# deepsound-project/pggan-pytorch

Measured on AMD Instinct MI355X. Metric: images/sec, PGGAN full train step (D+GP step + G step + Adam) at 1024x1024, higher is better.
Workload: dtype f32; 1 GPU; BASELINE config 5: PGGAN 1024x1024 net (fmap_base 4096, C=3, latent 512), stage depth 8 = 1024x1024, alpha 1.00, minibatch 3/GPU (reference schedule), Trainer.train(): WGAN-GP + Adam(0,0.99) at lr 0, fp32; resolution=1024, depth=8, minibatch_per_gpu=3, global_batch=3, parallelism=dp1, fmap_base=4096, hip_graphs=False

## Files before the change

pggan-pytorch_amd/_lib.py:

```python
import ast
import ctypes
import os
import re

_HERE = os.path.dirname(os.path.abspath(__file__))
LIB_PATH = os.environ.get('PGGAN_HIP_LIB') or os.path.join(_HERE, 'libpggan_hip.so')
_INCLUDE = os.path.join(os.path.dirname(_HERE), 'include')


class PgganLibraryError(RuntimeError):
    pass


P = ctypes.c_void_p
I = ctypes.c_int
L = ctypes.c_int64
F = ctypes.c_float
D = ctypes.c_double

_ARGTYPES = {'pg_stream_t': P, 'int': I, 'int64_t': L, 'float': F, 'double': D, 'size_t': ctypes.c_size_t, 'uint64_t': ctypes.c_uint64}
_RESTYPES = {'int': I, 'const char*': ctypes.c_char_p}


def _define_value(name, text):
    def value(node):
        if isinstance(node, ast.Constant) and type(node.value) is int:
            return node.value
        if isinstance(node, ast.UnaryOp) and isinstance(node.op, ast.USub):
            return -value(node.operand)
        if isinstance(node, ast.BinOp) and isinstance(node.op, ast.LShift):
            return value(node.left) << value(node.right)
        raise PgganLibraryError('#define %s %s: not an integer expression' % (name, text))
    try:
        return value(ast.parse(text.strip(), mode='eval').body)
    except SyntaxError:
        raise PgganLibraryError('#define %s %s: not an integer expression' % (name, text))


def _argtype(name, param):
    if '*' in param:
        return P
    words = [w for w in param.split() if w != 'const']
    ctype = ' '.join(words[:-1])
    if ctype not in _ARGTYPES or not re.fullmatch(r'[A-Za-z_]\w*', words[-1]):
        raise PgganLibraryError('%s: parameter "%s" has no ctypes mapping' % (name, ' '.join(param.split())))
    return _ARGTYPES[ctype]


def parse_header(text):
    text = re.sub(r'/\*.*?\*/|//[^\n]*', ' ', text, flags=re.S)
    guards = set(re.findall(r'^[ \t]*#[ \t]*define[ \t]+(\w+)[ \t]*$', text, flags=re.M))
    constants, body, conditionals = {}, [], []
    for line in text.split('\n'):
        directive = re.match(r'\s*#\s*(\w+)\s*(.*?)\s*$', line)
        foreign = next((c for c in conditionals if c), None)
        if foreign and re.search(r'\bpg_\w+\s*\(|#\s*define\s+PG_', line):
            raise PgganLibraryError('declaration under the preprocessor conditional "%s": %s' % (foreign, line.strip()))
        if not directive:
            body.append(line)
            continue
        word, rest = directive.groups()
        if word in ('if', 'ifdef', 'ifndef'):
            known = (word, rest) == ('ifdef', '__cplusplus') or word == 'ifndef' and rest in guards
            conditionals.append(None if known else line.strip())
        elif word == 'endif':
            conditionals.pop()
        elif word == 'define' and rest.startswith('PG_'):
            name, value = re.match(r'(\w+)(.*)', rest).groups()
            constants[name] = _define_value(name, value)
    body = '\n'.join(body)
    argtypes, restypes = {}, {}
    for m in re.finditer(r'\b(pg_\w+)\s*\(', body):
        name = m.group(1)
        params = re.compile(r'([^()]*)\)\s*;').match(body, m.end())
        if not params:
            raise PgganLibraryError('%s: cannot read the parameter list' % name)
        ret = ' '.join(body[max(body.rfind(c, 0, m.start()) for c in ';{}') + 1:m.start()].split()).replace(' *', '*')
        if ret not in _RESTYPES:
            raise PgganLibraryError('%s: return type "%s" has no ctypes mapping' % (name, ret))
        params = [p.strip() for p in params.group(1).split(',')]
        argtypes[name] = [] if params in ([''], ['void']) else [_argtype(name, p) for p in params]
        restypes[name] = _RESTYPES[ret]
    return argtypes, restypes, constants


def _read_header(name):
    try:
        with open(os.path.join(_INCLUDE, name)) as f:
            return parse_header(f.read())
    except OSError as e:
        raise PgganLibraryError('cannot read the C-ABI header %s: %s' % (name, e))


SIGNATURES, _RESTYPE_OF, CONSTANTS = _read_header('pggan_hip.h')
DEBUG_SIGNATURES, _debug_restypes, _ = _read_header('pggan_hip_debug.h')
_RESTYPE_OF.update(_debug_restypes)
CLUSTER_SIGNATURES, _cluster_restypes, CLUSTER_CONSTANTS = _read_header('pggan_hip_cluster.h')
_RESTYPE_OF.update(_cluster_restypes)
GAN_SIGNATURES, _gan_restypes, GAN_CONSTANTS = _read_header('pggan_hip_gan.h')
_RESTYPE_OF.update(_gan_restypes)
PHASE_SIGNATURES, _phase_restypes, PHASE_CONSTANTS = _read_header('pggan_hip_phase.h')
_RESTYPE_OF.update(_phase_restypes)
SAMPLING_SIGNATURES, _sampling_restypes, SAMPLING_CONSTANTS = _read_header('pggan_hip_sampling.h')
_RESTYPE_OF.update(_sampling_restypes)
PROJECTION_SIGNATURES, _projection_restypes, PROJECTION_CONSTANTS = _read_header('pggan_hip_projection.h')
_RESTYPE_OF.update(_projection_restypes)
CROP_SIGNATURES, _crop_restypes, CROP_CONSTANTS = _read_header('pggan_hip_crop.h')
_RESTYPE_OF.update(_crop_restypes)
SWD_SIGNATURES, _swd_restypes, SWD_CONSTANTS = _read_header('pggan_hip_swd.h')
_RESTYPE_OF.update(_swd_restypes)
MEL_SIGNATURES, _mel_restypes, MEL_CONSTANTS = _read_header('pggan_hip_mel.h')
_RESTYPE_OF.update(_mel_restypes)
RESAMPLE_SIGNATURES, _resample_restypes, RESAMPLE_CONSTANTS = _read_header('pggan_hip_resample.h')
_RESTYPE_OF.update(_resample_restypes)
SHIFT_SIGNATURES, _shift_restypes, SHIFT_CONSTANTS = _read_header('pggan_hip_shift.h')
_RESTYPE_OF.update(_shift_restypes)
PRD_SIGNATURES, _prd_restypes, PRD_CONSTANTS = _read_header('pggan_hip_prd.h')
_RESTYPE_OF.update(_prd_restypes)
AUGMENT_SIGNATURES, _augment_restypes, AUGMENT_CONSTANTS = _read_header('pggan_hip_augment.h')
_RESTYPE_OF.update(_augment_restypes)
EMBED_SIGNATURES, _embed_restypes, EMBED_CONSTANTS = _read_header('pggan_hip_embed.h')
_RESTYPE_OF.update(_embed_restypes)
ABI_VERSION = CONSTANTS['PG_ABI_VERSION']

_lib = None


def load():
    global _lib
    if _lib is not None:
        return _lib
    if not os.path.exists(LIB_PATH):
        raise PgganLibraryError(
            'libpggan_hip.so not found at %s: the HIP extension is not built (run '
            '`python __graft_entry__.py`). There is no CPU fallback.' % LIB_PATH)
    try:
        lib = ctypes.CDLL(LIB_PATH)
    except OSError as e:
        raise PgganLibraryError('cannot load %s: %s' % (LIB_PATH, e))
    for name, argtypes in (list(SIGNATURES.items()) + list(DEBUG_SIGNATURES.items()) + list(CLUSTER_SIGNATURES.items())
                           + list(GAN_SIGNATURES.items()) + list(PHASE_SIGNATURES.items()) + list(SAMPLING_SIGNATURES.items())
                           + list(PROJECTION_SIGNATURES.items()) + list(CROP_SIGNATURES.items()) + list(SWD_SIGNATURES.items())
                           + list(MEL_SIGNATURES.items()) + list(RESAMPLE_SIGNATURES.items()) + list(SHIFT_SIGNATURES.items())
                           + list(PRD_SIGNATURES.items()) + list(AUGMENT_SIGNATURES.items()) + list(EMBED_SIGNATURES.items())):
        try:
            fn = getattr(lib, name)
        except AttributeError:
            raise PgganLibraryError('symbol %s missing from %s' % (name, LIB_PATH))
        fn.argtypes = argtypes
        fn.restype = _RESTYPE_OF[name]
    v = lib.pg_abi_version()
    if v != ABI_VERSION:
        raise PgganLibraryError('ABI version mismatch: library %d, binding %d' % (v, ABI_VERSION))
    _lib = lib
    return lib


_ERR = {CONSTANTS['PG_E_ARG']: 'PG_E_ARG (bad dimension / null pointer)', CONSTANTS['PG_E_ALIGN']: 'PG_E_ALIGN (channel count / alignment)',
        CONSTANTS['PG_E_UNSUP']: 'PG_E_UNSUP (unsupported configuration)', CONSTANTS['PG_E_NOLIB']: 'PG_E_NOLIB (no RCCL library could be loaded)'}
_E_UNSUP, _E_RCCL_BASE = CONSTANTS['PG_E_UNSUP'], CONSTANTS['PG_E_RCCL_BASE']


class Unsupported(RuntimeError):
    """PG_E_UNSUP: the entry point does not take this configuration (callers with a fallback catch exactly this)."""


def check(rc, name):
    if rc != 0:
        what = _ERR.get(rc) or ('RCCL ncclResult_t %d' % (_E_RCCL_BASE - rc) if rc <= _E_RCCL_BASE else 'hipError_t %d' % rc)
        raise (Unsupported if rc == _E_UNSUP else RuntimeError)('%s failed: %s' % (name, what))


CALL_HOOK = None


def call(name, *args):
    fn = getattr(load(), name)
    check(fn(*args) if CALL_HOOK is None else CALL_HOOK(fn, args, name), name)
```

pggan-pytorch_amd/csrc/conv_api.hip:

```cpp
#include "convp.h"

__thread char pgk::g_last_kernel[96] = "";
__thread int pgk::g_tune[4] = {-1, -1, -1, -1};

namespace {

using namespace pgk;

__device__ __forceinline__ void pack_dgrad_tile(const float* __restrict__ w, float* __restrict__ wt, int KS, int Cout, int Cin,
                                                int tap, int ci_b, int co_b)
{
    __shared__ float tile[32][33];
    const int kh = tap / KS, kw = tap % KS;
    const int otap = (KS - 1 - kh) * KS + (KS - 1 - kw);
    const int tx = threadIdx.x & 31, ty = threadIdx.x >> 5;
    for (int r = ty; r < 32; r += 8) {
        const int co = co_b + r, ci = ci_b + tx;
        tile[r][tx] = (co < Cout && ci < Cin) ? w[((size_t)tap * Cout + co) * Cin + ci] : 0.f;
    }
    __syncthreads();
    for (int r = ty; r < 32; r += 8) {
        const int ci = ci_b + r, co = co_b + tx;
        if (ci < Cin && co < Cout) wt[((size_t)otap * Cin + ci) * Cout + co] = tile[tx][r];
    }
}

__global__ void pack_dgrad_kernel(const float* __restrict__ w, float* __restrict__ wt, int KS, int Cout, int Cin)
{
    pack_dgrad_tile(w, wt, KS, Cout, Cin, blockIdx.z, blockIdx.x * 32, blockIdx.y * 32);
}

constexpr int PACK_MAX_LAYERS = 32;
struct PackDesc {
    int n;
    int first_block[PACK_MAX_LAYERS + 1];
    long long off[PACK_MAX_LAYERS];
    int ks[PACK_MAX_LAYERS], cout[PACK_MAX_LAYERS], cin[PACK_MAX_LAYERS];
};

__global__ void pack_dgrad_batched_kernel(const float* __restrict__ wbase, float* __restrict__ wtbase, PackDesc d)
{
    int l = 0;
    while (l + 1 < d.n && (int)blockIdx.x >= d.first_block[l + 1]) ++l;
    const int Cout = d.cout[l], Cin = d.cin[l];
    int b = blockIdx.x - d.first_block[l];
    const int nbx = (Cin + 31) / 32, nby = (Cout + 31) / 32;
    const int bx = b % nbx; b /= nbx;
    const int by = b % nby; const int tap = b / nby;
    pack_dgrad_tile(wbase + d.off[l], wtbase + d.off[l], d.ks[l], Cout, Cin, tap, bx * 32, by * 32);
}

}

static int second_pass(const ConvP& want, bool pooled, pg_stream_t stream)
{
    const int64_t P = (int64_t)want.N * want.Hout * want.Wout;
    if (want.ypool && !pooled)
        return pg_avgpool2_fwd(want.y, want.pool_other, want.ypool, want.N, want.Hout >> 1, want.Wout >> 1, want.Cout, want.pool_a, want.pool_b, stream);
    if (want.yup) return pg_avgpool2_bwd(want.y, want.upmask, want.yup, want.N, want.Hout, want.Wout, want.Cout, want.up_mul, want.mask_slope, stream);
    if (want.pn_r) return pg_pixelnorm_fwd(want.y, want.y, want.pn_r, P, want.Cout, want.pn_eps, stream);
    if (want.pnb_y) return pg_pixelnorm_lrelu_bwd(want.y, want.pnb_y, want.pnb_r, want.y, P, want.Cout, want.mask_slope, stream);
    return 0;
}

static bool thin_shape(const ConvP& p, bool channels)
{
    return channels && p.KS == 3 && p.pad == 1 && (p.Wout & 31) == 0 && (p.Hout & 7) == 0 && g_tune[PG_TUNE_PATH] != PG_PATH_NO_THIN;
}

static ConvP conv_request(const float* x, const float* w, const float* bias, const float* mask, float* y,
                          int N, int Hin, int Win, int Cin, int Cout, int KS, int pad, float scale, float slope, float mask_slope)
{
    ConvP p;
    p.x = x; p.w = w; p.bias = bias; p.mask = mask; p.y = y;
    p.N = N; p.Hin = Hin; p.Win = Win; p.Cin = Cin; p.Cout = Cout; p.KS = KS; p.pad = pad;
    p.scale = scale; p.slope = slope; p.mask_slope = mask_slope;
    return p;
}

static int conv2d_impl(ConvP& p, int flags, pg_stream_t stream)
{
    if (!p.x || !p.w || !p.y || p.N <= 0 || p.Hin <= 0 || p.Win <= 0 || p.Cin <= 0 || p.Cout <= 0) return PG_E_ARG;
    if ((p.Cin & 3) || (p.Cout & 3)) return PG_E_ALIGN;
    const int KS = p.KS, Cin = p.Cin, Cout = p.Cout;
    p.ups = flags & PG_FLAG_UPSAMPLE;
    p.mask_bytes = (flags & PG_FLAG_MASK_BYTES) ? 1 : 0; p.y_bytes = (flags & PG_FLAG_Y_BYTES) ? 1 : 0;
    if (flags & PG_FLAG_SIGNS_OUT) {
        if (!p.mask || p.mask_bytes) return PG_E_ARG;
        p.ysigns = reinterpret_cast<unsigned char*>(const_cast<float*>(p.mask));
        p.mask = nullptr;
    }
    p.Hout = p.Hin + 2 * p.pad - KS + 1; p.Wout = p.Win + 2 * p.pad - KS + 1;
    if (p.Hout <= 0 || p.Wout <= 0 || !is_pow2(p.Hout) || !is_pow2(p.Wout)) return PG_E_UNSUP;
    if (p.ups && ((p.Hin | p.Win) & 1)) return PG_E_ARG;
    if (p.ypool && ((p.Hout | p.Wout) & 1)) return PG_E_ARG;
    if ((long long)p.N * p.Hin * p.Win * Cin >= (1ll << 31) || (long long)p.N * p.Hout * p.Wout * Cout >= (1ll << 31) ||
        (long long)KS * KS * Cout * Cin >= (1ll << 31)) return PG_E_UNSUP;
    const ConvP want = p;
    if (KS != 3) p.ypool = nullptr;
    p.yup = nullptr; p.pn_r = nullptr; p.pnb_y = nullptr;
    hipStream_t s = (hipStream_t)stream;
    int rc;
    if (p.mask_bytes || p.y_bytes || p.ysigns) {
        if (KS != 3 || (p.y_bytes && !p.ypool) || want.pn_r || want.pnb_y) return PG_E_UNSUP;
        p.yup = want.yup;
        const bool thin_plain = !p.y_bytes && !p.yup && !p.ypool && ((Cout == 8 && (Cin == 8 || Cin == 16)) || (Cout == 16 && Cin == 8 && p.mask));
        const bool thin_pool = g_tune[PG_TUNE_PATH] != PG_PATH_NO_THIN_POOL16 && !p.yup && p.ypool && Cout == 16 && Cin == 8;
        return thin_shape(p, thin_plain || thin_pool) ? dispatch_thin(p, s) : dispatch_conv_tile(p, s);
    }
    const bool thin_pn = thin_shape(p, Cout == 8 && (Cin == 8 || Cin == 16));
    if (want.pnb_y && want.pnb_r && KS == 3 && Cout <= 32) {
        p.pnb_y = want.pnb_y;
        rc = thin_pn ? dispatch_thin(p, s) : dispatch_conv_tile(p, s);
        if (rc != PG_E_UNSUP) return rc;
        p.pnb_y = nullptr;
    }
    if (want.pn_r && KS == 3 && Cout <= 32 && !p.mask && g_tune[PG_TUNE_PATH] != PG_PATH_UNFUSED_PIXELNORM) {
        p.pn_r = want.pn_r;
        rc = thin_pn ? dispatch_thin(p, s) : dispatch_conv_tile(p, s);
        if (rc != PG_E_UNSUP) return rc;
        p.pn_r = nullptr;
    }
    if (want.yup && KS == 3) {
        p.yup = want.yup;
        rc = dispatch_conv_tile(p, s);
        if (rc != PG_E_UNSUP) return rc;
        p.yup = nullptr;
    }
    if (thin_shape(p, (Cout == 8 && (Cin == 8 || Cin == 16)) || (Cout == 16 && Cin == 8 && p.mask && !want.ypool)))
        rc = dispatch_thin(p, s);
    else if (k4_layer(p, KS))
        rc = launch_k4_conv(p, s);
    else
        rc = dispatch_conv_tile(p, s);
    if (rc) return rc;
    return second_pass(want, p.ypool && p.ksplit == 1, stream);
}

extern "C" int pg_conv2d_nhwc(const float* x, const float* w, const float* bias, const float* mask, float* y,
                              int N, int Hin, int Win, int Cin, int Cout, int KS, int pad, int ups,
                              float scale, float slope, float mask_slope, pg_stream_t stream)
{
    ConvP p = conv_request(x, w, bias, mask, y, N, Hin, Win, Cin, Cout, KS, pad, scale, slope, mask_slope);
    return conv2d_impl(p, ups, stream);
}

extern "C" int pg_conv2d_pixelnorm_nhwc(const float* x, const float* w, const float* bias, float* y, float* r,
                                        int N, int Hin, int Win, int Cin, int Cout, int KS, int pad, int ups,
                                        float scale, float slope, float eps, pg_stream_t stream)
{
    if (!r) return PG_E_ARG;
    ConvP p = conv_request(x, w, bias, nullptr, y, N, Hin, Win, Cin, Cout, KS, pad, scale, slope, 0.2f);
    p.pn_r = r; p.pn_eps = eps;
    return conv2d_impl(p, ups, stream);
}

extern "C" int pg_conv2d_pnbwd_nhwc(const float* x, const float* w, const float* ysaved, const float* r, float* y,
                                    int N, int Hin, int Win, int Cin, int Cout, int KS, int pad,
                                    float scale, float slope, pg_stream_t stream)
{
    if (!ysaved) return PG_E_ARG;
    ConvP p = conv_request(x, w, nullptr, nullptr, y, N, Hin, Win, Cin, Cout, KS, pad, scale, 1.0f, slope);
    p.pnb_y = ysaved; p.pnb_r = r;
    return conv2d_impl(p, 0, stream);
}

extern "C" int pg_conv2d_unpool_nhwc(const float* x, const float* w, const float* upmask, float* y, float* yup,
                                     int N, int Hin, int Win, int Cin, int Cout, int KS, int pad, int flags,
                                     float scale, float up_mul, float mask_slope, pg_stream_t stream)
{
    if (!yup) return PG_E_ARG;
    ConvP p = conv_request(x, w, nullptr, nullptr, y, N, Hin, Win, Cin, Cout, KS, pad, scale, 1.0f, mask_slope);
    p.yup = yup; p.upmask = upmask; p.up_mul = up_mul;
    return conv2d_impl(p, flags & PG_FLAG_MASK_BYTES, stream);
}

extern "C" int pg_conv2d_pool_nhwc(const float* x, const float* w, const float* bias, const float* mask, float* y,
                                   float* ypool, const float* pool_other, float pool_a, float pool_b, int pool_only,
                                   int N, int Hin, int Win, int Cin, int Cout, int KS, int pad, int ups,
                                   float scale, float slope, float mask_slope, pg_stream_t stream)
{
    if (!ypool) return PG_E_ARG;
    ConvP p = conv_request(x, w, bias, mask, y, N, Hin, Win, Cin, Cout, KS, pad, scale, slope, mask_slope);
    p.ypool = ypool; p.pool_other = pool_other; p.pool_a = pool_a; p.pool_b = pool_b; p.pool_only = pool_only;
    return conv2d_impl(p, ups, stream);
}

extern "C" int pg_conv2d_unpooled_nhwc(const float* g, const float* w, const unsigned char* gbytes, float gmul, float gslope,
                                       const float* mask, float* y, int N, int Hin, int Win, int Cin, int Cout, int flags,
                                       float scale, float mask_slope, pg_stream_t stream)
{
    if (!g || !w || !gbytes || !y || N <= 0 || Hin <= 0 || Win <= 0) return PG_E_ARG;
    if ((Hin | Win) & 1) return PG_E_ARG;
    if (!(Cout == 8 && (Cin == 8 || Cin == 16)) || (Win & 31) || (Hin & 7) || !is_pow2(Hin) || !is_pow2(Win)) return PG_E_UNSUP;
    if ((long long)N * Hin * Win * Cin >= (1ll << 31)) return PG_E_UNSUP;
    ConvP p = conv_request(g, w, nullptr, mask, y, N, Hin, Win, Cin, Cout, 3, 1, scale, 1.f, mask_slope);
    p.ups = 1; p.Hout = Hin; p.Wout = Win;
    p.mask_bytes = (flags & PG_FLAG_MASK_BYTES) ? 1 : 0;
    p.gbytes = gbytes; p.gmul = gmul; p.gslope = gslope;
    return dispatch_thin(p, (hipStream_t)stream);
}

extern "C" int pg_conv2d_fromrgb_nhwc(const float* img, const float* rgb_w, const float* rgb_b, float rgb_scale, float rgb_slope,
                                      unsigned char* x_signs, const float* w, const float* bias, float* y, unsigned char* y_signs,
                                      int N, int C, int H, int W, int Cmid, int Cout, float scale, float slope, pg_stream_t stream)
{
    if (!img || !rgb_w || !w || !y || N <= 0 || C <= 0 || H <= 0 || W <= 0 || Cmid <= 0 || Cout <= 0) return PG_E_ARG;
    return pgk::launch_conv_strip_fromrgb(img, rgb_w, rgb_b, rgb_scale, rgb_slope, x_signs, w, bias, y, y_signs, N, C, H, W, Cmid, Cout,
                                          scale, slope, (hipStream_t)stream);
}

extern "C" int pg_conv2d_pixelnorm_torgb_nhwc(const float* x, const float* w, const float* bias, float* y, float* r,
                                              const float* t_w, const float* t_b, float t_scale, float* img,
                                              int N, int C, int H, int W, int Cin, int Cout, float scale, float slope, float eps,
                                              pg_stream_t stream)
{
    if (!x || !w || !y || !r || !t_w || !img || N <= 0 || C <= 0 || H <= 0 || W <= 0 || Cin <= 0 || Cout <= 0) return PG_E_ARG;
    return pgk::launch_conv_strip_pn_torgb(x, w, bias, y, r, t_w, t_b, t_scale, img, N, C, H, W, Cin, Cout, scale, slope, eps,
                                           (hipStream_t)stream);
}

extern "C" int pg_conv2d_masked_fromrgb_bwd_nhwc(const float* gz, const float* wt, const unsigned char* mask_bytes, float mask_slope, float* y,
                                                 const float* rgb_w, float rgb_scale, float* gimg,
                                                 const float* img, float* rgb_dw, float* rgb_db,
                                                 int N, int C, int H, int W, int Cin, int Cout, float scale, pg_stream_t stream)
{
    if (!gz || !wt || !mask_bytes || N <= 0 || C <= 0 || H <= 0 || W <= 0 || Cin <= 0 || Cout <= 0) return PG_E_ARG;
    if ((!gimg && !rgb_dw) || (gimg && !rgb_w) || (rgb_dw && !img) || (rgb_db && !rgb_dw)) return PG_E_ARG;
    return pgk::launch_conv_strip_masked_rgb_bwd(gz, wt, mask_bytes, mask_slope, y, rgb_w, rgb_scale, gimg, img, rgb_dw, rgb_db,
                                                 N, C, H, W, Cin, Cout, scale, (hipStream_t)stream);
}

extern "C" const char* pg_debug_last_conv_kernel(void) { return g_last_kernel; }

extern "C" int pg_debug_set_tuning(int key, int value)
{
    if (key < 0 || key >= 4) return PG_E_ARG;
    g_tune[key] = value;
    return 0;
}

extern "C" int pg_pack_dgrad_weights_batched(const float* wbase, float* wtbase, int nlayers, const int64_t* off,
                                             const int* ks, const int* cout, const int* cin, pg_stream_t stream)
{
    if (!wbase || !wtbase || nlayers <= 0 || !off || !ks || !cout || !cin) return PG_E_ARG;
    for (int l0 = 0; l0 < nlayers; l0 += PACK_MAX_LAYERS) {
        PackDesc d;
        d.n = nlayers - l0 < PACK_MAX_LAYERS ? nlayers - l0 : PACK_MAX_LAYERS;
        int total = 0;
        for (int l = 0; l < d.n; ++l) {
            const int i = l0 + l;
            if (ks[i] <= 0 || cout[i] <= 0 || cin[i] <= 0 || off[i] < 0) return PG_E_ARG;
            d.first_block[l] = total;
            d.off[l] = off[i]; d.ks[l] = ks[i]; d.cout[l] = cout[i]; d.cin[l] = cin[i];
            total += ((cin[i] + 31) / 32) * ((cout[i] + 31) / 32) * ks[i] * ks[i];
        }
        d.first_block[d.n] = total;
        hipLaunchKernelGGL(pack_dgrad_batched_kernel, dim3(total), dim3(256), 0, (hipStream_t)stream, wbase, wtbase, d);
    }
    return (int)hipGetLastError();
}

extern "C" int pg_pack_dgrad_weights(const float* w, float* wt, int KS, int Cout, int Cin, pg_stream_t stream)
{
    if (!w || !wt || KS <= 0 || Cout <= 0 || Cin <= 0) return PG_E_ARG;
    dim3 grid((Cin + 31) / 32, (Cout + 31) / 32, KS * KS);
    hipLaunchKernelGGL(pack_dgrad_kernel, grid, dim3(256), 0, (hipStream_t)stream, w, wt, KS, Cout, Cin);
    return (int)hipGetLastError();
}
```

pggan-pytorch_amd/csrc/conv_strip.hip:

```cpp
#include "convp.h"

#ifndef PG_STRIP_ABL
#define PG_STRIP_ABL 0
#endif

namespace {

using pgk::ConvP;
using pgk::pg_sign_byte;
using pgk::pg_sign_factors;
using pgk::g_last_kernel; using pgk::set_smem; using pgk::SMEM_ANY;

constexpr int SW = 64;
constexpr int RP = SW + 2;
constexpr int RB = 4;
constexpr int NBLK = 3;

enum { EPI_GENERIC = 0, EPI_FWD = 1, EPI_MASK = 2, EPI_PN = 3, EPI_PNB = 4 };

struct SArgs {
    const float* x; const float* w; const float* bias; const void* mask; float* y;
    unsigned char* ysigns; float* pn_r; const float* pnb_y; const float* pnb_r; float* ypool; const float* pool_other;
    float scale, slope, mask_slope, pn_eps, pool_a, pool_b;
    int H, W, ups, mask_bytes, y_bytes, pool_only;
    int strips, segs, seg_rows;
    const unsigned char* gbytes; float gmul, gslope;
    const float* rgb_w; const float* rgb_b; float rgb_scale, rgb_slope; int rgbC; unsigned char* xsigns;
    float* t_out; const float* t_w; const float* t_b; float t_scale; int tC, t_sc, t_sco, t_only;
    const float* fw_img; float* fw_dw; float* fw_db; float fw_scale;
};

template <int CIN> struct Blk {
    static constexpr int C4 = CIN / 4;
    static constexpr int USED = C4 * RB * RP;
    static constexpr int NWI = (USED + 63) / 64;
    static constexpr int NI = (NWI + 3) / 4;
    static constexpr int SLOTS = NWI * 64;
};

typedef __attribute__((address_space(3))) const char* lds_cptr;
typedef __attribute__((address_space(3))) const f32x4* lds_v4ptr;

__device__ __forceinline__ pg_u32x4 rsrc_words(const void* base, unsigned bytes)
{
    const unsigned long long a = (unsigned long long)base;
    return pg_u32x4{(unsigned)__builtin_amdgcn_readfirstlane((int)(unsigned)a),
                    (unsigned)__builtin_amdgcn_readfirstlane((int)((unsigned)(a >> 32) & 0xffffu)), bytes, 0x00020000u};
}
__device__ __forceinline__ void buf_store4(__amdgpu_buffer_rsrc_t r, unsigned voff, float4 v)
{
    __builtin_amdgcn_raw_buffer_store_b128(pg_u32x4{__float_as_uint(v.x), __float_as_uint(v.y), __float_as_uint(v.z), __float_as_uint(v.w)},
                                           r, (int)voff, 0, 0);
}

constexpr int RGB_MAXC = 3;
template <int COUT, int CIN, int EPI, bool WREG, int GM, int XM = 0>
__device__ __forceinline__ void conv_strip_body(const SArgs& p)
{
    constexpr bool GATH = GM != 0;
    using B = Blk<CIN>;
    constexpr int C4 = B::C4;
    constexpr int QO = COUT / 4, QP = 16 / QO, PXG = 4 * QP;
    constexpr int GPR = 32 / PXG, G = 2 * GPR;
    constexpr int BLKB = B::SLOTS * 16;
    constexpr bool GEN = EPI == EPI_GENERIC;
    extern __shared__ __align__(16) float lds[];
    constexpr int WS = CIN == 16 ? CIN + 4 : CIN;
    float* wl = lds + NBLK * B::SLOTS * 4;
    const int tid = threadIdx.x, lane = tid & 63, wave = __builtin_amdgcn_readfirstlane(tid >> 6);
    const int blk = lane >> 2, j = lane & 3, qo = blk % QO, qp = blk / QO;

    int t = (int)pg_xcd_remap(blockIdx.x, gridDim.x);
    const int strip = __builtin_amdgcn_readfirstlane(t % p.strips); t /= p.strips;
    const int seg = __builtin_amdgcn_readfirstlane(t % p.segs), n = __builtin_amdgcn_readfirstlane(t / p.segs);
    const int r0 = seg * p.seg_rows, ow0 = strip * SW;
    const int niter = p.seg_rows / RB;
    const int xH = p.ups ? (p.H >> 1) : p.H, xW = p.ups ? (p.W >> 1) : p.W;
    const unsigned npix = (unsigned)(p.H * p.W);

    const unsigned rowbytes = 4u * (unsigned)(xW * CIN);
    unsigned voff[B::NI], vstep[B::NI];
    const unsigned blkstep = (p.ups ? 2u : 4u) * rowbytes;
#pragma unroll
    for (int i = 0; i < B::NI; ++i) {
        const int sl = (i * 4 + wave) * 64 + lane;
        const int q = sl / (RB * RP), rem = sl - q * (RB * RP);
        const int m = rem / RP, px = rem - m * RP;
        const int col = ow0 - 1 + px, row = r0 - 1 + m;
        const bool ok = sl < B::USED && (unsigned)col < (unsigned)p.W;
        voff[i] = ok ? (unsigned)(p.ups ? (row >> 1) : row) * rowbytes + 4u * (unsigned)((p.ups ? (col >> 1) : col) * CIN + 4 * q) : PG_OOB;
        vstep[i] = ok ? blkstep : 0u;
    }
    const size_t ximg = (size_t)xH * xW * CIN;
    const pg_u32x4 rxs = rsrc_words(p.x + (size_t)n * ximg, (unsigned)(ximg * 4));
    const unsigned lds0 = (unsigned)(size_t)(__attribute__((address_space(3))) char*)lds;
    const unsigned wdst = __builtin_amdgcn_readfirstlane(lds0 + (unsigned)wave * 1024u);
    auto dma16 = [&](unsigned vo, unsigned dst) {
        unsigned keep;
        asm volatile("s_mov_b32 %0, m0\n\ts_mov_b32 m0, %3\n\ts_nop 0\n\tbuffer_load_dwordx4 %1, %2, 0 offen lds\n\ts_mov_b32 m0, %0"
                     : "=&s"(keep) : "v"(vo), "s"(rxs), "s"(dst) : "memory");
    };
    auto issue_block = [&](int pos) {
#pragma unroll
        for (int i = 0; i < B::NI; ++i) {
            if (i * 4 + wave < B::NWI) dma16(voff[i], wdst + (unsigned)pos * BLKB + (unsigned)i * 4096u);
            voff[i] += vstep[i];
        }
    };

    constexpr int NG = GATH ? (B::USED + 255) / 256 : 1;
    unsigned cvo[NG], cvs[NG], bvo[NG], bvs[NG];
    float4 gxr[NG];
    unsigned gbr[NG];
    __amdgpu_buffer_rsrc_t rgx = pg_make_rsrc(p.x + (size_t)n * ximg, (unsigned)(ximg * 4)), rgb = rgx;
    constexpr int NR = GM == 2 ? NG : 1;
    int rrow[NR];
    float rw[NR][4][RGB_MAXC], rb[NR][4], rpx[NR][RGB_MAXC];
    if constexpr (GM == 2) {
        rgx = pg_make_rsrc(p.x + (size_t)n * npix * p.rgbC, npix * (unsigned)p.rgbC * 4u);
        rgb = pg_make_rsrc(p.xsigns + (size_t)n * npix * C4, npix * C4);
#pragma unroll
        for (int i = 0; i < NG; ++i) {
            const int sl = i * 256 + tid;
            const int q = sl / (RB * RP), rem = sl - q * (RB * RP);
            const int m = rem / RP, px = rem - m * RP;
            const int col = ow0 - 1 + px;
            const bool ok = sl < B::USED && (unsigned)col < (unsigned)p.W;
            rrow[i] = ok ? r0 - 1 + m : -(1 << 28);
            cvo[i] = ok ? 4u * (unsigned)((r0 - 1 + m) * p.W + col) : PG_OOB;
            cvs[i] = ok ? 4u * (unsigned)(RB * p.W) : 0u;
            bvo[i] = (ok && px >= 1 && px <= SW) ? (unsigned)((r0 - 1 + m) * p.W + col) * C4 + q : PG_OOB;
            bvs[i] = (ok && px >= 1 && px <= SW) ? (unsigned)(RB * p.W * C4) : 0u;
            const int qq = sl < B::USED ? q : 0;
#pragma unroll
            for (int k = 0; k < 4; ++k) {
#pragma unroll
                for (int c = 0; c < RGB_MAXC; ++c) rw[i][k][c] = c < p.rgbC ? p.rgb_w[(4 * qq + k) * p.rgbC + c] : 0.f;
                rb[i][k] = p.rgb_b ? p.rgb_b[4 * qq + k] : 0.f;
            }
        }
    }
    if constexpr (GM == 1) {
        rgb = pg_make_rsrc(p.gbytes + (size_t)n * npix * C4, npix * C4);
#pragma unroll
        for (int i = 0; i < NG; ++i) {
            const int sl = i * 256 + tid;
            const int q = sl / (RB * RP), rem = sl - q * (RB * RP);
            const int m = rem / RP, px = rem - m * RP;
            const int col = ow0 - 1 + px, row = r0 - 1 + m;
            const bool ok = sl < B::USED && (unsigned)col < (unsigned)p.W;
            cvo[i] = ok ? (unsigned)(row >> 1) * rowbytes + 4u * (unsigned)((col >> 1) * CIN + 4 * q) : PG_OOB;
            cvs[i] = ok ? 2u * rowbytes : 0u;
            bvo[i] = ok ? (unsigned)(row * p.W + col) * C4 + q : PG_OOB;
            bvs[i] = ok ? (unsigned)(RB * p.W * C4) : 0u;
        }
    }
    auto gather_load = [&]() {
        if constexpr (GM == 2) {
#pragma unroll
            for (int i = 0; i < NG; ++i) {
                const bool in = (unsigned)rrow[i] < (unsigned)p.H;
#pragma unroll
                for (int c = 0; c < RGB_MAXC; ++c)
                    rpx[i][c] = c < p.rgbC ? __uint_as_float(__builtin_amdgcn_raw_buffer_load_b32(rgx, in ? (int)(cvo[i] + (unsigned)c * npix * 4u) : (int)PG_OOB, 0, 0)) : 0.f;
                cvo[i] += cvs[i];
            }
            return;
        }
#pragma unroll
        for (int i = 0; i < NG; ++i) {
            gxr[i] = pg_buf_load4(rgx, cvo[i], 0);
            gbr[i] = __builtin_amdgcn_raw_buffer_load_b8(rgb, (int)bvo[i], 0, 0);
            cvo[i] += cvs[i]; bvo[i] += bvs[i];
        }
    };
    auto gather_store = [&](int pos) {
        if constexpr (GM == 2) {
#pragma unroll
            for (int i = 0; i < NG; ++i) {
                const int sl = i * 256 + tid;
                const bool in = (unsigned)rrow[i] < (unsigned)p.H;
                float o[4];
#pragma unroll
                for (int k = 0; k < 4; ++k) {
                    float a = 0.f;
#pragma unroll
                    for (int c = 0; c < RGB_MAXC; ++c) if (c < p.rgbC) a = fmaf(rpx[i][c], rw[i][k][c], a);
                    const float v = __fadd_rn(__fmul_rn(a, p.rgb_scale), rb[i][k]);
                    o[k] = in ? (v > 0.f ? v : v * p.rgb_slope) : 0.f;
                }
                const float4 v4 = make_float4(o[0], o[1], o[2], o[3]);
                if (sl < B::SLOTS) *reinterpret_cast<float4*>(lds + (pos * B::SLOTS + sl) * 4) = (cvs[i] ? v4 : make_float4(0.f, 0.f, 0.f, 0.f));
                if (p.xsigns && in && rrow[i] >= r0 && rrow[i] < r0 + p.seg_rows && bvs[i])
                    __builtin_amdgcn_raw_buffer_store_b8(pg_sign_byte(v4), rgb, (int)bvo[i], 0, 0);
                bvo[i] += bvs[i];
                rrow[i] += RB;
            }
            return;
        }
#pragma unroll
        for (int i = 0; i < NG; ++i) {
            const int sl = i * 256 + tid;
            if (sl < B::SLOTS) {
                const float4 f = pg_sign_factors((unsigned char)gbr[i], p.gslope);
                const float4 v = gxr[i];
                *reinterpret_cast<float4*>(lds + (pos * B::SLOTS + sl) * 4) =
                    make_float4(v.x * (f.x * p.gmul), v.y * (f.y * p.gmul), v.z * (f.z * p.gmul), v.w * (f.w * p.gmul));
            }
        }
    };

    float4 wreg[WREG ? 9 : 1][WREG ? C4 : 1];
    if constexpr (WREG) {
#pragma unroll
        for (int tp = 0; tp < 9; ++tp)
#pragma unroll
            for (int c4 = 0; c4 < C4; ++c4)
                wreg[tp][c4] = *reinterpret_cast<const float4*>(p.w + ((size_t)(tp * COUT + 4 * qo + j) * CIN + 4 * c4));
    } else {
        for (int e = tid; e < 9 * COUT * C4; e += 256)
            *reinterpret_cast<float4*>(wl + (e / C4) * WS + 4 * (e % C4)) = *reinterpret_cast<const float4*>(p.w + 4 * e);
    }
    const float* wrow = wl + (4 * qo + j) * WS;

    if constexpr (GATH) {
        gather_load(); gather_store(0);
        gather_load(); gather_store(1);
    } else {
        issue_block(0);
        issue_block(1);
    }

    const int rp = wave >> 1;
    const int col0 = (wave & 1) * 32;
    const lds_cptr lbase = (lds_cptr)lds + (col0 + 4 * qp + j) * 16;

    const bool has_mask = (GEN && p.mask) || EPI == EPI_MASK;
    const bool mask_bytes = has_mask && p.mask_bytes;
    const bool has_pnb = (GEN && p.pnb_y) || EPI == EPI_PNB;
    const bool has_pn = (GEN && p.pn_r) || EPI == EPI_PN;
    const bool has_signs = (GEN || EPI == EPI_FWD) && p.ysigns;
    const bool has_pool = GEN && p.ypool;
    const bool y_bytes = GEN && p.y_bytes;
    const bool has_trgb = (XM & 1) != 0 && (EPI == EPI_PN || EPI == EPI_MASK) && p.t_out != nullptr;
    const bool has_fw = (XM & 2) != 0 && EPI == EPI_MASK && COUT == 8 && p.fw_dw != nullptr;
    const bool y_store = !(has_pool && p.pool_only) && !y_bytes && !((has_trgb || has_fw) && p.t_only);
    const __amdgpu_buffer_rsrc_t ry = y_bytes ? pg_make_rsrc((const unsigned char*)p.y + (size_t)n * npix * (COUT / 4), npix * (COUT / 4))
                                              : pg_make_rsrc(p.y + (size_t)n * npix * COUT, npix * COUT * 4u);
    __amdgpu_buffer_rsrc_t rmask = ry, rsig = ry, rpnr = ry, rpnby = ry, rpnbr = ry;
    if (has_mask) rmask = mask_bytes ? pg_make_rsrc((const unsigned char*)p.mask + (size_t)n * npix * (COUT / 4), npix * (COUT / 4))
                                     : pg_make_rsrc((const float*)p.mask + (size_t)n * npix * COUT, npix * COUT * 4u);
    if (has_signs) rsig = pg_make_rsrc(p.ysigns + (size_t)n * npix * (COUT / 4), npix * (COUT / 4));
    if (has_pn) rpnr = pg_make_rsrc(p.pn_r + (size_t)n * npix, npix * 4u);
    if (has_pnb) {
        rpnby = pg_make_rsrc(p.pnb_y + (size_t)n * npix * COUT, npix * COUT * 4u);
        rpnbr = pg_make_rsrc(p.pnb_r + (size_t)n * npix, npix * 4u);
    }
    const unsigned pix0 = (unsigned)((r0 + 2 * rp) * p.W + ow0 + col0 + 4 * qp + j);
    float4 bv = make_float4(0.f, 0.f, 0.f, 0.f);
    if (!has_mask && p.bias) bv = *reinterpret_cast<const float4*>(p.bias + 4 * qo);
    float tw[RGB_MAXC][4], tb[RGB_MAXC];
    float aw[4][RGB_MAXC], ab[4], fi[G][RGB_MAXC];
#pragma unroll
    for (int k = 0; k < 4; ++k) {
        ab[k] = 0.f;
#pragma unroll
        for (int c = 0; c < RGB_MAXC; ++c) aw[k][c] = 0.f;
    }
    __amdgpu_buffer_rsrc_t rfimg = ry;
    if (has_fw) rfimg = pg_make_rsrc(p.fw_img + (size_t)n * npix * p.tC, npix * (unsigned)p.tC * 4u);
    __amdgpu_buffer_rsrc_t rtout = ry;
    if (has_trgb) {
        rtout = pg_make_rsrc(p.t_out + (size_t)n * npix * p.tC, npix * (unsigned)p.tC * 4u);
#pragma unroll
        for (int c = 0; c < RGB_MAXC; ++c) {
#pragma unroll
            for (int k = 0; k < 4; ++k) tw[c][k] = c < p.tC ? p.t_w[c * p.t_sc + (4 * qo + k) * p.t_sco] : 0.f;
            tb[c] = (c < p.tC && p.t_b) ? p.t_b[c] : 0.f;
        }
    }

    f32x4 acc[G], acc2[G];
    auto compute = [&](auto ph_, auto rp_) {
        constexpr int PH = decltype(ph_)::value, RPAIR = decltype(rp_)::value;
#pragma unroll
        for (int g = 0; g < G; ++g) { acc[g] = f32x4{0.f, 0.f, 0.f, 0.f}; acc2[g] = f32x4{0.f, 0.f, 0.f, 0.f}; }
#pragma unroll
        for (int tp = 0; tp < ((PG_STRIP_ABL & 4) ? 1 : 9); ++tp) {
            const int dy = tp / 3, dx = tp % 3;
#pragma unroll
            for (int c4 = 0; c4 < C4; ++c4) {
                float4 a;
                if constexpr (WREG) a = wreg[tp][c4];
                else a = *reinterpret_cast<const float4*>(wrow + tp * COUT * WS + 4 * c4);
                f32x4 bq[G];
#pragma unroll
                for (int g = 0; g < G; ++g) {
                    const int m = 2 * RPAIR + g / GPR + dy;
                    const int pos = m < RB ? PH : (PH + 1) % NBLK;
                    const int off = ((pos * B::SLOTS) + c4 * (RB * RP) + (m & (RB - 1)) * RP + (g % GPR) * PXG + dx) * 16;
                    bq[g] = *(lds_v4ptr)(lbase + off);
                }
#pragma unroll
                for (int g = 0; g < G; ++g) acc[g] = __builtin_amdgcn_mfma_f32_4x4x1f32(a.x, bq[g][0], acc[g], 0, 0, 0);
#pragma unroll
                for (int g = 0; g < G; ++g) acc2[g] = __builtin_amdgcn_mfma_f32_4x4x1f32(a.y, bq[g][1], acc2[g], 0, 0, 0);
#pragma unroll
                for (int g = 0; g < G; ++g) acc[g] = __builtin_amdgcn_mfma_f32_4x4x1f32(a.z, bq[g][2], acc[g], 0, 0, 0);
#pragma unroll
                for (int g = 0; g < G; ++g) acc2[g] = __builtin_amdgcn_mfma_f32_4x4x1f32(a.w, bq[g][3], acc2[g], 0, 0, 0);
            }
        }
#pragma unroll
        for (int g = 0; g < G; ++g) acc[g] += acc2[g];
    };

    float4 pm[G];
    unsigned pmb[G];
    float prr[G];
    auto prefetch_epilogue = [&](unsigned pix) {
#pragma unroll
        for (int g = 0; g < G; ++g) {
            const unsigned pg_ = pix + (unsigned)((g / GPR) * p.W + (g % GPR) * PXG);
            if (has_fw) {
#pragma unroll
                for (int c = 0; c < RGB_MAXC; ++c)
                    fi[g][c] = c < p.tC ? __uint_as_float(__builtin_amdgcn_raw_buffer_load_b32(rfimg, (int)(((unsigned)c * npix + pg_) * 4u), 0, 0)) : 0.f;
            }
            if (has_mask) {
                if (mask_bytes) pmb[g] = __builtin_amdgcn_raw_buffer_load_b8(rmask, (int)(pg_ * (COUT / 4) + qo), 0, 0);
                else pm[g] = pg_buf_load4(rmask, (pg_ * COUT + 4 * qo) * 4u, 0);
            } else if (has_pnb) {
                pm[g] = pg_buf_load4(rpnby, (pg_ * COUT + 4 * qo) * 4u, 0);
                prr[g] = __uint_as_float(__builtin_amdgcn_raw_buffer_load_b32(rpnbr, (int)(pg_ * 4u), 0, 0));
            }
        }
    };
    auto epilogue = [&](unsigned pix) {
        float4 ov[G];
#pragma unroll
        for (int g = 0; g < G; ++g) {
            const unsigned pg_ = pix + (unsigned)((g / GPR) * p.W + (g % GPR) * PXG);
            const unsigned off = pg_ * COUT + 4 * qo;
            float4 o = make_float4(acc[g][0] * p.scale, acc[g][1] * p.scale, acc[g][2] * p.scale, acc[g][3] * p.scale);
            if (has_mask) {
                float4 f;
                if (mask_bytes) f = pg_sign_factors((unsigned char)pmb[g], p.mask_slope);
                else {
// ... 28 lines not shown
                o.x *= rr; o.y *= rr; o.z *= rr; o.w *= rr;
                if (qo == 0 && !(PG_STRIP_ABL & 2)) __builtin_amdgcn_raw_buffer_store_b32(__float_as_uint(rr), rpnr, (int)(pg_ * 4u), 0, 0);
            }
            if (has_fw) {
                const float ov4[4] = {o.x, o.y, o.z, o.w};
#pragma unroll
                for (int k = 0; k < 4; ++k) {
                    ab[k] += ov4[k];
#pragma unroll
                    for (int c = 0; c < RGB_MAXC; ++c) aw[k][c] = fmaf(ov4[k], fi[g][c], aw[k][c]);
                }
            }
            if (has_trgb) {
#pragma unroll
                for (int c = 0; c < RGB_MAXC; ++c) {
                    if (c >= p.tC) break;
                    float a = fmaf(o.w, tw[c][3], fmaf(o.z, tw[c][2], fmaf(o.y, tw[c][1], o.x * tw[c][0])));
                    a += __shfl_xor(a, 4, 64);
                    if (QO >= 4) a += __shfl_xor(a, 8, 64);
                    if (qo == 0) __builtin_amdgcn_raw_buffer_store_b32(__float_as_uint(fmaf(a, p.t_scale, tb[c])), rtout, (int)(((unsigned)c * npix + pg_) * 4u), 0, 0);
                }
            }
            if (!(PG_STRIP_ABL & 2)) {
                if (y_bytes) __builtin_amdgcn_raw_buffer_store_b8(pg_sign_byte(o), ry, (int)(off >> 2), 0, 0);
                else if (y_store) buf_store4(ry, off * 4u, o);
            }
            ov[g] = o;
        }
        if (has_pool) {
#pragma unroll
            for (int g = 0; g < G; ++g) {
                ov[g].x += __shfl_xor(ov[g].x, 1, 64); ov[g].y += __shfl_xor(ov[g].y, 1, 64);
                ov[g].z += __shfl_xor(ov[g].z, 1, 64); ov[g].w += __shfl_xor(ov[g].w, 1, 64);
            }
#pragma unroll
            for (int g = 0; g < GPR; ++g) {
                float4 v = make_float4((ov[g].x + ov[g + GPR].x) * 0.25f, (ov[g].y + ov[g + GPR].y) * 0.25f,
                                       (ov[g].z + ov[g + GPR].z) * 0.25f, (ov[g].w + ov[g + GPR].w) * 0.25f);
                if (j & 1) continue;
                const unsigned pg_ = pix + (unsigned)(g * PXG);
                const unsigned oy = pg_ / (unsigned)p.W, ox = pg_ - oy * (unsigned)p.W;
                const size_t poff = (((size_t)n * (p.H >> 1) + (oy >> 1)) * (p.W >> 1) + (ox >> 1)) * COUT + 4 * qo;
                if (p.pool_other) {
                    const float4 q = *reinterpret_cast<const float4*>(p.pool_other + poff);
                    v.x = fmaf(v.x, p.pool_a, p.pool_b * q.x); v.y = fmaf(v.y, p.pool_a, p.pool_b * q.y);
                    v.z = fmaf(v.z, p.pool_a, p.pool_b * q.z); v.w = fmaf(v.w, p.pool_a, p.pool_b * q.w);
                } else if (p.pool_a != 1.f) { v.x *= p.pool_a; v.y *= p.pool_a; v.z *= p.pool_a; v.w *= p.pool_a; }
                *reinterpret_cast<float4*>(p.ypool + poff) = v;
            }
        }
    };

    int nstores = (y_bytes || y_store) ? G : 0;
    if (has_signs) nstores += G;
    if (has_pn) nstores += G;
    if (has_pool) nstores += GPR;
    if (has_trgb) nstores += G * p.tC;
    if (PG_STRIP_ABL & 2) nstores = 0;
    nstores = __builtin_amdgcn_readfirstlane(nstores);
    auto wait_dma = [&]() {
        if constexpr (EPI == EPI_MASK || EPI == EPI_PNB || EPI == EPI_PN) {
            static_assert(G == 2, "");
            if (!has_trgb && !has_fw) {
                if constexpr (EPI == EPI_PN) asm volatile("s_waitcnt vmcnt(4)" ::: "memory");
                else asm volatile("s_waitcnt vmcnt(2)" ::: "memory");
            } else switch (nstores) {
                case 2: asm volatile("s_waitcnt vmcnt(2)" ::: "memory"); break;
                case 4: asm volatile("s_waitcnt vmcnt(4)" ::: "memory"); break;
                case 6: asm volatile("s_waitcnt vmcnt(6)" ::: "memory"); break;
                case 8: asm volatile("s_waitcnt vmcnt(8)" ::: "memory"); break;
                case 10: asm volatile("s_waitcnt vmcnt(10)" ::: "memory"); break;
                default: asm volatile("s_waitcnt vmcnt(0)" ::: "memory"); break;
            }
        }
        else switch (nstores) {
            case 0: asm volatile("s_waitcnt vmcnt(0)" ::: "memory"); break;
            case 1: asm volatile("s_waitcnt vmcnt(1)" ::: "memory"); break;
            case 2: asm volatile("s_waitcnt vmcnt(2)" ::: "memory"); break;
            case 3: asm volatile("s_waitcnt vmcnt(3)" ::: "memory"); break;
            case 4: asm volatile("s_waitcnt vmcnt(4)" ::: "memory"); break;
            case 5: asm volatile("s_waitcnt vmcnt(5)" ::: "memory"); break;
            default: asm volatile("s_waitcnt vmcnt(6)" ::: "memory"); break;
        }
    };
    unsigned pix = pix0;
    const unsigned pixstep = (unsigned)(RB * p.W);
    auto step = [&](int it, auto ph_) {
        constexpr int PH = decltype(ph_)::value;
        if constexpr (!GATH) {
            if (it == 0 || (PG_STRIP_ABL & 2)) asm volatile("s_waitcnt vmcnt(0)" ::: "memory");
            else wait_dma();
        }
        __syncthreads();
        const bool more = it + 2 <= niter;
        if constexpr (GATH) { if (more) gather_load(); }
        else if (more && !((PG_STRIP_ABL & 1) && it > 0)) issue_block((PH + 2) % NBLK);
        prefetch_epilogue(pix);
        __builtin_amdgcn_sched_barrier(0);
        if (rp == 0) compute(ph_, std::integral_constant<int, 0>{});
        else compute(ph_, std::integral_constant<int, 1>{});
        if constexpr (GATH) { if (more) gather_store((PH + 2) % NBLK); }
        epilogue(pix);
        pix += pixstep;
    };
    for (int it = 0; it < niter; it += 3) {
        step(it, std::integral_constant<int, 0>{});
        if (it + 1 < niter) step(it + 1, std::integral_constant<int, 1>{});
        if (it + 2 < niter) step(it + 2, std::integral_constant<int, 2>{});
    }
    if (has_fw) {
        static_assert(COUT != 8 || QO == 2, "");
        float v[16];
#pragma unroll
        for (int k = 0; k < 4; ++k) {
#pragma unroll
            for (int c = 0; c < RGB_MAXC; ++c) v[4 * k + c] = aw[k][c];
            v[4 * k + 3] = ab[k];
        }
#pragma unroll
        for (int i = 0; i < 16; ++i) {
            float a = v[i];
            a += __shfl_xor(a, 1, 64); a += __shfl_xor(a, 2, 64); a += __shfl_xor(a, 8, 64); a += __shfl_xor(a, 16, 64); a += __shfl_xor(a, 32, 64);
            v[i] = a;
        }
        __syncthreads();
        if ((lane & ~4) == 0) {
#pragma unroll
            for (int i = 0; i < 16; ++i) lds[(wave * 2 + (lane >> 2)) * 16 + i] = v[i];
        }
        __syncthreads();
        const int q2 = (tid >> 4) & 1, i = tid & 15, k = i >> 2, c = i & 3, co = 4 * q2 + k;
        auto commit = [&](float a) {
            if (c < 3) { if (c < p.tC) atomicAdd(p.fw_dw + co * p.tC + c, a * p.fw_scale); }
            else if (p.fw_db) atomicAdd(p.fw_db + co, a);
        };
        float a = 0.f;
        if (tid < 32) a = (lds[(0 * 2 + q2) * 16 + i] + lds[(1 * 2 + q2) * 16 + i]) + (lds[(2 * 2 + q2) * 16 + i] + lds[(3 * 2 + q2) * 16 + i]);
        if (tid < 32) commit(a);
    }
}

template <int COUT, int CIN, int EPI, bool WREG, bool GATH>
__global__ __launch_bounds__(256, GATH ? 2 : (WREG ? 3 : 4)) void conv_strip_kernel(SArgs p)
{
    conv_strip_body<COUT, CIN, EPI, WREG, GATH ? 1 : 0>(p);
}

template <int EPI, bool WREG, int XM>
__global__ __launch_bounds__(256, 3) void conv_strip_x_kernel(SArgs p)
{
    conv_strip_body<8, 8, EPI, WREG, 0, XM>(p);
}

template <int EPI>
__global__ __launch_bounds__(256, 2) void conv_strip_rgb_kernel(SArgs p)
{
    conv_strip_body<8, 8, EPI, false, 2>(p);
}

template <int COUT, int CIN, int EPI, bool WREG, bool GATH = false>
int launch_strip(const SArgs& a, int N, hipStream_t s)
{
    using B = Blk<CIN>;
    const size_t smem = (size_t)NBLK * B::SLOTS * 16 + (WREG ? 0 : (size_t)9 * COUT * (CIN == 16 ? CIN + 4 : CIN) * 4);
    auto kern = conv_strip_kernel<COUT, CIN, EPI, WREG, GATH>;
    if (int rc = set_smem(kern, smem, SMEM_ANY)) return rc;
    snprintf(g_last_kernel, sizeof(g_last_kernel), "conv_strip_kernel<%d, %d, %d, %s, %s>", COUT, CIN, EPI, WREG ? "true" : "false", GATH ? "true" : "false");
    hipLaunchKernelGGL(kern, dim3((unsigned)(N * a.strips * a.segs)), dim3(256), smem, s, a);
    return (int)hipGetLastError();
}

template <int EPI, bool WREG, int XM>
int launch_strip_x(const SArgs& a, int N, hipStream_t s)
{
    const size_t smem = (size_t)NBLK * Blk<8>::SLOTS * 16 + (WREG ? 0 : (size_t)9 * 8 * 8 * 4);
    auto kern = conv_strip_x_kernel<EPI, WREG, XM>;
    if (int rc = set_smem(kern, smem, SMEM_ANY)) return rc;
    snprintf(g_last_kernel, sizeof(g_last_kernel), "conv_strip_x_kernel<%d, %s, %d>", EPI, WREG ? "true" : "false", XM);
    hipLaunchKernelGGL(kern, dim3((unsigned)(N * a.strips * a.segs)), dim3(256), smem, s, a);
    return (int)hipGetLastError();
}

template <int COUT, int CIN, bool WREG>
int launch_strip_epi(const SArgs& a, int epi, int N, hipStream_t s)
{
    switch (epi) {
        case EPI_FWD: return launch_strip<COUT, CIN, EPI_FWD, WREG>(a, N, s);
        case EPI_MASK: return launch_strip<COUT, CIN, EPI_MASK, WREG>(a, N, s);
        case EPI_PN: return launch_strip<COUT, CIN, EPI_PN, WREG>(a, N, s);
        case EPI_PNB: return launch_strip<COUT, CIN, EPI_PNB, WREG>(a, N, s);
        default: return launch_strip<COUT, CIN, EPI_GENERIC, WREG>(a, N, s);
    }
}

struct WArgs { const float* x; const float* gz; float* dw; float* db; float scale; int H, W, ups, strips, segs, seg_rows;
               const unsigned char* gbytes; float gmul, gslope; };

template <int CO, int CI, bool GATH>
__global__ __launch_bounds__(256, 2) void wgrad_strip_kernel(WArgs p)
{
    constexpr int TAPS = 9;
    constexpr int QO = CO / 4, QI = CI / 4, NB = QO * QI, PPM = 16 / NB, RNG = SW / PPM;
    static_assert(NB == 4 || NB == 8, "8x8, 16x8 or 8x16 channels");
    constexpr int XU = RNG + 2, XRS = PPM * XU;
    constexpr int XBS = 320, GBS = RB * SW;
    static_assert(RB * XRS <= XBS, "");
    constexpr int XRING = 3, GRING = 2;
    constexpr int XPS = XRING * XBS + 2, GPS = GRING * GBS + 2;
    constexpr int XNWI = QI * 5, GNWI = QO * RB, XNI = (XNWI + 3) / 4, GNI = (GNWI + 3) / 4;
    extern __shared__ __align__(16) float lds[];
    const unsigned lds0 = (unsigned)(size_t)(__attribute__((address_space(3))) char*)lds;
    constexpr unsigned GLDS = (unsigned)QI * XPS * 16;
    const int tid = threadIdx.x, lane = tid & 63, wave = __builtin_amdgcn_readfirstlane(tid >> 6);
    const int blk = lane >> 2, i4 = lane & 3;
    const int hi = blk % QI, ho = (blk / QI) % QO, slot = blk / NB;

    int t = (int)pg_xcd_remap(blockIdx.x, gridDim.x);
    const int strip = __builtin_amdgcn_readfirstlane(t % p.strips); t /= p.strips;
    const int seg = __builtin_amdgcn_readfirstlane(t % p.segs), n = __builtin_amdgcn_readfirstlane(t / p.segs);
    const int r0 = seg * p.seg_rows, ow0 = strip * SW;
    const int niter = p.seg_rows / RB;
    const int xH = p.ups ? (p.H >> 1) : p.H, xW = p.ups ? (p.W >> 1) : p.W;

    const unsigned xrowbytes = 4u * (unsigned)(xW * CI), grow = 4u * (unsigned)(p.W * CO);
    unsigned xvoff[XNI], xvstep[XNI], xdst[XNI], gvoff[GNI], gdst[GNI];
    const unsigned xblkstep = (p.ups ? 2u : 4u) * xrowbytes;
#pragma unroll
    for (int i = 0; i < XNI; ++i) {
        const int ii = i * 4 + wave, q = ii / 5, part = ii - q * 5;
        const int idx = part * 64 + lane;
        const int m = idx / XRS, e = idx - m * XRS, u = e / PPM, s = e - u * PPM;
        const int col = ow0 + RNG * s + u - 1, row = r0 - 1 + m;
        const bool ok = ii < XNWI && idx < RB * XRS && (unsigned)col < (unsigned)p.W;
        xvoff[i] = ok ? (unsigned)(p.ups ? (row >> 1) : row) * xrowbytes + 4u * (unsigned)((p.ups ? (col >> 1) : col) * CI + 4 * q) : PG_OOB;
        xvstep[i] = ok ? xblkstep : 0u;
        xdst[i] = lds0 + (unsigned)(q * XPS + part * 64) * 16u;
    }
#pragma unroll
    for (int i = 0; i < GNI; ++i) {
        const int jj = i * 4 + wave, q = jj / RB, m = jj - q * RB;
        const int u = lane / PPM, s = lane - u * PPM;
        const int col = ow0 + RNG * s + u, row = r0 + m;
        gvoff[i] = jj < GNWI ? (unsigned)row * grow + 4u * (unsigned)(col * CO + 4 * q) : PG_OOB;
        gdst[i] = lds0 + GLDS + (unsigned)(q * GPS + m * SW) * 16u;
    }
    const size_t ximg = (size_t)xH * xW * CI, gimg = GATH ? (size_t)(p.H >> 1) * (p.W >> 1) * CO : (size_t)p.H * p.W * CO;
    const pg_u32x4 rxs = rsrc_words(p.x + (size_t)n * ximg, (unsigned)(ximg * 4));
    const pg_u32x4 rgs = rsrc_words(p.gz + (size_t)n * gimg, (unsigned)(gimg * 4));
    constexpr int NGZ = GATH ? QO : 1;
    unsigned cvo[NGZ], bvo[NGZ];
    float4 gxr[NGZ];
    unsigned gbr[NGZ];
    __amdgpu_buffer_rsrc_t rgc = pg_make_rsrc(p.gz + (size_t)n * gimg, (unsigned)(gimg * 4)), rgb = rgc;
    if constexpr (GATH) {
        rgb = pg_make_rsrc(p.gbytes + (size_t)n * p.H * p.W * QO, (unsigned)(p.H * p.W * QO));
        const int m = tid >> 6, e = tid & 63, u = e / PPM, s = e - u * PPM;
        const int col = ow0 + RNG * s + u, row = r0 + m;
#pragma unroll
        for (int q = 0; q < NGZ; ++q) {
            cvo[q] = 4u * (unsigned)(((row >> 1) * (p.W >> 1) + (col >> 1)) * CO + 4 * q);
            bvo[q] = (unsigned)(row * p.W + col) * QO + q;
        }
    }
    auto gather_load = [&]() {
#pragma unroll
        for (int q = 0; q < NGZ; ++q) {
            gxr[q] = pg_buf_load4(rgc, cvo[q], 0);
            gbr[q] = __builtin_amdgcn_raw_buffer_load_b8(rgb, (int)bvo[q], 0, 0);
            cvo[q] += 2u * 4u * (unsigned)((p.W >> 1) * CO); bvo[q] += (unsigned)(RB * p.W * QO);
        }
    };
    auto gather_store = [&](int pos) {
#pragma unroll
        for (int q = 0; q < NGZ; ++q) {
            const float4 f = pg_sign_factors((unsigned char)gbr[q], p.gslope);
            const float4 v = gxr[q];
            *reinterpret_cast<float4*>(lds + GLDS / 4 + ((q * GPS + pos * GBS) + tid) * 4) =
                make_float4(v.x * (f.x * p.gmul), v.y * (f.y * p.gmul), v.z * (f.z * p.gmul), v.w * (f.w * p.gmul));
        }
    };
    auto dma16 = [&](const pg_u32x4& rs, unsigned vo, unsigned dst) {
        unsigned keep;
        asm volatile("s_mov_b32 %0, m0\n\ts_mov_b32 m0, %3\n\ts_nop 0\n\tbuffer_load_dwordx4 %1, %2, 0 offen lds\n\ts_mov_b32 m0, %0"
                     : "=&s"(keep) : "v"(vo), "s"(rs), "s"(dst) : "memory");
    };
    auto issue_x = [&](int pos) {
#pragma unroll
        for (int i = 0; i < XNI; ++i) {
            if (i * 4 + wave < XNWI) dma16(rxs, xvoff[i], __builtin_amdgcn_readfirstlane(xdst[i]) + (unsigned)pos * (XBS * 16u));
            xvoff[i] += xvstep[i];
        }
    };
    auto issue_g = [&](int pos) {
#pragma unroll
        for (int i = 0; i < GNI; ++i) {
            if (i * 4 + wave < GNWI) dma16(rgs, gvoff[i], __builtin_amdgcn_readfirstlane(gdst[i]) + (unsigned)pos * (GBS * 16u));
            gvoff[i] += 4u * grow;
        }
    };
    issue_x(0);
    if constexpr (GATH) { gather_load(); gather_store(0); } else issue_g(0);
    issue_x(1);

    f32x4 acc[TAPS];
#pragma unroll
    for (int tp = 0; tp < TAPS; ++tp) acc[tp] = f32x4{0.f, 0.f, 0.f, 0.f};
    float bsum = 0.f;
    typedef __attribute__((address_space(3))) const float* lds_fptr;
    const lds_cptr xl = (lds_cptr)lds + (hi * XPS + slot) * 16 + i4 * 4;
    const lds_cptr gl = (lds_cptr)lds + GLDS + (ho * GPS + slot) * 16 + i4 * 4;

    for (int it = 0; it < niter; ++it) {
        asm volatile("s_waitcnt vmcnt(0)" ::: "memory");
        __syncthreads();
        if (it + 2 <= niter) issue_x((it + 2) % XRING);
        if constexpr (GATH) { if (it + 1 < niter) gather_load(); }
        else if (it + 1 < niter) issue_g((it + 1) % GRING);
        __builtin_amdgcn_sched_barrier(0);
        const int rr0 = (RB * (it % XRING) + wave);
        lds_cptr xb[3];
#pragma unroll
        for (int dy = 0; dy < 3; ++dy) {
            int rr = rr0 + dy; if (rr >= RB * XRING) rr -= RB * XRING;
            xb[dy] = xl + ((rr / RB) * XBS + (rr % RB) * XRS) * 16;
        }
        const lds_cptr gb = gl + ((it % GRING) * GBS + wave * SW) * 16;
        float bcol[3][3];
#pragma unroll
        for (int dy = 0; dy < 3; ++dy) {
            bcol[dy][0] = *(lds_fptr)(xb[dy] + 0 * PPM * 16);
            bcol[dy][1] = *(lds_fptr)(xb[dy] + 1 * PPM * 16);
        }
#pragma unroll
        for (int ks = 0; ks < RNG; ++ks) {
            const float a = *(lds_fptr)(gb + ks * PPM * 16);
#pragma unroll
            for (int dy = 0; dy < 3; ++dy) bcol[dy][(ks + 2) % 3] = *(lds_fptr)(xb[dy] + (ks + 2) * PPM * 16);
            bsum += a;
#pragma unroll
            for (int dy = 0; dy < 3; ++dy)
#pragma unroll
                for (int dx = 0; dx < 3; ++dx)
                    acc[dy * 3 + dx] = __builtin_amdgcn_mfma_f32_4x4x1f32(a, bcol[dy][(ks + dx) % 3], acc[dy * 3 + dx], 0, 0, 0);
        }
        if constexpr (GATH) { if (it + 1 < niter) gather_store((it + 1) % GRING); }
    }

#pragma unroll
    for (int tp = 0; tp < TAPS; ++tp)
#pragma unroll
        for (int r = 0; r < 4; ++r) {
            float v = acc[tp][r];
            v += __shfl_xor(v, 32, 64);
            if (PPM >= 4) v += __shfl_xor(v, 16, 64);
            acc[tp][r] = v;
        }
    bsum += __shfl_xor(bsum, 32, 64);
    if (PPM >= 4) bsum += __shfl_xor(bsum, 16, 64);
    constexpr int NL = 4 * NB, NE = TAPS * 4 + 1;
    __syncthreads();
    float* red = lds;
    if (lane < NL) {
#pragma unroll
        for (int tp = 0; tp < TAPS; ++tp)
#pragma unroll
            for (int r = 0; r < 4; ++r) red[(wave * NE + tp * 4 + r) * NL + lane] = acc[tp][r];
        red[(wave * NE + TAPS * 4) * NL + lane] = bsum;
    }
    __syncthreads();
    for (int e = tid; e < NE * NL; e += 256) {
        const int l = e % NL, ve = e / NL;
        const float v = (red[e] + red[e + NE * NL]) + (red[e + 2 * NE * NL] + red[e + 3 * NE * NL]);
        const int b_ = l >> 2, jj = l & 3;
        const int hi_ = b_ % QI, ho_ = (b_ / QI) % QO;
        if (ve < TAPS * 4) {
            const int tp = ve >> 2, r = ve & 3;
            atomicAdd(p.dw + ((size_t)(tp * CO + 4 * ho_ + r) * CI + 4 * hi_ + jj), v * p.scale);
        } else if (p.db && hi_ == 0) {
            atomicAdd(p.db + 4 * ho_ + jj, v);
        }
    }
}

template <int CO, int CI, bool GATH = false>
int launch_wgrad_strip_t(const WArgs& a, int N, hipStream_t s)
{
    constexpr int QO = CO / 4, QI = CI / 4;
    const size_t smem = ((size_t)QI * (3 * 320 + 2) + (size_t)QO * (2 * RB * SW + 2)) * 16;
    auto kern = wgrad_strip_kernel<CO, CI, GATH>;
    if (int rc = set_smem(kern, smem, SMEM_ANY)) return rc;
    snprintf(g_last_kernel, sizeof(g_last_kernel), "wgrad_strip_kernel<%d, %d, %s>", CO, CI, GATH ? "true" : "false");
    hipLaunchKernelGGL(kern, dim3((unsigned)(N * a.strips * a.segs)), dim3(256), smem, s, a);
    return (int)hipGetLastError();
}

int strip_seg_rows(int N, int H, int W)
{
    int seg = 64;
    while (seg > 16 && ((long long)N * (W / SW) * (H / seg) < 768 || (H % seg))) seg >>= 1;
    return (seg < 16 || (seg % RB) || (H % seg)) ? 0 : seg;
}

constexpr bool STRIP_WREG = true;

}

int pgk::launch_conv_strip(ConvP& p, hipStream_t s)
{
    if (p.KS != 3 || p.pad != 1 || p.yup || p.ksplit != 1) return PG_E_UNSUP;
    if ((p.Wout % SW) || (p.Hout % 16) || p.Hout != p.Hin || p.Wout != p.Win) return PG_E_UNSUP;
    if (!(p.Cout == 8 && (p.Cin == 8 || p.Cin == 16))) return PG_E_UNSUP;
    if ((long long)p.Hin * p.Win * 16 * 4 >= (1ll << 31)) return PG_E_UNSUP;
    const int seg = strip_seg_rows(p.N, p.Hout, p.Wout);
    if (!seg) return PG_E_UNSUP;
    SArgs a{};
    a.x = p.x; a.w = p.w; a.bias = p.bias; a.mask = p.mask; a.y = p.y;
    a.ysigns = p.ysigns; a.pn_r = p.pn_r; a.pnb_y = p.pnb_y; a.pnb_r = p.pnb_r; a.ypool = p.ypool; a.pool_other = p.pool_other;
    a.scale = p.scale; a.slope = p.slope; a.mask_slope = p.mask_slope; a.pn_eps = p.pn_eps; a.pool_a = p.pool_a; a.pool_b = p.pool_b;
    a.H = p.Hout; a.W = p.Wout; a.ups = p.ups; a.mask_bytes = p.mask_bytes; a.y_bytes = p.y_bytes; a.pool_only = p.pool_only;
    a.strips = p.Wout / SW; a.segs = p.Hout / seg; a.seg_rows = seg;
    a.gbytes = p.gbytes; a.gmul = p.gmul; a.gslope = p.gslope;
    if (p.gbytes) {
        if (!p.ups || p.bias || p.ypool || p.y_bytes || p.pnb_y || p.pn_r || p.ysigns) return PG_E_UNSUP;
        if (p.Cin == 8) return p.mask ? launch_strip<8, 8, EPI_MASK, false, true>(a, p.N, s)
                                      : launch_strip<8, 8, EPI_FWD, false, true>(a, p.N, s);
        return p.mask ? launch_strip<8, 16, EPI_MASK, false, true>(a, p.N, s)
                      : launch_strip<8, 16, EPI_FWD, false, true>(a, p.N, s);
    }
    int epi = EPI_GENERIC;
    if (!p.ypool && !p.y_bytes) {
        if (p.pnb_y && !p.mask && !p.pn_r && !p.ysigns) epi = EPI_PNB;
        else if (p.pn_r && !p.mask && !p.pnb_y && !p.ysigns) epi = EPI_PN;
        else if (p.mask && !p.pnb_y && !p.pn_r) epi = EPI_MASK;
        else if (!p.mask && !p.pnb_y && !p.pn_r) epi = EPI_FWD;
    }
    if (p.Cin == 8) return launch_strip_epi<8, 8, STRIP_WREG>(a, epi, p.N, s);
    return launch_strip_epi<8, 16, false>(a, epi, p.N, s);
}

int pgk::launch_conv_strip_fromrgb(const float* img, const float* rgb_w, const float* rgb_b, float rgb_scale, float rgb_slope,
                                   unsigned char* x_signs, const float* w, const float* bias, float* y, unsigned char* y_signs,
                                   int N, int C, int H, int W, int Cmid, int Cout, float scale, float slope,
                                   hipStream_t s)
{
    if (C > RGB_MAXC || Cmid != 8 || Cout != 8 || (W % SW) || (H % 16)) return PG_E_UNSUP;
    if ((long long)H * W * 16 * 4 >= (1ll << 31)) return PG_E_UNSUP;
    const int seg = strip_seg_rows(N, H, W);
    if (!seg) return PG_E_UNSUP;
    SArgs a{};
    a.x = img; a.w = w; a.bias = bias; a.y = y; a.ysigns = y_signs;
    a.scale = scale; a.slope = slope; a.mask_slope = 1.f; a.pool_a = 1.f;
    a.H = H; a.W = W; a.strips = W / SW; a.segs = H / seg; a.seg_rows = seg;
    a.rgb_w = rgb_w; a.rgb_b = rgb_b; a.rgb_scale = rgb_scale; a.rgb_slope = rgb_slope; a.rgbC = C; a.xsigns = x_signs;
    const size_t smem = (size_t)NBLK * Blk<8>::SLOTS * 16 + (size_t)9 * 8 * 8 * 4;
    auto kern = conv_strip_rgb_kernel<EPI_FWD>;
    if (int rc = set_smem(kern, smem, SMEM_ANY)) return rc;
    snprintf(g_last_kernel, sizeof(g_last_kernel), "conv_strip_rgb_kernel<%d>", (int)EPI_FWD);
    hipLaunchKernelGGL(kern, dim3((unsigned)(N * a.strips * a.segs)), dim3(256), smem, s, a);
    return (int)hipGetLastError();
}

int pgk::launch_conv_strip_pn_torgb(const float* x, const float* w, const float* bias, float* y, float* r,
                                    const float* t_w, const float* t_b, float t_scale, float* img,
                                    int N, int C, int H, int W, int Cin, int Cout, float scale, float slope, float eps,
                                    hipStream_t s)
{
    if (C < 1 || C > RGB_MAXC || Cin != 8 || Cout != 8 || (W % SW) || (H % 16)) return PG_E_UNSUP;
    if ((long long)H * W * 16 * 4 >= (1ll << 31)) return PG_E_UNSUP;
    const int seg = strip_seg_rows(N, H, W);
    if (!seg) return PG_E_UNSUP;
    SArgs a{};
    a.x = x; a.w = w; a.bias = bias; a.y = y; a.pn_r = r; a.pn_eps = eps;
    a.scale = scale; a.slope = slope; a.mask_slope = 1.f; a.pool_a = 1.f;
    a.H = H; a.W = W; a.strips = W / SW; a.segs = H / seg; a.seg_rows = seg;
    a.t_out = img; a.t_w = t_w; a.t_b = t_b; a.t_scale = t_scale; a.tC = C; a.t_sc = Cout; a.t_sco = 1;
    return launch_strip_x<EPI_PN, STRIP_WREG, 1>(a, N, s);
}

int pgk::launch_conv_strip_masked_rgb_bwd(const float* gz, const float* wt, const unsigned char* mask_bytes, float mask_slope, float* y,
                                          const float* rgb_w, float rgb_scale, float* gimg,
                                          const float* img, float* rgb_dw, float* rgb_db,
                                          int N, int C, int H, int W, int Cin, int Cout, float scale,
                                          hipStream_t s)
{
    if (C < 1 || C > RGB_MAXC || Cin != 8 || Cout != 8 || (W % SW) || (H % 16)) return PG_E_UNSUP;
    if ((long long)H * W * 16 * 4 >= (1ll << 31)) return PG_E_UNSUP;
    const int seg = strip_seg_rows(N, H, W);
    if (!seg) return PG_E_UNSUP;
    SArgs a{};
    a.x = gz; a.w = wt; a.mask = mask_bytes; a.mask_bytes = 1; a.y = y;
    a.scale = scale; a.slope = 1.f; a.mask_slope = mask_slope; a.pool_a = 1.f;
    a.H = H; a.W = W; a.strips = W / SW; a.segs = H / seg; a.seg_rows = seg;
    a.t_out = gimg; a.t_w = rgb_w; a.t_b = nullptr; a.t_scale = rgb_scale; a.tC = C; a.t_sc = 1; a.t_sco = C; a.t_only = y ? 0 : 1;
    a.fw_img = img; a.fw_dw = rgb_dw; a.fw_db = rgb_db; a.fw_scale = rgb_scale;
    if (rgb_dw) return launch_strip_x<EPI_MASK, false, 3>(a, N, s);
    return launch_strip_x<EPI_MASK, false, 1>(a, N, s);
}

int pgk::launch_wgrad_strip(WgP& p, hipStream_t s)
{
    if (p.pad != 1 || p.Hout != p.Hin || p.Wout != p.Win || (p.gbytes && p.ups)) return PG_E_UNSUP;
    if ((p.Wout % SW) || (p.Hout % 16)) return PG_E_UNSUP;
    if (!((p.Cout == 8 && p.Cin == 8) || (p.Cout == 16 && p.Cin == 8) || (p.Cout == 8 && p.Cin == 16))) return PG_E_UNSUP;
    if ((long long)p.Hin * p.Win * 16 * 4 >= (1ll << 31)) return PG_E_UNSUP;
    int seg = 256;
    auto tasks = [&](int sg) { return (long long)p.N * (p.Wout / SW) * (p.Hout / sg); };
    while (seg > 64 && (seg > p.Hout || (p.Hout % seg) || tasks(seg) < 1024)) seg >>= 1;
    while (seg > 16 && (seg > p.Hout || (p.Hout % seg) || tasks(seg) < 512)) seg >>= 1;
    if (seg < 16 || (seg % RB) || (p.Hout % seg)) return PG_E_UNSUP;
    WArgs a;
    a.x = p.x; a.gz = p.gz; a.dw = p.dw; a.db = p.db; a.scale = p.scale;
    a.H = p.Hout; a.W = p.Wout; a.ups = p.ups; a.strips = p.Wout / SW; a.segs = p.Hout / seg; a.seg_rows = seg;
    a.gbytes = p.gbytes; a.gmul = p.gmul; a.gslope = p.gslope;
    if (p.gbytes) {
        if (p.Cout == 8 && p.Cin == 8) return launch_wgrad_strip_t<8, 8, true>(a, p.N, s);
        if (p.Cout == 16 && p.Cin == 8) return launch_wgrad_strip_t<16, 8, true>(a, p.N, s);
        return launch_wgrad_strip_t<8, 16, true>(a, p.N, s);
    }
    if (p.Cout == 8 && p.Cin == 8) return launch_wgrad_strip_t<8, 8>(a, p.N, s);
    if (p.Cout == 16 && p.Cin == 8) return launch_wgrad_strip_t<16, 8>(a, p.N, s);
    return launch_wgrad_strip_t<8, 16>(a, p.N, s);
}
```

pggan-pytorch_amd/csrc/conv_wgrad.hip:

```cpp
#include "convp.h"

namespace {

using namespace pgk;

#ifdef PG_WINO_TRACE
#define PG_WSTAMP(i) do { __builtin_amdgcn_sched_barrier(0); if (p.trace && lane == 0 && blockIdx.x < 1024 && (tile - t_begin) < 8) \
    p.trace[((size_t)(blockIdx.x * 4 + wave) * 8 + (tile - t_begin)) * 8 + (i)] = __builtin_amdgcn_s_memtime(); __builtin_amdgcn_sched_barrier(0); } while (0)
thread_local unsigned long long* g_wgrad_trace = nullptr;
#else
#define PG_WSTAMP(i) do { } while (0)
#endif

template <int KS, int WM, int WN, int WAVES_CO, int WAVES_CI, int BPX>
__global__ __launch_bounds__(256) void conv_wgrad_kernel(WgP p)
{
    constexpr int WAVES_K = 4 / (WAVES_CO * WAVES_CI);
    constexpr int BCO = 16 * WM * WAVES_CO, BCI = 16 * WN * WAVES_CI;
    constexpr int SZ = PixStride<BCO>::value, SX = PixStride<BCI>::value;
    constexpr int TAPS = KS * KS;
    constexpr int ZV = BCO / 4, XV = BCI / 4;
    constexpr int ZPT = (BPX * ZV + 255) / 256;
    constexpr int XMAX = KS == 1 ? BPX : (KS == 3 ? (BPX * 9) / 4 : 16 * BPX);
    constexpr int XPT = (XMAX * XV + 255) / 256;
    extern __shared__ __align__(16) float lds[];

    const int TW = 1 << p.lgTW, TH = 1 << p.lgTH;
    const int HT = TH + KS - 1, WT = TW + KS - 1;
    float* gzt = lds;
    float* xt = lds + BPX * SZ;

    const int tid = threadIdx.x, lane = tid & 63, wave = tid >> 6;
    const int wave_co = wave % WAVES_CO, wave_ci = (wave / WAVES_CO) % WAVES_CI, wave_k = wave / (WAVES_CO * WAVES_CI);
    const int li = lane & 15, kk = lane >> 4;
    const int co0 = blockIdx.y * BCO, ci0 = blockIdx.z * BCI;
    const bool do_bias = (p.db != nullptr) && blockIdx.z == 0 && wave_ci == 0;

    f32x4 acc[TAPS][WM][WN];
    f32x4 accb[WM];
#pragma unroll
    for (int tp = 0; tp < TAPS; ++tp)
#pragma unroll
        for (int m = 0; m < WM; ++m)
#pragma unroll
            for (int n = 0; n < WN; ++n) acc[tp][m][n] = f32x4{0.f, 0.f, 0.f, 0.f};
#pragma unroll
    for (int m = 0; m < WM; ++m) accb[m] = f32x4{0.f, 0.f, 0.f, 0.f};

    const int xH = p.ups ? (p.Hin >> 1) : p.Hin, xW = p.ups ? (p.Win >> 1) : p.Win;
    const int npix = p.TN * HT * WT;

    int zq[ZPT], zc[ZPT];
    int xq[XPT], xc[XPT], xdst[XPT];
#pragma unroll
    for (int i = 0; i < ZPT; ++i) {
        const int idx = tid + 256 * i;
        const int q = idx / ZV, v = idx - q * ZV;
        zq[i] = idx < BPX * ZV ? q : -1;
        zc[i] = co0 + 4 * v;
    }
#pragma unroll
    for (int i = 0; i < XPT; ++i) {
        const int idx = tid + 256 * i;
        const int q = idx / XV, v = idx - q * XV;
        const int r2 = (int)__umulhi((unsigned)q, p.mWT), tw = q - r2 * WT;
        const int tn = (int)__umulhi((unsigned)r2, p.mHT), th = r2 - tn * HT;
        xq[i] = q < npix ? ((tn << 20) | (th << 10) | tw) : -1;
        xc[i] = ci0 + 4 * v;
        xdst[i] = q * SX + 4 * v;
    }
    int tapoff[TAPS];
#pragma unroll
    for (int tp = 0; tp < TAPS; ++tp) tapoff[tp] = ((tp / KS) * WT + (tp % KS)) * SX;

    float4 zreg[ZPT], xreg[XPT];
    auto fetch = [&](int tile) {
        int t = tile;
        const int tw_i = t % p.tilesW; t /= p.tilesW;
        const int th_i = t % p.tilesH; t /= p.tilesH;
        const int n0 = t * p.TN;
        const int oh0 = th_i << p.lgTH, ow0 = tw_i << p.lgTW;
#pragma unroll
        for (int i = 0; i < ZPT; ++i) {
            float4 val = make_float4(0.f, 0.f, 0.f, 0.f);
            if (zq[i] >= 0) {
                const int q = zq[i];
                const int tw = q & (TW - 1), th = (q >> p.lgTW) & (TH - 1), tn = q >> (p.lgTW + p.lgTH);
                const int n = n0 + tn;
                if (n < p.N && zc[i] < p.Cout)
                    val = *reinterpret_cast<const float4*>(p.gz + (((size_t)n * p.Hout + oh0 + th) * p.Wout + ow0 + tw) * p.Cout + zc[i]);
            }
            zreg[i] = val;
        }
#pragma unroll
        for (int i = 0; i < XPT; ++i) {
            float4 val = make_float4(0.f, 0.f, 0.f, 0.f);
            if (xq[i] >= 0) {
                const int tw = xq[i] & 1023, th = (xq[i] >> 10) & 1023, tn = xq[i] >> 20;
                const int n = n0 + tn;
                int ih = oh0 + th - p.pad, iw = ow0 + tw - p.pad;
                if (n < p.N && xc[i] < p.Cin && (unsigned)ih < (unsigned)p.Hin && (unsigned)iw < (unsigned)p.Win) {
                    if (p.ups) { ih >>= 1; iw >>= 1; }
                    val = *reinterpret_cast<const float4*>(p.x + (((size_t)n * xH + ih) * xW + iw) * p.Cin + xc[i]);
                }
            }
            xreg[i] = val;
        }
    };

    const int t_begin = (int)pg_xcd_remap(blockIdx.x, gridDim.x) * p.tiles_per_block;
    const int t_end = min(t_begin + p.tiles_per_block, p.ntiles);
    constexpr int NSTEPS = BPX / 4;

    if (t_begin < t_end) fetch(t_begin);
    for (int tile = t_begin; tile < t_end; ++tile) {
#pragma unroll
        for (int i = 0; i < ZPT; ++i)
            if (zq[i] >= 0) *reinterpret_cast<float4*>(gzt + zq[i] * SZ + (zc[i] - co0)) = zreg[i];
#pragma unroll
        for (int i = 0; i < XPT; ++i)
            if (xq[i] >= 0) *reinterpret_cast<float4*>(xt + xdst[i]) = xreg[i];
        __syncthreads();
        if (tile + 1 < t_end) fetch(tile + 1);

        auto frag_addr = [&](int step, int& aoff, int& boff) {
            const int q = 4 * step + kk;
            const int tw = q & (TW - 1), th = (q >> p.lgTW) & (TH - 1), tn = q >> (p.lgTW + p.lgTH);
            aoff = q * SZ + wave_co * WM * 16 + li;
            boff = ((tn * HT + th) * WT + tw) * SX + wave_ci * WN * 16 + li;
        };
        float a[2][WM], b[2][TAPS][WN];
        auto load_frags = [&](int step, float (&af)[WM], float (&bf)[TAPS][WN]) {
            int ao, bo; frag_addr(step, ao, bo);
#pragma unroll
            for (int m = 0; m < WM; ++m) af[m] = gzt[ao + m * 16];
#pragma unroll
            for (int tp = 0; tp < TAPS; ++tp)
#pragma unroll
                for (int n = 0; n < WN; ++n) bf[tp][n] = xt[bo + tapoff[tp] + n * 16];
        };
        auto mfmas = [&](const float (&af)[WM], const float (&bf)[TAPS][WN]) {
            if (do_bias) {
#pragma unroll
                for (int m = 0; m < WM; ++m) accb[m] = MFMA16(af[m], 1.0f, accb[m]);
            }
#pragma unroll
            for (int tp = 0; tp < TAPS; ++tp)
#pragma unroll
                for (int m = 0; m < WM; ++m)
#pragma unroll
                    for (int n = 0; n < WN; ++n) acc[tp][m][n] = MFMA16(af[m], bf[tp][n], acc[tp][m][n]);
        };
        constexpr int T = NSTEPS / WAVES_K;
// ... 304 lines not shown
#pragma unroll
        for (int g = 0; g < GQ; ++g) {
#pragma unroll
            for (int tp = 0; tp < TAPS; ++tp)
#pragma unroll
                for (int r = 0; r < 4; ++r) red[(wave * NE + g * (TAPS * 4 + 1) + tp * 4 + r) * NL + lane] = acc[g][tp][r];
            red[(wave * NE + g * (TAPS * 4 + 1) + TAPS * 4) * NL + lane] = bsum[g];
        }
    }
    __syncthreads();
    for (int e = tid; e < NE * NL; e += 256) {
        const int l = e % NL, ve = e / NL;
        const int g = ve / (TAPS * 4 + 1), slot_e = ve % (TAPS * 4 + 1);
        const float v = (red[e] + red[e + NE * NL]) + (red[e + 2 * NE * NL] + red[e + 3 * NE * NL]);
        const int b_ = l >> 2, j = l & 3;
        const int hi_ = b_ % QI, ho_ = ((16 * g + b_) / QI) % QO;
        if (slot_e < TAPS * 4) {
            const int tp = slot_e >> 2, r = slot_e & 3;
            float* dst = p.dw + ((size_t)(tp * CO + 4 * ho_ + r) * CI + 4 * hi_ + j);
            if (p.atomic) atomicAdd(dst, v * p.scale); else *dst += v * p.scale;
        } else if (do_bias && hi_ == 0) {
            float* dst = p.db + 4 * ho_ + j;
            if (p.atomic) atomicAdd(dst, v); else *dst += v;
        }
    }
}

template <int CO, int CI, int BPX, bool FIX>
int launch_wgrad_thin_kernel(const WgP& p, int chunks, size_t smem, hipStream_t s)
{
    auto kern = conv_wgrad_thin_kernel<CO, CI, BPX, FIX>;
    if (int rc = set_smem(kern, smem)) return rc;
    hipLaunchKernelGGL(kern, dim3(chunks), dim3(256), smem, s, p);
    return (int)hipGetLastError();
}

template <int BPX, bool FIX>
int launch_wgrad_thin_shape(const WgP& p, int chunks, size_t smem, hipStream_t s)
{
    if (p.Cout == 8 && p.Cin == 8) return launch_wgrad_thin_kernel<8, 8, BPX, FIX>(p, chunks, smem, s);
    if (p.Cout == 16 && p.Cin == 8) return launch_wgrad_thin_kernel<16, 8, BPX, FIX>(p, chunks, smem, s);
    if (p.Cout == 8 && p.Cin == 16) return launch_wgrad_thin_kernel<8, 16, BPX, FIX>(p, chunks, smem, s);
    if (p.Cout == 32 && p.Cin == 16) return launch_wgrad_thin_kernel<32, 16, BPX, FIX>(p, chunks, smem, s);
    if (p.Cout == 16 && p.Cin == 32) return launch_wgrad_thin_kernel<16, 32, BPX, FIX>(p, chunks, smem, s);
    return PG_E_UNSUP;
}

template <int BPX>
int launch_wgrad_thin(WgP& p, hipStream_t s)
{
    if (g_tune[PG_TUNE_WGRAD] != PG_WGRAD_TILE_NOT_STRIP) {
        const int rc = launch_wgrad_strip(p, s);
        if (rc != PG_E_UNSUP) return rc;
    }
    TileGeom g;
    if (!set_geom(p, g, BPX, 3, halo_max(3, BPX))) return PG_E_UNSUP;
    if ((long long)g.TN * p.Hout * p.Wout * (p.Cout > p.Cin ? p.Cout : p.Cin) * 4 >= (1ll << 31)) return PG_E_UNSUP;
    const int sz = p.Cout == 16 ? 16 : p.Cout + 16, sx = p.Cin == 16 ? 16 : p.Cin + 16;
    size_t smem = ((size_t)BPX * sz + (size_t)g.halo * sx) * sizeof(float);
    const int nb = (p.Cout / 4) * (p.Cin / 4);
    const size_t red = (size_t)4 * (nb <= 16 ? 1 : nb / 16) * 37 * (nb <= 16 ? 4 * nb : 64) * sizeof(float);
    if (red > smem) smem = red;
    int chunks = 1024; if (chunks > g.ntiles) chunks = g.ntiles;
    p.tiles_per_block = (g.ntiles + chunks - 1) / chunks;
    chunks = (g.ntiles + p.tiles_per_block - 1) / p.tiles_per_block;
    p.atomic = chunks > 1 ? 1 : 0;
    snprintf(g_last_kernel, sizeof(g_last_kernel), "conv_wgrad_thin_kernel<%d, %d, %d>", p.Cout, p.Cin, BPX);
#ifdef PG_WINO_TRACE
    p.trace = g_wgrad_trace;
#endif
    const bool fix = BPX == 64 && g.lgTW == 4 && g.lgTH == 2 && g.TN == 1;
    return fix ? launch_wgrad_thin_shape<BPX, BPX == 64>(p, chunks, smem, s) : launch_wgrad_thin_shape<BPX, false>(p, chunks, smem, s);
}

template <int KS>
int dispatch_wgrad(WgP& p, hipStream_t s)
{
    if constexpr (KS == 4) {
        return launch_wgrad<KS, 1, 1, 2, 2, 16>(p, s);
    } else {
        const long long M = (long long)p.N * p.Hout * p.Wout;
        if (M <= 32) return launch_wgrad<KS, 1, 1, 2, 2, 16>(p, s);
        if constexpr (KS == 3) {
            if ((p.Cout == 16 && p.Cin == 32) || (p.Cout == 32 && p.Cin == 16 && M < 1500000))
                return launch_wgrad_thin<64>(p, s);
        }
        if (p.Cout <= 16 && p.Cin <= 16) {
            if constexpr (KS == 3) {
                if ((p.Cout == 8 || p.Cin == 8) && (p.Cout == 8 || p.Cout == 16) && (p.Cin == 8 || p.Cin == 16))
                    return launch_wgrad_thin<64>(p, s);
            }
            return launch_wgrad<KS, 1, 1, 1, 1, 128>(p, s);
        }
        if constexpr (KS == 3) {
            switch (g_tune[PG_TUNE_WGRAD]) {
                case PG_WGRAD_32x16_128PX: return launch_wgrad<KS, 2, 1, 1, 1, 128>(p, s);
                case PG_WGRAD_64x16_64PX: return launch_wgrad<KS, 2, 1, 2, 1, 64>(p, s);
                default: break;
            }
        }
        if constexpr (KS == 3) {
            const double macs = (double)M * p.Cout * p.Cin;
            if (g_tune[PG_TUNE_WGRAD] < 0 && macs >= 4e8) {
                if (p.Cin >= 64) return launch_wgrad<KS, 2, 1, 2, 1, 64>(p, s);
                return launch_wgrad<KS, 2, 1, 1, 1, 128>(p, s);
            }
        }
        return launch_wgrad<KS, 2, 1, 1, 1, 64>(p, s);
    }
}

}

extern "C" int pg_conv2d_wgrad_nhwc(const float* x, const float* gz, float* dw, float* db,
                                    int N, int Hin, int Win, int Cin, int Cout, int KS, int pad, int ups,
                                    float scale, pg_stream_t stream)
{
    if (!x || !gz || !dw || N <= 0 || Hin <= 0 || Win <= 0 || Cin <= 0 || Cout <= 0) return PG_E_ARG;
    if ((Cin & 3) || (Cout & 3)) return PG_E_ALIGN;
    WgP p;
    p.x = x; p.gz = gz; p.dw = dw; p.db = db;
    p.N = N; p.Hin = Hin; p.Win = Win; p.Cin = Cin; p.Cout = Cout; p.pad = pad; p.ups = ups;
    p.Hout = Hin + 2 * pad - KS + 1; p.Wout = Win + 2 * pad - KS + 1;
    if (p.Hout <= 0 || p.Wout <= 0 || !is_pow2(p.Hout) || !is_pow2(p.Wout)) return PG_E_UNSUP;
    if (ups && ((Hin | Win) & 1)) return PG_E_ARG;
    p.scale = scale;
    hipStream_t s = (hipStream_t)stream;
    if (k4_layer(p, KS)) return launch_k4_wgrad(p, s);
    switch (KS) {
        case 1: return dispatch_wgrad<1>(p, s);
        case 3: return dispatch_wgrad<3>(p, s);
        case 4: return dispatch_wgrad<4>(p, s);
        default: return PG_E_UNSUP;
    }
}

extern "C" int pg_conv2d_wgrad_unpooled_nhwc(const float* x, const float* g, const unsigned char* gbytes, float gmul, float gslope,
                                             float* dw, float* db, int N, int Hin, int Win, int Cin, int Cout,
                                             float scale, pg_stream_t stream)
{
    if (!x || !g || !gbytes || !dw || N <= 0 || Hin <= 0 || Win <= 0) return PG_E_ARG;
    if ((Hin | Win) & 1) return PG_E_ARG;
    if (!((Cout == 16 && Cin == 8) || (Cout == 8 && Cin == 8) || (Cout == 8 && Cin == 16)) || !is_pow2(Hin) || !is_pow2(Win) || Hin < 8 || Win < 8)
        return PG_E_UNSUP;
    WgP p;
    p.x = x; p.gz = g; p.dw = dw; p.db = db;
    p.N = N; p.Hin = Hin; p.Win = Win; p.Cin = Cin; p.Cout = Cout; p.pad = 1; p.ups = 0;
    p.Hout = Hin; p.Wout = Win;
    p.scale = scale;
    p.gbytes = gbytes; p.gmul = gmul; p.gslope = gslope;
    return launch_wgrad_thin<64>(p, (hipStream_t)stream);
}

#ifdef PG_WINO_TRACE
extern "C" int pg_debug_wgrad_trace(void* buf) { g_wgrad_trace = (unsigned long long*)buf; return 0; }
#endif
```

pggan-pytorch_amd/csrc/convp.h:

```cpp
#pragma once
#include <hip/hip_runtime.h>
#include <stdint.h>
#include <cstdio>
#include <type_traits>
#include "pggan_hip.h"
#include "pggan_hip_debug.h"
#include "bufload.h"

typedef float f32x4 __attribute__((ext_vector_type(4)));
#define MFMA16(a, b, c) __builtin_amdgcn_mfma_f32_16x16x4f32((a), (b), (c), 0, 0, 0)

namespace pgk {

inline int ilog2(int v) { int l = 0; while ((1 << l) < v) ++l; return l; }
inline bool is_pow2(int v) { return v > 0 && (v & (v - 1)) == 0; }

struct ConvP {
    const float* x = nullptr; const float* w = nullptr; const float* bias = nullptr; const float* mask = nullptr; float* y = nullptr;
    int N = 0, Hin = 0, Win = 0, Cin = 0, Cout = 0, Hout = 0, Wout = 0, KS = 0, pad = 0, ups = 0;
    float scale = 1.f, slope = 1.f, mask_slope = 1.f;
    int lgTW = 0, lgTH = 0, TN = 0, tilesW = 0, tilesH = 0;
    unsigned mWT = 0, mHT = 0;
    int ksplit = 1;
    float* ypool = nullptr; const float* pool_other = nullptr; float pool_a = 1.f, pool_b = 0.f; int pool_only = 0;
    float* yup = nullptr; const float* upmask = nullptr; float up_mul = 1.f;
    float* pn_r = nullptr; float pn_eps = 0.f;
    const float* pnb_y = nullptr; const float* pnb_r = nullptr;
    int mask_bytes = 0, y_bytes = 0;
    unsigned char* ysigns = nullptr;
    const unsigned char* gbytes = nullptr; float gmul = 1.f, gslope = 1.f;
};
static_assert(sizeof(ConvP) == 248 && std::is_trivially_copyable_v<ConvP>, "ConvP is a kernel argument: its layout is part of the compiled kernels");

__device__ __forceinline__ float4 pg_sign_factors(unsigned char b, float slope)
{
    return make_float4((b & 1) ? 1.f : slope, (b & 2) ? 1.f : slope, (b & 4) ? 1.f : slope, (b & 8) ? 1.f : slope);
}
__device__ __forceinline__ unsigned char pg_sign_byte(float4 o)
{
    return (unsigned char)((o.x > 0.f ? 1 : 0) | (o.y > 0.f ? 2 : 0) | (o.z > 0.f ? 4 : 0) | (o.w > 0.f ? 8 : 0));
}

struct WgP {
    const float* x = nullptr; const float* gz = nullptr; float* dw = nullptr; float* db = nullptr;
    int N = 0, Hin = 0, Win = 0, Cin = 0, Cout = 0, Hout = 0, Wout = 0, pad = 0, ups = 0;
    float scale = 1.f;
    int lgTW = 0, lgTH = 0, TN = 0, tilesW = 0, tilesH = 0, ntiles = 0, tiles_per_block = 0;
    unsigned mWT = 0, mHT = 0;
    int atomic = 0;
    const unsigned char* gbytes = nullptr; float gmul = 1.f, gslope = 1.f;
#ifdef PG_WINO_TRACE
    unsigned long long* trace = nullptr;
#endif
};
#ifndef PG_WINO_TRACE
static_assert(sizeof(WgP) == 128, "WgP is a kernel argument: its layout is part of the compiled kernels");
#endif
static_assert(std::is_trivially_copyable_v<WgP>, "WgP is a kernel argument");

struct Workspace { int device; hipStream_t stream; char* ptr; size_t bytes; };
constexpr size_t WS_TICKETS = 4096, WS_HEAD = WS_TICKETS * sizeof(unsigned);
bool find_workspace(hipStream_t s, Workspace& out);

template <int VEC> __device__ __forceinline__ void lds_load(const float* p, float (&o)[VEC]);
template <> __device__ __forceinline__ void lds_load<4>(const float* p, float (&o)[4]) {
    float4 v = *reinterpret_cast<const float4*>(p); o[0] = v.x; o[1] = v.y; o[2] = v.z; o[3] = v.w;
}
template <> __device__ __forceinline__ void lds_load<2>(const float* p, float (&o)[2]) {
    float2 v = *reinterpret_cast<const float2*>(p); o[0] = v.x; o[1] = v.y;
}
template <> __device__ __forceinline__ void lds_load<1>(const float* p, float (&o)[1]) { o[0] = *p; }

template <int VEC> struct RowStride { static constexpr int value = VEC == 4 ? 24 : (VEC == 2 ? 12 : 8); };

template <int B> struct PixStride { static constexpr int value = (B % 32 == 16) ? B : B + 16; };

constexpr int halo_max(int KS, int BPX)
{
    return KS == 1 ? BPX : (KS == 4 ? 16 * BPX : (BPX >= 512 ? (BPX / 32 + 2) * 34 : (BPX * 9) / 4));
}

template <typename P>
inline bool k4_layer(const P& p, int KS)
{
    return KS == 4 && !p.ups && (p.Cin & 15) == 0 && (p.Cout & 15) == 0 &&
           ((p.pad == 3 && p.Hin == 1 && p.Win == 1) || (p.pad == 0 && p.Hin == 4 && p.Win == 4));
}

struct TileGeom { int lgTW, lgTH, TN, tilesW, tilesH, ntiles, HT, WT, halo; };

inline TileGeom make_geom(int N, int Hout, int Wout, int BPX, int KS, int max_tw = 32)
{
    TileGeom g;
    int TW = Wout < max_tw ? Wout : max_tw; if (TW > BPX) TW = BPX;
    while (TW > 4 && BPX / TW < 4 && Hout >= 4) TW >>= 1;
    int TH = BPX / TW; if (TH > Hout) TH = Hout;
    g.lgTW = ilog2(TW); g.lgTH = ilog2(TH);
    g.TN = BPX / (TW * TH);
    g.tilesW = Wout / TW; g.tilesH = Hout / TH;
    g.ntiles = ((N + g.TN - 1) / g.TN) * g.tilesH * g.tilesW;
    g.HT = TH + KS - 1; g.WT = TW + KS - 1;
    g.halo = g.TN * g.HT * g.WT;
    return g;
}

template <typename P>
inline bool set_geom(P& p, TileGeom& g, int BPX, int KS, int halo_budget, int max_tw = 32)
{
    g = make_geom(p.N, p.Hout, p.Wout, BPX, KS, max_tw);
    p.lgTW = g.lgTW; p.lgTH = g.lgTH; p.TN = g.TN; p.tilesW = g.tilesW; p.tilesH = g.tilesH;
    if constexpr (std::is_same_v<P, WgP>) p.ntiles = g.ntiles;
    auto magic = [](int d) { return (unsigned)((1ull << 32) / (unsigned)d) + 1u; };
    p.mWT = magic(g.WT); p.mHT = magic(g.HT);
    return g.halo <= halo_budget;
}

inline int whole_slices(int nchunks, int ks)
{
    if (ks > nchunks) ks = nchunks;
    const int cper = (nchunks + ks - 1) / ks;
    return (nchunks + cper - 1) / cper;
}

inline int splitk_rule(long long blocks, int nchunks)
{
    if (blocks >= 192 || nchunks < 4) return 1;
    return whole_slices(nchunks, (int)((512 + blocks - 1) / blocks));
}

constexpr size_t SMEM_ANY = ~(size_t)0;
template <typename K>
inline int set_smem(K kern, size_t smem, size_t refuse_above = 160 * 1024)
{
    if (smem > refuse_above) return PG_E_UNSUP;
    if (smem > 48 * 1024) {
        hipError_t e = hipFuncSetAttribute(reinterpret_cast<const void*>(kern), hipFuncAttributeMaxDynamicSharedMemorySize, (int)smem);
        if (e != hipSuccess) return (int)e;
    }
    return 0;
}

extern __thread char g_last_kernel[96];
extern __thread int g_tune[4];

int dispatch_conv_tile(ConvP& p, hipStream_t s);
int dispatch_thin(ConvP& p, hipStream_t s);
int launch_k4_conv(ConvP& p, hipStream_t s);
int launch_k4_wgrad(WgP& p, hipStream_t s);
int launch_conv_strip(ConvP& p, hipStream_t s);
int launch_wgrad_strip(WgP& p, hipStream_t s);
int launch_conv_strip_pn_torgb(const float* x, const float* w, const float* bias, float* y, float* r,
                               const float* t_w, const float* t_b, float t_scale, float* img,
                               int N, int C, int H, int W, int Cin, int Cout, float scale, float slope, float eps, hipStream_t s);
int launch_conv_strip_masked_rgb_bwd(const float* gz, const float* wt, const unsigned char* mask_bytes, float mask_slope, float* y,
                                     const float* rgb_w, float rgb_scale, float* gimg, const float* img, float* rgb_dw, float* rgb_db,
                                     int N, int C, int H, int W, int Cin, int Cout, float scale, hipStream_t s);
int launch_conv_strip_fromrgb(const float* img, const float* rgb_w, const float* rgb_b, float rgb_scale, float rgb_slope,
                              unsigned char* x_signs, const float* w, const float* bias, float* y, unsigned char* y_signs,
                              int N, int C, int H, int W, int Cmid, int Cout, float scale, float slope, hipStream_t s);

}
```

pggan-pytorch_amd/engine.py:

```python
import collections as _collections
import contextlib as _contextlib
import os
import weakref as _weakref

import torch

from . import ops
from . import saved


def _check_dev(t, what):
    if not torch.is_tensor(t) or not t.is_cuda:
        raise RuntimeError('%s must be a tensor on the MI355X device (no CPU path exists); got %s'
                           % (what, getattr(t, 'device', type(t))))
    if t.dtype != torch.float32:
        raise RuntimeError('%s must be float32' % what)
    return t.contiguous()


USE_WINOGRAD = True
WINO_MIN_WORKGROUPS = 32
_WINO_MIN_CHANNELS = 8
_WINO_MIN_COUT = 16
_WINO_WGRAD_MIN_CHANNELS = 16
# ... 216 lines not shown
    if mask is None or mask.bytes is None:
        return run(mask and mask.f32, False)
    return _bytes_first(run, mask, lambda: 'dgrad masked %dx%d %s' % (Hout, Hout, tuple(layer.conv.weight.shape)))


def _dgrad_pool(net, gz, layer, N, H, other=None, a=1.0, b=0.0, pnb=None):
    u = _wino(layer, N, H, layer.conv.weight.shape[3], transposed=True)
    if pnb is not None:
        if u is not None and u.shape[1] <= 32 and pnb[1] is not None:
            return ops.conv2d_wino_pnbwd(gz, u, pnb[0], pnb[1], N, H, H, layer.c, pnb[2], pool=True, other=other, a=a, b=b), True
        return _dgrad_pool(net, gz, layer, N, H, other=other, a=a, b=b), False
    if u is not None:
        return ops.conv2d_wino(gz, u, None, N, H, H, layer.c, 1.0, pool=True, other=other, a=a, b=b, pool_only=True)[1]
    return ops.conv2d_pool(gz, _wt(net, layer), None, N, H, H, layer.ksize, layer.ksize - 1 - layer.pad, layer.c, 1.0,
                           other=other, a=a, b=b, pool_only=True)[1]


def _dgrad_unpool(net, gz, layer, N, H, up, mul):
    u = _wino(layer, N, H, layer.conv.weight.shape[3], transposed=True)
    if u is not None:
        return ops.conv2d_wino(gz, u, None, N, H, H, layer.c, 1.0, mask_slope=up.slope, unpool=True,
                               upmask=up.bytes if up.bytes is not None else up.f32, up_mul=mul)

    def launch(mask):
        return ops.conv2d_unpool(gz, _wt(net, layer), N, H, H, layer.ksize, layer.ksize - 1 - layer.pad, layer.c,
                                 upmask=mask(), mul=mul, mask_slope=up.slope)
    return _bytes_first(lambda m, _: launch(lambda: m), up, lambda: 'dgrad unpool %dx%d %s' % (H, H, tuple(layer.conv.weight.shape)),
                        redo=lambda: launch(lambda: _f32(up)))


def _dgrad_pnbwd(net, gz, layer, N, H, ysaved, r, slope):
    u = _wino(layer, N, H, layer.conv.weight.shape[3], transposed=True)
    if u is not None and u.shape[1] <= 32 and r is not None:
        return ops.conv2d_wino_pnbwd(gz, u, ysaved, r, N, H, H, layer.c, slope)
    if u is not None:
        g = ops.conv2d_wino(gz, u, None, N, H, H, layer.c, 1.0)
        return ops.pixelnorm_lrelu_bwd(g, ysaved, r, slope, inplace=True)
    return ops.conv2d_pnbwd(gz, _wt(net, layer), ysaved, r, N, H, H, layer.ksize, layer.ksize - 1 - layer.pad, layer.c, slope)


ASYNC_WGRAD = os.environ.get('PGGAN_ASYNC_WGRAD', '1') != '0'
DERIVED_EVENT = True
_SIDE = {}


def _wait_stream(waiter, other):
    waiter.wait_stream(other)


def _record_event(ev, stream):
    ev.record(stream)


def _wait_event(stream, ev):
    stream.wait_event(ev)


PROBES = None


def probe(tag):
    if PROBES is not None:
        ev = torch.cuda.Event(enable_timing=True)
        _record_event(ev, torch.cuda.current_stream(torch._C._cuda_getDevice()))
        PROBES.setdefault(tag, []).append(ev)


def _side_stream():
    dev = torch.cuda.current_device()
    if dev not in _SIDE:
        _SIDE[dev] = torch.cuda.Stream(device=dev)
        ops._no_workspace_streams.add(_SIDE[dev].cuda_stream)
    return _SIDE[dev]


class _on_side(object):

    def __init__(self, *tensors):
        self.tensors = [t for t in tensors if t is not None]
        self.active = ASYNC_WGRAD and len(self.tensors) > 0 and self.tensors[0].is_cuda

    def __enter__(self):
        if not self.active:
            return self
        main = torch.cuda.current_stream(torch._C._cuda_getDevice())
        self.side = _side_stream()
        _wait_stream(self.side, main)
        self.ctx = torch.cuda.stream(self.side)
        self.ctx.__enter__()
        return self

    def __exit__(self, *exc):
        if not self.active:
            return False
        self.ctx.__exit__(*exc)
        for t in self.tensors:
            t.record_stream(self.side)
        return False


def _join_side():
    if ASYNC_WGRAD and torch.cuda.is_available() and torch.cuda.current_device() in _SIDE:
        _wait_stream(torch.cuda.current_stream(torch._C._cuda_getDevice()), _SIDE[torch.cuda.current_device()])


def defer_to_side(net, fn):
    if not (ASYNC_WGRAD and net._flat_param.is_cuda):
        fn()
        return
    main = torch.cuda.current_stream(torch._C._cuda_getDevice())
    side = _side_stream()
    side.wait_stream(main)
    rt = net._rt
    rt.defer_active = True
    try:
        with torch.cuda.stream(side):
            fn()
            ev = rt.take('pending_ev')
            if ev is None:
                ev = torch.cuda.Event()
                ev.record(side)
    finally:
        rt.defer_active = False
    rt.pending = ev


def wait_pending(net):
    ev = net._rt.pending
    if ev is not None:
        torch.cuda.current_stream(torch._C._cuda_getDevice()).wait_event(ev)
        net._rt.pending = None


def _grads_ready(net, layers):
    hook = net._rt.grad_hook
    if hook is not None:
        for m in layers:
            if m._pending_wgrad is not None:
                _flush_wgrad(m)
        side = None
        if ASYNC_WGRAD and net._flat_param.is_cuda:
            side = _SIDE.get(torch.cuda.current_device())
        hook(layers, side)


DEFER_TANGENT_WGRAD = True


def _wino_wgrad_ok(layer, Hin):
    return (USE_WINOGRAD and layer.ksize == 3 and layer.pad == 1 and Hin >= 16 and not (Hin & (Hin - 1))
            and min(layer._gw.shape[2], layer._gw.shape[3]) >= _WINO_WGRAD_MIN_CHANNELS)


def _tail_wgrad_on_main(H):
    return 2 if H >= 1024 else 1 if H >= 512 else 0


def _on_main(*tensors):
    return _contextlib.nullcontext()


def _wgrad(x, gz, layer, N, Hin, bias=True, ups=False, defer=False, on_main=False):
    wino = _wino_wgrad_ok(layer, Hin)
    if defer and wino and DEFER_TANGENT_WGRAD and not bias and not ups:
        layer._pending_wgrad = (x, gz, N, Hin)
        return
    pend = layer._pending_wgrad
    if pend is not None and not (wino and pend[3] == Hin and not ups):
        _flush_wgrad(layer)
        pend = None
    layer._pending_wgrad = None
    with (_on_main if on_main else _on_side)(x, gz, *(pend[:2] if pend is not None else ())):
        if wino:
            ops.conv2d_wgrad_wino(x, gz, layer._gw, layer._gb if bias else None, N, Hin, Hin, layer.c, ups=ups,
                                  second=(pend[0], pend[1], pend[2], False) if pend is not None else None)
            return
        ops.conv2d_wgrad(x, gz, layer._gw, layer._gb if bias else None, N, Hin, Hin, layer.ksize, layer.pad,
                         layer.c, ups=ups)


def _flush_wgrad(layer):
    pend = layer._pending_wgrad
    if pend is None:
        return
    layer._pending_wgrad = None
    x, gz, N, Hin = pend
    with _on_side(x, gz):
        ops.conv2d_wgrad_wino(x, gz, layer._gw, None, N, Hin, Hin, layer.c)


_ONES = {}


def _ones(n, device):
    key = (n, str(device))
    if key not in _ONES:
        _ONES[key] = torch.ones(n, device=device, dtype=torch.float32)
    return _ONES[key]


def generator_forward(G, z, save=False, out=None, pair_out=None):
    wait_pending(G)
    ops.require_gpu()
    G._sync_version()
    z = _check_dev(z, 'latents')
    N, L = z.shape
    if L != G.latent_size or L % 4:
        raise ValueError('latent size %d (expected %d, multiple of 4)' % (L, G.latent_size))
    depth, alpha = int(G.depth), float(G.alpha)
    C = G.num_channels
    b0 = G.block0
    G._ensure_buffers()
    ctx = saved.GContext(N=N, depth=depth, alpha=alpha, recs=[])
    if G.normalize_latents:
        zn, _ = ops.pixelnorm_fwd(z, G.eps)
    else:
        zn = z
    ctx.zn = zn

    def layer(x, lay, H, ups=False):
        if lay.pixelnorm:
            u = _wino(lay, N, H, lay.conv.weight.shape[2]) if lay.ksize == 3 else None
            if u is not None and u.shape[1] <= 32:
                return ops.conv2d_wino_pixelnorm(x, u, lay.conv.bias.data, N, H, H, lay.c, lay.slope, lay.eps, ups=ups)
            if u is not None:
                y = ops.conv2d_wino(x, u, lay.conv.bias.data, N, H, H, lay.c, lay.slope, ups=ups)
                return ops.pixelnorm_fwd(y, lay.eps, inplace=True)
            return ops.conv2d_pixelnorm(x, lay.conv.weight.data, lay.conv.bias.data, N, H, H, lay.ksize, lay.pad, lay.c,
                                        lay.slope, lay.eps, ups=ups)
        return _conv(x, lay, N, H, ups=ups), None

    y1, r1 = layer(zn.view(N, 1, 1, L), b0.c1, 1)
    y2, r2 = layer(y1, b0.c2, 4)
    ctx.y1, ctx.r1, ctx.y2, ctx.r2 = y1, r1, y2, r2
    def to_rgb(h, t, H, out_mul=1.0, prev=None, prev_mul=0.0):
        if pair_out is None:
            return ops.torgb_fwd(h, t.conv.weight.data, t.conv.bias.data, N, C, H, H, t.c, out_mul=out_mul, prev=prev, prev_mul=prev_mul, out=out)
        n2 = N // 2
        return tuple(ops.torgb_fwd(h[a:b], t.conv.weight.data, t.conv.bias.data, n2, C, H, H, t.c, out_mul=out_mul,
                                   prev=prev[a:b] if prev is not None else None, prev_mul=prev_mul, out=o)
                     for (a, b), o in zip(((0, n2), (n2, N)), pair_out))
    if depth == 0:
        img = to_rgb(y2, b0.toRGB, 4)
        return (img, ctx) if save else img
    h, H = y2, 4
    for i in range(depth):
        blk = G.blocks[i]
        H *= 2
        a1, ra1 = layer(h, blk.c1, H, ups=True)
        img = None
        if (i == depth - 1 and alpha >= 1.0 and pair_out is None and blk.c2.pixelnorm and blk.c2.ksize == 3 and a1.is_cuda
                and _wino(blk.c2, N, H, blk.c2.conv.weight.shape[2]) is None):
            t = blk.toRGB
            try:
                a2, ra2, img = ops.conv2d_pixelnorm_torgb(a1, blk.c2.conv.weight.data, blk.c2.conv.bias.data, t.conv.weight.data, t.conv.bias.data,
                                                          N, C, H, H, blk.c2.c, blk.c2.slope, t.c, blk.c2.eps, out=out)
            except ops.Unsupported:
                FALLBACKS['toRGB in the epilogue %dx%d' % (H, H)] += 1
                img = None
        if img is None:
            a2, ra2 = layer(a1, blk.c2, H)
        ctx.recs.append(saved.GBlock(blk=blk, inp=h, a1=a1, r1=ra1, a2=a2, r2=ra2, H=H))
        hprev, h = h, a2
    if img is not None:
        return (img, ctx) if save else img
    t, pt = G.rgb_heads(depth, alpha)
    prev = None
    if pt is not None:
        prev = ops.torgb_fwd(hprev, pt.conv.weight.data, pt.conv.bias.data, N, C, H // 2, H // 2, pt.c)
    img = to_rgb(h, t, H, out_mul=alpha, prev=prev, prev_mul=1.0 - alpha)
    return (img, ctx) if save else img


def generator_backward(G, ctx, g_out):
    wait_pending(G)
    G._ensure_buffers()
    N, depth, alpha = ctx.N, ctx.depth, ctx.alpha
    C = G.num_channels
    b0 = G.block0
    active = [b0.c1, b0.c2]
    g_extra = None
    top_done = False
    t, pt = G.rgb_heads(depth, alpha)
    if depth == 0:
        with _on_side(g_out, ctx.y2):
            ops.torgb_wgrad(g_out, ctx.y2, t._gw, t._gb, N, C, 4, 4, t.c, 1.0)
        g = ops.torgb_bwd_data(g_out, t.conv.weight.data, N, C, 4, 4, t.c)
        active.append(t)
    else:
        rec = ctx.recs[-1]
        H = rec.H
        with _on_side(g_out, rec.a2):
            ops.torgb_wgrad(g_out, rec.a2, t._gw, t._gb, N, C, H, H, alpha * t.c, alpha)
        if rec.r2 is not None:
            g = ops.torgb_bwd_data_pnbwd(g_out, t.conv.weight.data, rec.a2, rec.r2, N, C, H, H, alpha * t.c, rec.blk.c2.slope)
            top_done = True
        else:
            g = ops.torgb_bwd_data(g_out, t.conv.weight.data, N, C, H, H, alpha * t.c)
        active.append(t)
        if pt is not None:
            with _on_side(g_out, rec.inp):
                ops.torgb_wgrad(g_out, rec.inp, pt._gw, pt._gb, N, C, H // 2, H // 2, (1 - alpha) * pt.c,
                                1 - alpha, down=True)
            g_extra = ops.torgb_bwd_data(g_out, pt.conv.weight.data, N, C, H // 2, H // 2, (1 - alpha) * pt.c, down=True)
            active.append(pt)
    _grads_ready(G, active[2:])
    recs = ctx.recs
    for k in range(len(recs) - 1, -1, -1):
        rec = recs[k]
        blk, H = rec.blk, rec.H
        c1, c2 = blk.c1, blk.c2
        if top_done:
            gz2, top_done = g, False
        else:
            gz2 = ops.pixelnorm_lrelu_bwd(g, rec.a2, rec.r2, c2.slope, inplace=True)
        _wgrad(rec.a1, gz2, c2, N, H)
        gz1 = _dgrad_pnbwd(G, gz2, c2, N, H, rec.a1, rec.r1, c1.slope)
        _wgrad(rec.inp, gz1, c1, N, H, ups=True)
        prev = (recs[k - 1].a2, recs[k - 1].r2, recs[k - 1].blk.c2.slope) if k > 0 else (ctx.y2, ctx.r2, b0.c2.slope)
        g, top_done = _dgrad_pool(G, gz1, c1, N, H, other=g_extra, a=4.0, b=1.0, pnb=prev)
        g_extra = None
        active += [c1, c2]
        _grads_ready(G, [c1, c2])
    gz2 = g if top_done else ops.pixelnorm_lrelu_bwd(g, ctx.y2, ctx.r2, b0.c2.slope, inplace=True)
    _wgrad(ctx.y1, gz2, b0.c2, N, 4)
    g1 = _dgrad(G, gz2, b0.c2, N, 4)
    gz1 = ops.pixelnorm_lrelu_bwd(g1, ctx.y1, ctx.r1, b0.c1.slope, inplace=True)
    _wgrad(ctx.zn.view(N, 1, 1, -1), gz1, b0.c1, N, 1)
    _grads_ready(G, [b0.c1, b0.c2])
    return active


def _mbstd_fwd(D, x, groups, cp):
    dp = D._rt.global_stddev
    if dp is None:
        return ops.mbstd_fwd(x, groups, cp)
    if D._rt.gs_checked != (int(x.shape[0]), groups):
        dp.assert_same_on_all_ranks(int(x.shape[0]) // groups, 'exact-global minibatch stddev: the per-rank minibatch size')
        D._rt.gs_checked = (int(x.shape[0]), groups)
    st = ops.mbstd_stats(x, groups)
    return ops.mbstd_write(x, st, dp.all_gather_rows(st), cp)


def _mbstd_tangent(D, x, tx, stats, cp):
    dp = D._rt.global_stddev
    if dp is None:
        return ops.mbstd_tangent(x, tx, stats, cp)
    ts = ops.mbstd_tangent_stats(x, tx, stats)
    return ops.mbstd_tangent_write(tx, ts, dp.all_gather_rows(ts), stats, cp)


def _mbstd_bwd(D, gy, x, stats, cp, apply_mask, mask_slope, tx=None, tstats=None, gy_first=None, out=None):
    dp = D._rt.global_stddev
    if dp is None:
        return ops.mbstd_bwd(gy, x, stats, cp, apply_mask, mask_slope, tx=tx, tstats=tstats, gy_first=gy_first, out=out)
    gs = ops.mbstd_gsum(gy, gy_first if tx is not None else None, stats.shape[0], tuple(x.shape), cp)
    dp.all_reduce_flat(gs.view(-1))
    return ops.mbstd_bwd_global(gy, x, stats, cp, apply_mask, gs, dp.world_size, mask_slope, tx=tx, tstats=tstats, gy_first=gy_first, out=out)


def _mbstd_bwd_hvp(D, g_head, g_mixed, rec, hvp, fr_slope):
    nh, inp, stats, cp = hvp.n_head, rec.inp, rec.stats, rec.blk.c1.cin_store
    gin = torch.empty_like(inp)
    ng = stats.shape[0] - 1
    _mbstd_bwd(D, g_head, inp[:nh], stats[:ng], cp, rec.first, fr_slope, out=gin[:nh])
    _mbstd_bwd(D, g_mixed, inp[nh:], stats[ng:], cp, rec.first, fr_slope, tx=hvp.tx, tstats=hvp.tstats, gy_first=hvp.gy_first, out=gin[nh:])
    return gin


def d_forward(D, x, groups=1, keep_input=True):
    wait_pending(D)
    D._sync_version()
    NB, C, r, _ = x.shape
    depth, alpha = int(D.depth), float(D.alpha)
    if r != 4 * 2 ** depth or C != D.num_channels:
        raise ValueError('input %s does not match depth %d / %d channels' % (tuple(x.shape), depth, D.num_channels))
    nb = len(D.blocks)
    e = nb - 1 - depth
    D._ensure_buffers()
    ctx = saved.DContext(NB=NB, groups=groups, depth=depth, alpha=alpha, x=x, recs=[])
    pn = bool(getattr(D, 'pixelnorm', False))
    fr = D.blocks[e].fromRGB
    sb = USE_SIGN_BYTES and not pn
    curb = None
    fused = None
    if not keep_input and sb and r >= SIGN_BYTES_MIN_H and e < nb - 1 and x.is_cuda:
        c1 = D.blocks[e].c1
        if c1.ksize == 3 and c1.pad == 1 and _wino(c1, NB, r, c1.conv.weight.shape[2]) is None:
            try:
                a1, a1b, curb = ops.conv2d_fromrgb(x, fr.conv.weight.data, fr.conv.bias.data, fr.c, fr.slope, c1.conv.weight.data,
                                                   c1.conv.bias.data, NB, C, r, r, c1.c, c1.slope)
                fused, cur = (a1, a1b), None
            except ops.Unsupported:
                FALLBACKS['fromRGB in the gather %dx%d' % (r, r)] += 1
    if fused is None:
        cur = ops.fromrgb_fwd(x, fr.conv.weight.data, fr.conv.bias.data, NB, C, r, r, fr.c, fr.slope, signs_out=sb and r >= SIGN_BYTES_MIN_H)
        if sb and r >= SIGN_BYTES_MIN_H:
            cur, curb = cur
    H = r
    a2 = None
    for k, j in enumerate(range(e, nb)):
        blk = D.blocks[j]
        last = (j == nb - 1)
        rec = saved.DBlock(blk=blk, inp=cur, H=H, first=(k == 0), last=last, inpb=curb if k == 0 else None)
        if last:
            mb, stats = _mbstd_fwd(D, cur, groups, blk.c1.cin_store)
            a1 = _conv(mb, blk.c1, NB, H)
            if pn:
                a1, rec.r1 = ops.pixelnorm_fwd(a1, inplace=True)
            a2 = _conv(a1, blk.c2, NB, H)
            if pn:
                a2, rec.r2 = ops.pixelnorm_fwd(a2, inplace=True)
            rec.mb, rec.stats, rec.a1, rec.a2 = mb, stats, a1, a2
        else:
            if k == 0 and fused is not None:
                a1, rec.a1b = fused
            elif sb and H >= SIGN_BYTES_MIN_H:
                a1, rec.a1b = _conv(cur, blk.c1, NB, H, signs_out=True)
            else:
                a1 = _conv(cur, blk.c1, NB, H)
            if pn:
                a1, rec.r1 = ops.pixelnorm_fwd(a1, inplace=True)
            pf = None
            if k == 0 and alpha < 1.0:
                nfr = D.blocks[j + 1].fromRGB
                pf = rec.pf = ops.fromrgb_fwd(x, nfr.conv.weight.data, nfr.conv.bias.data, NB, C, H // 2, H // 2,
                                              nfr.c, nfr.slope, pool=True)
            pa, pb = (alpha, 1.0 - alpha) if pf is not None else (1.0, 0.0)
            if pn:
                a2 = _conv(a1, blk.c2, NB, H)
                a2, rec.r2 = ops.pixelnorm_fwd(a2, inplace=True)
                cur = ops.avgpool2_fwd(a2, pf, pa, pb)
            else:
                a2, cur = _conv_pool(a1, blk.c2, NB, H, other=pf, a=pa, b=pb, y_bytes=USE_SIGN_BYTES and H >= SIGN_BYTES_MIN_H)
            rec.a1, rec.a2 = a1, a2
            H //= 2
        ctx.recs.append(rec)
    s = ops.linear1_fwd(a2, D.linear.weight.data, D.linear.bias.data)
    return s, ctx


class _DForwardBuffers(object):

    def __init__(self):
        self.arena = ops.Arena()
        self.x3 = None
        self.g_out = None
        self.key = None
        self.owner = None


class _ArenaUse(object):
    __slots__ = ('consumed', '__weakref__')

    def __init__(self):
        self.consumed = False


def _arena_free(st):
    tok = st.owner() if st.owner is not None else None
    return tok is None or tok.consumed


def _lazy_unpool_ok(rec, save_adjoints):
    if not (USE_LAZY_UNPOOL and not save_adjoints and rec.H % 32 == 0 and rec.a2.dtype == torch.uint8):
        return False
    c2 = rec.blk.c2
    w = c2.conv.weight.shape
    return w[3] == 8 and w[2] in (8, 16) and c2.ksize == 3


def _consume(D, hand, rec, n, full):
    c2, H = rec.blk.c2, rec.H
    a1 = saved.Sign.a1(rec, n if rec.last else None)

    def lazy(up, _):
        if up is not hand.up.bytes:
            return ops.avgpool2_bwd(hand.coarse, up, 4.0 * hand.mul, hand.up.slope), None
        gz1 = ops.conv2d_unpooled(hand.coarse, _wt(D, c2), up, hand.mul, hand.up.slope, n, H, H, c2.c,
                                  mask=a1.bytes if a1.bytes is not None else a1.f32, mask_slope=a1.slope)
        if full:
            _flush_wgrad(c2)
            with _on_side(a1.f32, hand.coarse, up):
                ops.conv2d_wgrad_unpooled(a1.f32, hand.coarse, up, hand.mul, hand.up.slope, c2._gw, c2._gb, n, H, H, c2.c)
        return None, gz1
    gz2, gz1 = (hand.g, None) if hand.g is not None else _bytes_first(lazy, hand.up, lambda: 'lazy unpool %dx%d' % (H, H))
    if gz1 is None:
        if full:
            _wgrad(a1.f32, gz2, c2, n, H)
        gz1 = _dgrad(D, gz2, c2, n, 1 if rec.last else H, a1)
    return gz2, gz1


_NO_INJECTION = saved.PNInjection()


def _pn_bwd(gy, y, r, slope, nh, inj):
    if inj is None:
        return ops.pixelnorm_lrelu_bwd(gy, y, r, slope, inplace=True)
    per = r.numel() // y.shape[0]
    if nh > 0:
        ops.pixelnorm_lrelu_bwd(gy[:nh], y[:nh], r[:nh * per], slope, inplace=True)
    ops.pixelnorm_lrelu_bwd(gy[nh:], y[nh:], r[nh * per:], slope, inj=inj, out=gy[nh:])
    return gy


def _pn_head_seed(D, gscore, a2, nh):
    g = ops.linear1_bwd_data(gscore, D.linear.weight.data, None, (nh,) + tuple(a2.shape[1:]))
    if nh < a2.shape[0]:
        gtop, g = g, torch.empty_like(a2)
        ops.zero_(g[nh:])
        ops.axpby_mask(gtop, a=1.0, out=g[:nh])
    return g


def _pn_adjoints(D, hand, rec, n, nh, full, adj, inj):
    c1, c2, H = rec.blk.c1, rec.blk.c2, rec.H
    if adj is not None:
        adj.gy2 = ops.axpby_mask(hand.g, a=1.0)
    gz2 = _pn_bwd(hand.g, rec.a2, rec.r2, c2.slope, nh, inj.inj2)
    if full:
        _wgrad(rec.a1, gz2, c2, n, H)
    gy1 = _dgrad(D, gz2, c2, n, 1 if rec.last else H)
    if adj is not None:
        adj.gy1 = ops.axpby_mask(gy1, a=1.0)
    return gz2, _pn_bwd(gy1, rec.a1, rec.r1, c1.slope, nh, inj.inj1)


def _fade_in(D, ctx, rec, prev, gin, full, adj):
    pfr = rec.blk.fromRGB
    x, H = ctx.x, rec.H
    gpf = ops.axpby_mask(gin, mask=prev.pf, a=1.0 - ctx.alpha, mask_slope=pfr.slope)
    if adj is not None:
        adj.gpf = gpf
    if full:
        with _on_side(gpf, x):
            ops.fromrgb_wgrad(gpf, x, pfr._gw, pfr._gb, ctx.NB, D.num_channels, H, H, pfr.c, pool=True)
    return gpf, pfr


def _hand_over(D, ctx, rec, prev, gz1, gin, full, adj, pn):
    c1, H, NB = rec.blk.c1, rec.H, ctx.NB
    fade = prev.first and ctx.alpha < 1.0
    mul = ctx.alpha if fade else 1.0
    up = None if pn else saved.Sign.a2(prev)
    lazy = not pn and (gin is None or fade) and _lazy_unpool_ok(prev, adj is not None)
    if gin is None and not (fade or lazy or pn):
        return saved.PoolAdjoint(g=_dgrad_unpool(D, gz1, c1, NB, H, up, 1.0)), None
    if gin is None:
        gin = _dgrad(D, gz1, c1, NB, H)
    if lazy:
        hand = saved.PoolAdjoint(coarse=gin, up=up, mul=0.25 * mul)
    elif pn:
        hand = saved.PoolAdjoint(g=ops.avgpool2_bwd(gin, None, mul))
    else:
        hand = saved.PoolAdjoint(g=ops.avgpool2_bwd(gin, _f32(up), mul, up.slope))
    return hand, (_fade_in(D, ctx, rec, prev, gin, full, adj) if fade else None)


def _entry(D, ctx, rec, gz1, gin, full, want_gimg, adj, faded, tail, pn):
    blk, H, NB, x, C = rec.blk, rec.H, ctx.NB, ctx.x, D.num_channels
    c1, fr = blk.c1, blk.fromRGB
    gimg = None
    fused = fw_fused = False
    fw = full and D._rt.grad_hook is None
    if (not pn and gin is None and (want_gimg or fw) and rec.inpb is not None and x.is_cuda and c1.ksize == 3 and c1.pad == 1
            and _wino(c1, NB, H, c1.conv.weight.shape[3], transposed=True) is None):
        try:
            gin, gimg = ops.conv2d_masked_fromrgb_bwd(gz1, _wt(D, c1), rec.inpb, fr.slope, fr.conv.weight.data, fr.c, NB, C, H, H, c1.c,
                                                      keep_gf=adj is not None or (full and not fw), want_gimg=want_gimg,
                                                      img=x if fw else None, rgb_dw=fr._gw if fw else None, rgb_db=fr._gb if fw else None)
            fused, fw_fused = True, fw
        except ops.Unsupported:
            FALLBACKS['fromRGB adjoint in the epilogue %dx%d' % (H, H)] += 1
    if gin is None and not fused:
        gin = _dgrad(D, gz1, c1, NB, H, saved.Sign.inp(rec))
    if adj is not None:
        adj.gf = gin
    if full and not fw_fused:
        with (_on_main if tail >= 1 else _on_side)(gin, x):
            ops.fromrgb_wgrad(gin, x, fr._gw, fr._gb, NB, C, H, H, fr.c)
    if not want_gimg:
        return None
    if not fused:
        gimg = torch.empty_like(x)
        ops.fromrgb_bwd_data(gin, fr.conv.weight.data, gimg, NB, C, H, H, fr.c)
    if faded is not None:
        gpf, pfr = faded
        ops.fromrgb_bwd_data(gpf, pfr.conv.weight.data, gimg, NB, C, H // 2, H // 2, pfr.c, pool=True, accumulate=True)
    return gimg


def d_backward(D, ctx, gscore, full, want_gimg, save_adjoints=False, hvp=None):
    wait_pending(D)
    D._ensure_buffers()
    pn = bool(getattr(D, 'pixelnorm', False))
    NB, alpha, recs = ctx.NB, ctx.alpha, ctx.recs
    adj = [saved.DAdjoint() for _ in recs] if save_adjoints else [None] * len(recs)
    nh = NB if hvp is None else hvp.n_head
    injs = hvp.injs if pn and hvp is not None else None
    n4 = NB if pn else nh
    a2 = recs[-1].a2
    tail = _tail_wgrad_on_main(recs[0].H) if (full and not pn and ASYNC_WGRAD and D._rt.grad_hook is None and len(recs) > 1) else 0
    if full and not pn:
        ops.linear1_wgrad(gscore, a2[:nh], D._lin_gw, D._lin_gb)
    hand = saved.PoolAdjoint(g=_pn_head_seed(D, gscore, a2, nh) if pn else ops.linear1_bwd_data(
        gscore, D.linear.weight.data, a2[:nh], (nh,) + tuple(a2.shape[1:]), recs[-1].blk.c2.slope))
    if full and pn:
        ops.linear1_wgrad(gscore, a2[:nh], D._lin_gw, D._lin_gb)
    gimg = faded = None
    for idx in range(len(recs) - 1, -1, -1):
        rec = recs[idx]
        c1, H = rec.blk.c1, rec.H
        n = n4 if rec.last else NB
        if pn:
            gz2, gz1 = _pn_adjoints(D, hand, rec, n, nh, full, adj[idx], injs[idx] if injs is not None else _NO_INJECTION)
        else:
            gz2, gz1 = _consume(D, hand, rec, n, full)
        if full:
            _wgrad(rec.mb[:n] if rec.last else rec.inp, gz1, c1, n, H, on_main=rec.first and not rec.last and tail >= 2)
        gin = None
        if rec.last:
            gmb = _dgrad(D, gz1, c1, n, H)
            if hvp is None:
                gin = _mbstd_bwd(D, gmb, rec.inp, rec.stats, c1.cin_store, rec.first, rec.blk.fromRGB.slope)
            else:
                gin = _mbstd_bwd_hvp(D, gmb[:nh], gmb[nh:] if pn else None, rec, hvp, rec.blk.fromRGB.slope)
        if save_adjoints:
            adj[idx].gz2, adj[idx].gz1 = gz2, gz1
            if rec.last:
                adj[idx].gmb = gmb
        if rec.first:
            gimg = _entry(D, ctx, rec, gz1, gin, full, want_gimg, adj[idx], faded, tail, pn)
        else:
            hand, faded = _hand_over(D, ctx, rec, recs[idx - 1], gz1, gin, full, adj[idx - 1], pn)
        if full:
            _grads_ready(D, _d_block_done(D, recs, idx, alpha))
    return gimg, (adj if save_adjoints else None)


def _d_block_done(D, recs, idx, alpha):
    rec = recs[idx]
    blk = rec.blk
    done = [blk.c1, blk.c2]
    if rec.last:
        done.append(D._lin_layer)
    if rec.first or (recs[idx - 1].first and alpha < 1.0):
        done.append(blk.fromRGB)
    return done


def d_tangent_wgrad(D, sub, adj, u):
    wait_pending(D)
    D._ensure_buffers()
    N, alpha = sub.NB, sub.alpha
    C = D.num_channels
    recs = sub.recs
    rec0 = recs[0]
    fr = rec0.blk.fromRGB
    H = rec0.H
    with _on_side(adj[0].gf, u):
        ops.fromrgb_wgrad(adj[0].gf, u, fr._gw, None, N, C, H, H, fr.c)
    cur = _bytes_first(lambda m, _: ops.fromrgb_fwd(u, fr.conv.weight.data, None, N, C, H, H, fr.c, 1.0, mask=m, mask_slope=fr.slope),
                       saved.Sign.inp(rec0), None, count=False)
    hvp = None
    t2 = None
    pn = bool(getattr(D, 'pixelnorm', False))
    injs = [saved.PNInjection() for _ in recs] if pn else None
    for idx, rec in enumerate(recs):
        blk, H = rec.blk, rec.H
        c1, c2 = blk.c1, blk.c2
        if rec.last:
            tmb, tstats = _mbstd_tangent(D, rec.inp, cur, rec.stats, c1.cin_store)
            hvp = saved.Hvp(tx=cur, tstats=tstats, gy_first=adj[idx].gmb, injs=injs)
            _wgrad(tmb, adj[idx].gz1, c1, N, H, bias=False, defer=True)
            t1 = _conv(tmb, c1, N, H, mask=saved.Sign.a1(rec), bias=False)
            if pn:
                t1, injs[idx].inj1 = ops.pixelnorm_tangent(t1, rec.a1, rec.r1, adj[idx].gy1)
            _wgrad(t1, adj[idx].gz2, c2, N, H, bias=False, defer=True)
            t2 = _conv(t1, c2, N, H, mask=saved.Sign.a2(rec), bias=False)
            if pn:
                t2, injs[idx].inj2 = ops.pixelnorm_tangent(t2, rec.a2, rec.r2, adj[idx].gy2)
        else:
            _wgrad(cur, adj[idx].gz1, c1, N, H, bias=False, defer=True)
            t1 = _conv(cur, c1, N, H, mask=saved.Sign.a1(rec), bias=False)
            if pn:
                t1, injs[idx].inj1 = ops.pixelnorm_tangent(t1, rec.a1, rec.r1, adj[idx].gy1)
            _wgrad(t1, adj[idx].gz2, c2, N, H, bias=False, defer=True)
            tpf = None
            if rec.first and alpha < 1.0:
                nfr = recs[idx + 1].blk.fromRGB
                with _on_side(adj[idx].gpf, u):
                    ops.fromrgb_wgrad(adj[idx].gpf, u, nfr._gw, None, N, C, H // 2, H // 2, nfr.c, pool=True)
                tpf = ops.fromrgb_fwd(u, nfr.conv.weight.data, None, N, C, H // 2, H // 2, nfr.c, 1.0,
                                      pool=True, mask=rec.pf, mask_slope=nfr.slope)
            pa, pb = (alpha, 1.0 - alpha) if tpf is not None else (1.0, 0.0)
            if pn:
                t2 = _conv(t1, c2, N, H, mask=saved.Sign.a2(rec), bias=False)
                t2, injs[idx].inj2 = ops.pixelnorm_tangent(t2, rec.a2, rec.r2, adj[idx].gy2)
                cur = ops.avgpool2_fwd(t2, tpf, pa, pb)
            else:
                t2, cur = _conv_pool(t1, c2, N, H, bias=False, mask=saved.Sign.a2(rec), other=tpf, a=pa, b=pb, pool_only=True)
    ops.linear1_wgrad(_ones(N, u.device), t2, D._lin_gw, None)
    return hvp


def d_active_params(D, depth, alpha):
    nb = len(D.blocks)
    e = nb - 1 - depth
    layers = [D.blocks[e].fromRGB]
    if depth > 0 and alpha < 1.0:
        layers.append(D.blocks[e + 1].fromRGB)
    for j in range(e, nb):
        layers += [D.blocks[j].c1, D.blocks[j].c2]
    return layers


def d_exchange_layers(D, depth, alpha):
    D._ensure_buffers()
    return d_active_params(D, depth, alpha) + [D._lin_layer]


def g_exchange_layers(G, depth, alpha):
    G._ensure_buffers()
    return [lay for _, lay in G.stage_convs(depth)] + [t for t in G.rgb_heads(depth, alpha) if t is not None]


def discriminator_forward(D, x):
    ops.require_gpu()
    x = _check_dev(x, 'D input')
    s, _ = d_forward(D, x, 1)
    return s.view(-1, 1)


def _assign_grads(net, layers, linear=False):
    for m in layers:
        m.conv.weight.grad = m._gw
        m.conv.bias.grad = m._gb
    if linear:
        net.linear.weight.grad = net._lin_gw
        net.linear.bias.grad = net._lin_gb


REAL_THIRD_IN_STEP = True


class Objective(_collections.namedtuple('Objective', 'kind drift penalty weight target family augment', defaults=('pinned', None))):
    __slots__ = ()


WGAN_GP = Objective('wgan', 0.001, 'gp', 10.0, 1.0, 'original')


def _d_loss_block(obj, s, pen, N):
    if obj.family == 'original':
        return ops.d_loss(s, pen, N, obj.drift)
    return ops.gan_d_loss(s, pen, N, obj.kind, obj.drift)


def _g_loss_block(obj, s):
    return ops.g_loss(s) if obj.family == 'original' else ops.gan_g_loss(s, obj.kind)


def _penalty_seed(obj, gimg, ss, N):
    if obj.penalty == 'r1':
        return ops.r1_seed(gimg, ss, obj.weight, 1.0 / N)
    return ops.gp_seed(gimg, ss, obj.weight, obj.target, 1.0 / N)


def _augmented(aug, x, table, out=None):
    return ops.augment_apply(x, table, aug.channel_mask, out=out)


def _step_table(objective, table, rows):
    if objective.augment is None:
        if table is not None:
            raise ValueError('an augmentation table for an objective without an Augmenter')
        return None
    if table is None or tuple(table.shape) != (rows, ops.AUGMENT_COLS):
        raise ValueError('an objective with an Augmenter needs a table of %d rows (got %s)' % (rows, None if table is None else tuple(table.shape)))
    return table


def _count_real_signs(aug, s, N):
    if aug is not None and aug.controller is not None:
        ops.score_signs(s[:N], aug.acc)


def d_loss_forward(D, G, real, latents, mix, objective, table=None):
    if objective.penalty is None:
        return _d_plain_loss_forward(D, G, real, latents, objective, table)
    ops.require_gpu()
    real = _check_dev(real, 'real images')
    latents = _check_dev(latents, 'latents')
    mix = _check_dev(mix, 'mixing factors').view(-1)
    N = real.shape[0]
    aug, table = objective.augment, _step_table(objective, table, 2 * real.shape[0])
    D._sync_version()
    fake_done = None
    arena_st = None
    if (REAL_THIRD_IN_STEP and float(D.alpha) >= 1.0 and not getattr(D, 'pixelnorm', False) and ASYNC_WGRAD and real.is_cuda
            and hasattr(ops, 'Arena') and D._rt.global_stddev is None
            and _three_pass_buffers(D, real) is not None):
        st = arena_st = D._rt.d_fwd_buffers
        x3 = st.x3
        main = torch.cuda.current_stream(torch._C._cuda_getDevice())
        side = _side_stream()
        wait_pending(D)
        step_start = torch.cuda.Event()
        _record_event(step_start, main)
        probe('D.start')
        if aug is None:
            d_step_generator(D, G, latents, x3[N:2 * N])
        else:
            if st.g_out is None:
                st.g_out = torch.empty_like(x3[:N])
            d_step_generator(D, G, latents, st.g_out)
            _augmented(aug, st.g_out, table[N:], out=x3[N:2 * N])
        probe('D.g_fwd_end')
        with torch.cuda.stream(side):
            _wait_event(side, step_start)
            probe('D.side_start')
            if aug is None:
                ops.axpby_mask(real, a=1.0, out=x3[:N])
            else:
                _augmented(aug, real, table[:N], out=x3[:N])
            real_copied = torch.cuda.Event()
            _record_event(real_copied, side)
            with st.arena.pass_(0):
                s_r, ctx_r = d_forward(D, x3[:N], groups=1)
            probe('D.real_end')
        real.record_stream(side)
        if aug is not None:
            table.record_stream(side)
        _wait_stream(side, main)
        with torch.cuda.stream(side):
            probe('D.fake_start')
            with st.arena.pass_(2):
# ... 227 lines not shown
```

pggan-pytorch_amd/ops.py:

```python
import os as _os

import ctypes

import torch

from . import _lib

_C = _lib.CONSTANTS


def _stream():
    return torch._C._cuda_getCurrentRawStream(torch._C._cuda_getDevice())


WORKSPACE_BYTES = int(_os.environ.get('PGGAN_WORKSPACE_MB', '32')) << 20
_workspaces = {}
_capture_workspace = {}
_no_workspace_streams = set()


def workspace_bytes(kind, N, H, W, cin, cout):
    n = ctypes.c_size_t(0)
    _lib.call('pg_workspace_bytes', kind, N, H, W, cin, cout, ctypes.addressof(n))
    return int(n.value)
# ... 143 lines not shown
    if u is None:
        u = torch.empty((16, cout, cin), device=w.device, dtype=torch.float32)
    _lib.call('pg_wino_transform_weights', _p(w), _p(u), cout, cin, _stream())
    return u


def wino_transform_weights_batched(flat_w, flat_u, layers, transposed=False):
    n = len(layers)
    if n == 0:
        return
    woff = (ctypes.c_int64 * n)(*[l[0] for l in layers])
    uoff = (ctypes.c_int64 * n)(*[l[1] for l in layers])
    co = (ctypes.c_int * n)(*[l[2] for l in layers])
    ci = (ctypes.c_int * n)(*[l[3] for l in layers])
    if isinstance(transposed, (list, tuple)):
        tr = (ctypes.c_int * n)(*[1 if t else 0 for t in transposed]) if any(transposed) else None
    else:
        tr = (ctypes.c_int * n)(*([1] * n)) if transposed else None
    _lib.call('pg_wino_transform_weights_batched', _p(flat_w), _p(flat_u), n, ctypes.cast(woff, ctypes.c_void_p),
              ctypes.cast(uoff, ctypes.c_void_p), ctypes.cast(co, ctypes.c_void_p), ctypes.cast(ci, ctypes.c_void_p),
              ctypes.cast(tr, ctypes.c_void_p) if tr is not None else None, _stream())


def signbytes_to_mask(b):
    m = torch.empty(tuple(b.shape[:-1]) + (4 * b.shape[-1],), device=b.device, dtype=torch.float32)
    _lib.call('pg_signbytes_to_mask', _p(b), _p(m), b.numel(), _stream())
    return m


def conv2d_wino(x, u, bias, N, H, W, scale, slope=1.0, mask=None, mask_slope=0.2, ups=False, out=None,
                pool=False, other=None, a=1.0, b=0.0, pool_only=False, unpool=False, upmask=None, up_mul=1.0, y_bytes=False,
                signs_out=False):
    cout, cin = u.shape[1], u.shape[2]
    flags = (FLAG_UPSAMPLE if ups else 0) | (FLAG_MASK_BYTES if _is_bytes(mask) or _is_bytes(upmask) else 0) | (FLAG_Y_BYTES if y_bytes else 0)
    if y_bytes:
        y = _empty((N, H, W, cout // 4), device=x.device, dtype=torch.uint8)
    else:
        y = out if out is not None else _empty((N, H, W, cout), device=x.device, dtype=torch.float32)
    yp = _empty((N, H // 2, W // 2, cout), device=x.device, dtype=torch.float32) if pool else None
    yu = _empty((N, 2 * H, 2 * W, cout), device=x.device, dtype=torch.float32) if unpool else None
    sb = None
    if signs_out:
        sb = _empty((N, H, W, cout // 4), device=x.device, dtype=torch.uint8)
        mask, flags = sb, flags | FLAG_SIGNS_OUT
    _lib.call('pg_conv2d_wino_nhwc', _p(x), _p(u), _p(bias), _p(mask), _p(y), _p(yp), _p(other), a, b, 1 if pool_only else 0,
              _p(yu), _p(upmask), up_mul, N, H, W, cin, cout, flags, scale, slope, mask_slope, _stream_with_workspace())
    if signs_out:
        return y, sb
    if pool:
        return y, yp
    if unpool:
        return yu
    return y


def conv2d_wino_pixelnorm(x, u, bias, N, H, W, scale, slope, eps=1e-8, ups=False):
    cout, cin = u.shape[1], u.shape[2]
    y = torch.empty((N, H, W, cout), device=x.device, dtype=torch.float32)
    r = torch.empty((N * H * W,), device=x.device, dtype=torch.float32)
    _lib.call('pg_conv2d_wino_pixelnorm_nhwc', _p(x), _p(u), _p(bias), _p(y), _p(r), N, H, W, cin, cout, 1 if ups else 0,
              scale, slope, eps, _stream())
    return y, r


def conv2d_wino_pnbwd(x, u, ysaved, r, N, H, W, scale, slope, pool=False, other=None, a=1.0, b=0.0):
    cout, cin = u.shape[1], u.shape[2]
    y = torch.empty((N, H // 2, W // 2, cout) if pool else (N, H, W, cout), device=x.device, dtype=torch.float32)
    _lib.call('pg_conv2d_wino_pnbwd_nhwc', _p(x), _p(u), _p(ysaved), _p(r), _p(y), 1 if pool else 0, _p(other), a, b,
              N, H, W, cin, cout, scale, slope, _stream())
    return y


def conv2d_pool(x, w, bias, N, Hin, Win, ks, pad, scale, slope=1.0, mask=None, mask_slope=0.2, other=None, a=1.0, b=0.0,
                pool_only=False, y_bytes=False):
    cout, cin = w.shape[2], w.shape[3]
    ho, wo = Hin + 2 * pad - ks + 1, Win + 2 * pad - ks + 1
    flags = (FLAG_MASK_BYTES if _is_bytes(mask) else 0) | (FLAG_Y_BYTES if y_bytes else 0)
    if y_bytes:
        y = _empty((N, ho, wo, cout // 4), device=x.device, dtype=torch.uint8)
    else:
        y = _empty((N, ho, wo, cout), device=x.device, dtype=torch.float32)
    yp = _empty((N, ho // 2, wo // 2, cout), device=x.device, dtype=torch.float32)
    _lib.call('pg_conv2d_pool_nhwc', _p(x), _p(w), _p(bias), _p(mask), _p(y), _p(yp), _p(other), a, b, 1 if pool_only else 0,
              N, Hin, Win, cin, cout, ks, pad, flags, scale, slope, mask_slope, _stream())
    return y, yp


def conv2d_pixelnorm(x, w, bias, N, Hin, Win, ks, pad, scale, slope, eps=1e-8, ups=False):
    cout, cin = w.shape[2], w.shape[3]
    ho, wo = Hin + 2 * pad - ks + 1, Win + 2 * pad - ks + 1
    y = torch.empty((N, ho, wo, cout), device=x.device, dtype=torch.float32)
    r = torch.empty((N * ho * wo,), device=x.device, dtype=torch.float32)
    _lib.call('pg_conv2d_pixelnorm_nhwc', _p(x), _p(w), _p(bias), _p(y), _p(r), N, Hin, Win, cin, cout, ks, pad,
              1 if ups else 0, scale, slope, eps, _stream())
    return y, r


def conv2d_pixelnorm_torgb(x, w, bias, t_w, t_b, N, C, H, W, scale, slope, t_scale, eps=1e-8, out=None):
    cout, cin = w.shape[2], w.shape[3]
    y = torch.empty((N, H, W, cout), device=x.device, dtype=torch.float32)
    r = torch.empty((N * H * W,), device=x.device, dtype=torch.float32)
    if out is None:
        out = torch.empty((N, C, H, W), device=x.device, dtype=torch.float32)
    _lib.call('pg_conv2d_pixelnorm_torgb_nhwc', _p(x), _p(w), _p(bias), _p(y), _p(r), _p(t_w), _p(t_b), t_scale, _p(out),
              N, C, H, W, cin, cout, scale, slope, eps, _stream())
    return y, r, out


def conv2d_pnbwd(x, w, ysaved, r, N, Hin, Win, ks, pad, scale, slope):
    cout, cin = w.shape[2], w.shape[3]
    ho, wo = Hin + 2 * pad - ks + 1, Win + 2 * pad - ks + 1
    y = torch.empty((N, ho, wo, cout), device=x.device, dtype=torch.float32)
    _lib.call('pg_conv2d_pnbwd_nhwc', _p(x), _p(w), _p(ysaved), _p(r), _p(y), N, Hin, Win, cin, cout, ks, pad, scale, slope, _stream())
    return y


def conv2d_unpool(x, w, N, Hin, Win, ks, pad, scale, upmask=None, mul=1.0, mask_slope=0.2):
    cout, cin = w.shape[2], w.shape[3]
    ho, wo = Hin + 2 * pad - ks + 1, Win + 2 * pad - ks + 1
    y = torch.empty((N, ho, wo, cout), device=x.device, dtype=torch.float32)
    yup = torch.empty((N, 2 * ho, 2 * wo, cout), device=x.device, dtype=torch.float32)
    _lib.call('pg_conv2d_unpool_nhwc', _p(x), _p(w), _p(upmask), _p(y), _p(yup), N, Hin, Win, cin, cout, ks, pad,
              FLAG_MASK_BYTES if _is_bytes(upmask) else 0, scale, mul, mask_slope, _stream())
    return yup


def conv2d_unpooled(g, w, gbytes, gmul, gslope, N, Hin, Win, scale, mask=None, mask_slope=0.2):
    cout, cin = w.shape[2], w.shape[3]
    y = torch.empty((N, Hin, Win, cout), device=g.device, dtype=torch.float32)
    _lib.call('pg_conv2d_unpooled_nhwc', _p(g), _p(w), _p(gbytes), gmul, gslope, _p(mask), _p(y), N, Hin, Win, cin, cout,
              FLAG_MASK_BYTES if _is_bytes(mask) else 0, scale, mask_slope, _stream())
    return y


def conv2d_fromrgb(img, rgb_w, rgb_b, rgb_scale, rgb_slope, w, bias, N, C, H, W, scale, slope, signs_out=True):
    cout, cmid = w.shape[2], w.shape[3]
    y = _empty((N, H, W, cout), device=img.device, dtype=torch.float32)
    yb = _empty((N, H, W, cout // 4), device=img.device, dtype=torch.uint8) if signs_out else None
    xb = _empty((N, H, W, cmid // 4), device=img.device, dtype=torch.uint8)
    _lib.call('pg_conv2d_fromrgb_nhwc', _p(img), _p(rgb_w), _p(rgb_b), rgb_scale, rgb_slope, _p(xb), _p(w), _p(bias), _p(y), _p(yb),
              N, C, H, W, cmid, cout, scale, slope, _stream())
    return y, yb, xb


def conv2d_masked_fromrgb_bwd(gz, wt, mask_bytes, mask_slope, rgb_w, rgb_scale, N, C, H, W, scale, keep_gf=True, gimg=None, want_gimg=True,
                              img=None, rgb_dw=None, rgb_db=None):
    cout, cin = wt.shape[2], wt.shape[3]
    gf = _empty((N, H, W, cout), device=gz.device, dtype=torch.float32) if keep_gf else None
    if gimg is None and want_gimg:
        gimg = torch.empty((N, C, H, W), device=gz.device, dtype=torch.float32)
    _lib.call('pg_conv2d_masked_fromrgb_bwd_nhwc', _p(gz), _p(wt), _p(mask_bytes), mask_slope, _p(gf), _p(rgb_w), rgb_scale, _p(gimg),
              _p(img), _p(rgb_dw), _p(rgb_db), N, C, H, W, cin, cout, scale, _stream())
    return gf, gimg



def conv2d_wgrad_unpooled(x, g, gbytes, gmul, gslope, dw, db, N, Hin, Win, scale):
    cout, cin = dw.shape[2], dw.shape[3]
    _lib.call('pg_conv2d_wgrad_unpooled_nhwc', _p(x), _p(g), _p(gbytes), gmul, gslope, _p(dw), _p(db), N, Hin, Win, cin, cout,
              scale, _stream())


def conv2d_wgrad(x, gz, dw, db, N, Hin, Win, ks, pad, scale, ups=False):
    cout, cin = dw.shape[2], dw.shape[3]
    _lib.call('pg_conv2d_wgrad_nhwc', _p(x), _p(gz), _p(dw), _p(db), N, Hin, Win, cin, cout, ks, pad,
              1 if ups else 0, scale, _stream())


def conv2d_wgrad_wino(x, gz, dw, db, N, H, W, scale, ups=False, second=None):
    cout, cin = dw.shape[2], dw.shape[3]
    if second is None:
        _lib.call('pg_conv2d_wgrad_wino_nhwc', _p(x), _p(gz), _p(dw), _p(db), N, H, W, cin, cout, 1 if ups else 0, scale, _stream())
        return
    x2, gz2, n2, bias2 = second
    _lib.call('pg_conv2d_wgrad_wino2_nhwc', _p(x), _p(gz), N, _p(x2), _p(gz2), n2, _p(dw), _p(db),
              (1 if db is not None else 0) | (2 if (bias2 and db is not None) else 0), H, W, cin, cout, 1 if ups else 0, scale, _stream())


def pack_dgrad_weights(w, wt):
    ks, _, cout, cin = w.shape
    _lib.call('pg_pack_dgrad_weights', _p(w), _p(wt), ks, cout, cin, _stream())
    return wt


def pack_dgrad_weights_batched(flat_w, flat_wt, layers):
    n = len(layers)
    off = (ctypes.c_int64 * n)(*[l[0] for l in layers])
    ks = (ctypes.c_int * n)(*[l[1] for l in layers])
    co = (ctypes.c_int * n)(*[l[2] for l in layers])
    ci = (ctypes.c_int * n)(*[l[3] for l in layers])
    _lib.call('pg_pack_dgrad_weights_batched', _p(flat_w), _p(flat_wt), n, ctypes.cast(off, ctypes.c_void_p),
              ctypes.cast(ks, ctypes.c_void_p), ctypes.cast(co, ctypes.c_void_p), ctypes.cast(ci, ctypes.c_void_p), _stream())


def fromrgb_fwd(img, w, bias, N, C, H, W, scale, slope, pool=False, mask=None, mask_slope=0.2, signs_out=False):
    cout = w.shape[0]
    y = _empty((N, H, W, cout), device=img.device, dtype=torch.float32)
    flags = (1 if pool else 0) | (FLAG_MASK_BYTES if _is_bytes(mask) else 0)
    sb = None
    if signs_out:
        sb = _empty((N, H, W, cout // 4), device=img.device, dtype=torch.uint8)
        mask, flags = sb, flags | FLAG_SIGNS_OUT
    _lib.call('pg_fromrgb_fwd', _p(img), _p(w), _p(bias), _p(mask), _p(y), N, C, H, W, cout, flags,
              scale, slope, mask_slope, _stream())
    return (y, sb) if signs_out else y


def fromrgb_bwd_data(gz, w, gimg, N, C, H, W, scale, pool=False, accumulate=False):
    cout = w.shape[0]
    _lib.call('pg_fromrgb_bwd_data', _p(gz), _p(w), _p(gimg), N, C, H, W, cout, 1 if pool else 0,
              1 if accumulate else 0, scale, _stream())


def fromrgb_wgrad(gz, img, dw, db, N, C, H, W, scale, pool=False):
    cout = dw.shape[0]
    _lib.call('pg_fromrgb_wgrad', _p(gz), _p(img), _p(dw), _p(db), N, C, H, W, cout, 1 if pool else 0, scale, _stream())


def torgb_fwd(x, w, bias, N, C, H, W, scale, out_mul=1.0, prev=None, prev_mul=0.0, out=None):
    cin = w.shape[1]
    if out is None:
        out = torch.empty((N, C, H, W), device=x.device, dtype=torch.float32)
    _lib.call('pg_torgb_fwd', _p(x), _p(w), _p(bias), _p(prev), _p(out), N, C, H, W, cin, scale, out_mul, prev_mul, _stream())
    return out


def torgb_bwd_data(g, w, N, C, H, W, mul_scale, down=False):
    cin = w.shape[1]
    gx = torch.empty((N, H, W, cin), device=g.device, dtype=torch.float32)
    _lib.call('pg_torgb_bwd_data', _p(g), _p(w), _p(gx), N, C, H, W, cin, 1 if down else 0, mul_scale, _stream())
    return gx


def torgb_bwd_data_pnbwd(g, w, ysaved, r, N, C, H, W, mul_scale, slope):
    cin = w.shape[1]
    gx = torch.empty((N, H, W, cin), device=g.device, dtype=torch.float32)
    try:
        _lib.call('pg_torgb_bwd_data_pnbwd', _p(g), _p(w), _p(ysaved), _p(r), _p(gx), N, C, H, W, cin, mul_scale, slope, _stream())
        return gx
    except Unsupported:
        return pixelnorm_lrelu_bwd(torgb_bwd_data(g, w, N, C, H, W, mul_scale), ysaved, r, slope, inplace=True)


def torgb_wgrad(g, x, dw, db, N, C, H, W, mul_scale, mul, down=False):
    cin = dw.shape[1]
    _lib.call('pg_torgb_wgrad', _p(g), _p(x), _p(dw), _p(db), N, C, H, W, cin, 1 if down else 0, mul_scale, mul, _stream())


def avgpool2_fwd(x, other=None, a=1.0, b=0.0):
    N, H2, W2, C = x.shape
    y = torch.empty((N, H2 // 2, W2 // 2, C), device=x.device, dtype=torch.float32)
    _lib.call('pg_avgpool2_fwd', _p(x), _p(other), _p(y), N, H2 // 2, W2 // 2, C, a, b, _stream())
    return y


def avgpool2_bwd(gy, mask=None, mul=1.0, mask_slope=0.2):
    N, H, W, C = gy.shape
    gx = torch.empty((N, 2 * H, 2 * W, C), device=gy.device, dtype=torch.float32)
    _lib.call('pg_avgpool2_bwd', _p(gy), _p(mask), _p(gx), N, H, W, C, mul, mask_slope, _stream())
    return gx


def upsample2_bwd(g):
    N, H2, W2, C = g.shape
    gx = torch.empty((N, H2 // 2, W2 // 2, C), device=g.device, dtype=torch.float32)
    _lib.call('pg_upsample2_bwd', _p(g), _p(gx), N, H2 // 2, W2 // 2, C, _stream())
    return gx


def axpby_mask(x, other=None, mask=None, a=1.0, b=0.0, mask_slope=0.2, out=None):
    y = out if out is not None else torch.empty_like(x)
    _lib.call('pg_axpby_mask', _p(x), _p(other), _p(mask), _p(y), x.numel(), a, b, mask_slope, _stream())
    return y


def pixelnorm_fwd(x, eps=1e-8, inplace=False):
    C = x.shape[-1]
    P = x.numel() // C
    y = x if inplace else torch.empty_like(x)
    r = torch.empty((P,), device=x.device, dtype=torch.float32)
    _lib.call('pg_pixelnorm_fwd', _p(x), _p(y), _p(r), P, C, eps, _stream())
    return y, r


def pixelnorm_lrelu_bwd(gy, y, r, slope, inplace=False, inj=None, out=None):
    C = y.shape[-1]
    P = y.numel() // C
    gz = out if out is not None else (gy if inplace else torch.empty_like(gy))
    if inj is None:
        _lib.call('pg_pixelnorm_lrelu_bwd', _p(gy), _p(y), _p(r), _p(gz), P, C, slope, _stream())
    else:
        _lib.call('pg_pixelnorm_lrelu_bwd_inj', _p(gy), _p(y), _p(r), _p(inj), _p(gz), P, C, slope, _stream())
    return gz


def pixelnorm_tangent(t, y, r, a):
    C = y.shape[-1]
    P = y.numel() // C
    ty, inj = torch.empty_like(t), torch.empty_like(t)
    _lib.call('pg_pixelnorm_tangent', _p(t), _p(y), _p(r), _p(a), _p(ty), _p(inj), P, C, _stream())
    return ty, inj


MBSTD_STATS_STRIDE = _C['PG_MBSTD_STATS_STRIDE']


# ... 1111 lines not shown
```

Measured before the change: 300.1 images/sec.

## Fuse fromRGB into entry-layer wgrad and tangent conv for 1024 D step

Adds kernels that recompute the 1x1 fromRGB activation on the fly inside the entry-layer 3x3 weight-gradient and tangent (GP double-backward) convolutions. The full-resolution 8-channel fromRGB activation therefore no longer has to be stored and reloaded in the D step. The D forward now keeps the input lazily by default when alpha is 1, and the fused wgrad can be placed on the main stream. This trades extra per-tile arithmetic and register pressure for less HBM traffic at 1024x1024, and it adds new code paths gated by environment flags.

```diff
diff --git a/include/pggan_hip_fromrgb.h b/include/pggan_hip_fromrgb.h
--- /dev/null
+++ b/include/pggan_hip_fromrgb.h
@@ -0,0 +1,24 @@
+#ifndef PGGAN_HIP_FROMRGB_H
+#define PGGAN_HIP_FROMRGB_H
+
+#include "pggan_hip.h"
+
+#ifdef __cplusplus
+extern "C" {
+#endif
+
+int pg_conv2d_wgrad_fromrgb_nhwc(const float* img, const float* rgb_w, const float* rgb_b, float rgb_scale, float rgb_slope,
+                                 const float* gz, float* dw, float* db,
+                                 int N, int C, int H, int W, int Cmid, int Cout, float scale, pg_stream_t stream);
+int pg_conv2d_fromrgb_tangent_nhwc(const float* v, const float* rgb_w, float rgb_scale, const unsigned char* x_signs, float rgb_slope,
+                                   const float* w, const unsigned char* mask_bytes, float mask_slope, float* y,
+                                   int N, int C, int H, int W, int Cmid, int Cout, float scale, pg_stream_t stream);
+int pg_conv2d_wgrad_fromrgb_tangent_nhwc(const float* v, const float* rgb_w, float rgb_scale, const unsigned char* x_signs,
+                                         float rgb_slope, const float* gz, float* dw,
+                                         int N, int C, int H, int W, int Cmid, int Cout, float scale, pg_stream_t stream);
+
+#ifdef __cplusplus
+}
+#endif
+
+#endif
diff --git a/pggan-pytorch_amd/_lib.py b/pggan-pytorch_amd/_lib.py
--- a/pggan-pytorch_amd/_lib.py
+++ b/pggan-pytorch_amd/_lib.py
@@ -121,6 +121,8 @@
 _RESTYPE_OF.update(_augment_restypes)
 EMBED_SIGNATURES, _embed_restypes, EMBED_CONSTANTS = _read_header('pggan_hip_embed.h')
 _RESTYPE_OF.update(_embed_restypes)
+FROMRGB_SIGNATURES, _fromrgb_restypes, _ = _read_header('pggan_hip_fromrgb.h')
+_RESTYPE_OF.update(_fromrgb_restypes)
 ABI_VERSION = CONSTANTS['PG_ABI_VERSION']
 
 _lib = None
@@ -142,7 +144,8 @@
                            + list(GAN_SIGNATURES.items()) + list(PHASE_SIGNATURES.items()) + list(SAMPLING_SIGNATURES.items())
                            + list(PROJECTION_SIGNATURES.items()) + list(CROP_SIGNATURES.items()) + list(SWD_SIGNATURES.items())
                            + list(MEL_SIGNATURES.items()) + list(RESAMPLE_SIGNATURES.items()) + list(SHIFT_SIGNATURES.items())
-                           + list(PRD_SIGNATURES.items()) + list(AUGMENT_SIGNATURES.items()) + list(EMBED_SIGNATURES.items())):
+                           + list(PRD_SIGNATURES.items()) + list(AUGMENT_SIGNATURES.items()) + list(EMBED_SIGNATURES.items())
+                           + list(FROMRGB_SIGNATURES.items())):
         try:
             fn = getattr(lib, name)
         except AttributeError:
diff --git a/pggan-pytorch_amd/csrc/conv_api.hip b/pggan-pytorch_amd/csrc/conv_api.hip
--- a/pggan-pytorch_amd/csrc/conv_api.hip
+++ b/pggan-pytorch_amd/csrc/conv_api.hip
@@ -1,4 +1,5 @@
 #include "convp.h"
+#include "pggan_hip_fromrgb.h"
 
 __thread char pgk::g_last_kernel[96] = "";
 __thread int pgk::g_tune[4] = {-1, -1, -1, -1};
@@ -210,6 +211,15 @@
                                           scale, slope, (hipStream_t)stream);
 }
 
+extern "C" int pg_conv2d_fromrgb_tangent_nhwc(const float* v, const float* rgb_w, float rgb_scale, const unsigned char* x_signs, float rgb_slope,
+                                              const float* w, const unsigned char* mask_bytes, float mask_slope, float* y,
+                                              int N, int C, int H, int W, int Cmid, int Cout, float scale, pg_stream_t stream)
+{
+    if (!v || !rgb_w || !x_signs || !w || !mask_bytes || !y || N <= 0 || C <= 0 || H <= 0 || W <= 0 || Cmid <= 0 || Cout <= 0) return PG_E_ARG;
+    return pgk::launch_conv_strip_fromrgb_tangent(v, rgb_w, rgb_scale, x_signs, rgb_slope, w, mask_bytes, mask_slope, y, N, C, H, W, Cmid, Cout,
+                                                  scale, (hipStream_t)stream);
+}
+
 extern "C" int pg_conv2d_pixelnorm_torgb_nhwc(const float* x, const float* w, const float* bias, float* y, float* r,
                                               const float* t_w, const float* t_b, float t_scale, float* img,
                                               int N, int C, int H, int W, int Cin, int Cout, float scale, float slope, float eps,
diff --git a/pggan-pytorch_amd/csrc/conv_strip.hip b/pggan-pytorch_amd/csrc/conv_strip.hip
--- a/pggan-pytorch_amd/csrc/conv_strip.hip
+++ b/pggan-pytorch_amd/csrc/conv_strip.hip
@@ -113,10 +113,10 @@
     float4 gxr[NG];
     unsigned gbr[NG];
     __amdgpu_buffer_rsrc_t rgx = pg_make_rsrc(p.x + (size_t)n * ximg, (unsigned)(ximg * 4)), rgb = rgx;
-    constexpr int NR = GM == 2 ? NG : 1;
+    constexpr int NR = GM >= 2 ? NG : 1;
     int rrow[NR];
     float rw[NR][4][RGB_MAXC], rb[NR][4], rpx[NR][RGB_MAXC];
-    if constexpr (GM == 2) {
+    if constexpr (GM >= 2) {
         rgx = pg_make_rsrc(p.x + (size_t)n * npix * p.rgbC, npix * (unsigned)p.rgbC * 4u);
         rgb = pg_make_rsrc(p.xsigns + (size_t)n * npix * C4, npix * C4);
 #pragma unroll
@@ -129,14 +129,15 @@
             rrow[i] = ok ? r0 - 1 + m : -(1 << 28);
             cvo[i] = ok ? 4u * (unsigned)((r0 - 1 + m) * p.W + col) : PG_OOB;
             cvs[i] = ok ? 4u * (unsigned)(RB * p.W) : 0u;
-            bvo[i] = (ok && px >= 1 && px <= SW) ? (unsigned)((r0 - 1 + m) * p.W + col) * C4 + q : PG_OOB;
-            bvs[i] = (ok && px >= 1 && px <= SW) ? (unsigned)(RB * p.W * C4) : 0u;
+            const bool bok = ok && (GM == 3 || (px >= 1 && px <= SW));
+            bvo[i] = bok ? (unsigned)((r0 - 1 + m) * p.W + col) * C4 + q : PG_OOB;
+            bvs[i] = bok ? (unsigned)(RB * p.W * C4) : 0u;
             const int qq = sl < B::USED ? q : 0;
 #pragma unroll
             for (int k = 0; k < 4; ++k) {
 #pragma unroll
                 for (int c = 0; c < RGB_MAXC; ++c) rw[i][k][c] = c < p.rgbC ? p.rgb_w[(4 * qq + k) * p.rgbC + c] : 0.f;
-                rb[i][k] = p.rgb_b ? p.rgb_b[4 * qq + k] : 0.f;
+                rb[i][k] = (GM == 2 && p.rgb_b) ? p.rgb_b[4 * qq + k] : 0.f;
             }
         }
     }
@@ -156,7 +157,7 @@
         }
     }
     auto gather_load = [&]() {
-        if constexpr (GM == 2) {
+        if constexpr (GM >= 2) {
 #pragma unroll
             for (int i = 0; i < NG; ++i) {
                 const bool in = (unsigned)rrow[i] < (unsigned)p.H;
@@ -164,6 +165,10 @@
                 for (int c = 0; c < RGB_MAXC; ++c)
                     rpx[i][c] = c < p.rgbC ? __uint_as_float(__builtin_amdgcn_raw_buffer_load_b32(rgx, in ? (int)(cvo[i] + (unsigned)c * npix * 4u) : (int)PG_OOB, 0, 0)) : 0.f;
                 cvo[i] += cvs[i];
+                if constexpr (GM == 3) {
+                    gbr[i] = __builtin_amdgcn_raw_buffer_load_b8(rgb, in ? (int)bvo[i] : (int)PG_OOB, 0, 0);
+                    bvo[i] += bvs[i];
+                }
             }
             return;
         }
@@ -175,25 +180,35 @@
         }
     };
     auto gather_store = [&](int pos) {
-        if constexpr (GM == 2) {
+        if constexpr (GM >= 2) {
 #pragma unroll
             for (int i = 0; i < NG; ++i) {
                 const int sl = i * 256 + tid;
                 const bool in = (unsigned)rrow[i] < (unsigned)p.H;
                 float o[4];
+                float4 f = make_float4(1.f, 1.f, 1.f, 1.f);
+                if constexpr (GM == 3) f = pg_sign_factors((unsigned char)gbr[i], p.rgb_slope);
+                const float f4[4] = {f.x, f.y, f.z, f.w};
 #pragma unroll
                 for (int k = 0; k < 4; ++k) {
+#pragma clang fp contract(off)
                     float a = 0.f;
 #pragma unroll
                     for (int c = 0; c < RGB_MAXC; ++c) if (c < p.rgbC) a = fmaf(rpx[i][c], rw[i][k][c], a);
-                    const float v = __fadd_rn(__fmul_rn(a, p.rgb_scale), rb[i][k]);
-                    o[k] = in ? (v > 0.f ? v : v * p.rgb_slope) : 0.f;
+                    const float sa = a * p.rgb_scale;
+                    if constexpr (GM == 3) o[k] = in ? sa * f4[k] : 0.f;
+                    else {
+                        const float v = sa + rb[i][k];
+                        o[k] = in ? (v > 0.f ? v : v * p.rgb_slope) : 0.f;
+                    }
                 }
                 const float4 v4 = make_float4(o[0], o[1], o[2], o[3]);
                 if (sl < B::SLOTS) *reinterpret_cast<float4*>(lds + (pos * B::SLOTS + sl) * 4) = (cvs[i] ? v4 : make_float4(0.f, 0.f, 0.f, 0.f));
-                if (p.xsigns && in && rrow[i] >= r0 && rrow[i] < r0 + p.seg_rows && bvs[i])
-                    __builtin_amdgcn_raw_buffer_store_b8(pg_sign_byte(v4), rgb, (int)bvo[i], 0, 0);
-                bvo[i] += bvs[i];
+                if constexpr (GM == 2) {
+                    if (p.xsigns && in && rrow[i] >= r0 && rrow[i] < r0 + p.seg_rows && bvs[i])
+                        __builtin_amdgcn_raw_buffer_store_b8(pg_sign_byte(v4), rgb, (int)bvo[i], 0, 0);
+                    bvo[i] += bvs[i];
+                }
                 rrow[i] += RB;
             }
             return;
@@ -528,10 +543,10 @@
     conv_strip_body<8, 8, EPI, WREG, 0, XM>(p);
 }
 
-template <int EPI>
+template <int EPI, int GM = 2>
 __global__ __launch_bounds__(256, 2) void conv_strip_rgb_kernel(SArgs p)
 {
-    conv_strip_body<8, 8, EPI, false, 2>(p);
+    conv_strip_body<8, 8, EPI, false, GM>(p);
 }
 
 template <int COUT, int CIN, int EPI, bool WREG, bool GATH = false>
@@ -570,10 +585,11 @@
 }
 
 struct WArgs { const float* x; const float* gz; float* dw; float* db; float scale; int H, W, ups, strips, segs, seg_rows;
-               const unsigned char* gbytes; float gmul, gslope; };
-
-template <int CO, int CI, bool GATH>
-__global__ __launch_bounds__(256, 2) void wgrad_strip_kernel(WArgs p)
+               const unsigned char* gbytes; float gmul, gslope;
+               const float* rgb_w; const float* rgb_b; float rgb_scale, rgb_slope; int rgbC; const unsigned char* xsigns; };
+
+template <int CO, int CI, bool GATH, int XM>
+__device__ __forceinline__ void wgrad_strip_body(const WArgs& p)
 {
     constexpr int TAPS = 9;
     constexpr int QO = CO / 4, QI = CI / 4, NB = QO * QI, PPM = 16 / NB, RNG = SW / PPM;
@@ -660,6 +676,77 @@
         asm volatile("s_mov_b32 %0, m0\n\ts_mov_b32 m0, %3\n\ts_nop 0\n\tbuffer_load_dwordx4 %1, %2, 0 offen lds\n\ts_mov_b32 m0, %0"
                      : "=&s"(keep) : "v"(vo), "s"(rs), "s"(dst) : "memory");
     };
+    constexpr int NXP = XM ? (RB * XRS + 255) / 256 : 1;
+    unsigned ivo[NXP], ivs[NXP], ibo[NXP];
+    int irow[NXP];
+    float ipx[NXP][RGB_MAXC];
+    unsigned ibr[NXP];
+    float rw[XM ? CI : 1][RGB_MAXC], rb[XM ? CI : 1];
+    const unsigned npix = (unsigned)(p.H * p.W);
+    __amdgpu_buffer_rsrc_t rimg = rgc, rxb = rgc;
+    if constexpr (XM != 0) {
+        static_assert(XM == 0 || (CI == 8 && !GATH), "fromRGB feeds the 8-channel entry layer");
+        rimg = pg_make_rsrc(p.x + (size_t)n * npix * p.rgbC, npix * (unsigned)p.rgbC * 4u);
+        if constexpr (XM == 2) rxb = pg_make_rsrc(p.xsigns + (size_t)n * npix * QI, npix * QI);
+#pragma unroll
+        for (int i = 0; i < NXP; ++i) {
+            const int idx = i * 256 + tid;
+            const int m = idx / XRS, e = idx - m * XRS, u = e / PPM, s = e - u * PPM;
+            const int col = ow0 + RNG * s + u - 1;
+            const bool ok = idx < RB * XRS && (unsigned)col < (unsigned)p.W;
+            irow[i] = ok ? r0 - 1 + m : -(1 << 28);
+            ivo[i] = ok ? 4u * (unsigned)((r0 - 1 + m) * p.W + col) : PG_OOB;
+            ivs[i] = ok ? 4u * (unsigned)(RB * p.W) : 0u;
+            ibo[i] = ok ? (unsigned)((r0 - 1 + m) * p.W + col) * QI : PG_OOB;
+        }
+#pragma unroll
+        for (int k = 0; k < CI; ++k) {
+#pragma unroll
+            for (int c = 0; c < RGB_MAXC; ++c) rw[k][c] = c < p.rgbC ? p.rgb_w[k * p.rgbC + c] : 0.f;
+            rb[k] = (XM == 1 && p.rgb_b) ? p.rgb_b[k] : 0.f;
+        }
+    }
+    auto xload = [&]() {
+#pragma unroll
+        for (int i = 0; i < NXP; ++i) {
+            const bool in = (unsigned)irow[i] < (unsigned)p.H;
+#pragma unroll
+            for (int c = 0; c < RGB_MAXC; ++c)
+                ipx[i][c] = c < p.rgbC ? __uint_as_float(__builtin_amdgcn_raw_buffer_load_b32(rimg, in ? (int)(ivo[i] + (unsigned)c * npix * 4u) : (int)PG_OOB, 0, 0)) : 0.f;
+            if constexpr (XM == 2) ibr[i] = __builtin_amdgcn_raw_buffer_load_b16(rxb, in ? (int)ibo[i] : (int)PG_OOB, 0, 0);
+            ivo[i] += ivs[i]; ibo[i] += ivs[i] ? (unsigned)(RB * p.W * QI) : 0u;
+        }
+    };
+    auto xstore = [&](int pos) {
+#pragma unroll
+        for (int i = 0; i < NXP; ++i) {
+            const int idx = i * 256 + tid;
+            const bool in = (unsigned)irow[i] < (unsigned)p.H;
+            irow[i] += RB;
+            if (idx >= RB * XRS) continue;
+#pragma unroll
+            for (int q = 0; q < QI; ++q) {
+                float o[4];
+                float4 f = make_float4(1.f, 1.f, 1.f, 1.f);
+                if constexpr (XM == 2) f = pg_sign_factors((unsigned char)(ibr[i] >> (8 * q)), p.rgb_slope);
+                const float f4[4] = {f.x, f.y, f.z, f.w};
+#pragma unroll
+                for (int k = 0; k < 4; ++k) {
+#pragma clang fp contract(off)
+                    float a = 0.f;
+#pragma unroll
+                    for (int c = 0; c < RGB_MAXC; ++c) if (c < p.rgbC) a = fmaf(ipx[i][c], rw[4 * q + k][c], a);
+                    const float sa = a * p.rgb_scale;
+                    if constexpr (XM == 2) o[k] = in ? sa * f4[k] : 0.f;
+                    else {
+                        const float v = sa + rb[4 * q + k];
+                        o[k] = in ? (v > 0.f ? v : v * p.rgb_slope) : 0.f;
+                    }
+                }
+                *reinterpret_cast<float4*>(lds + ((q * XPS + pos * XBS) + idx) * 4) = make_float4(o[0], o[1], o[2], o[3]);
+            }
+        }
+    };
     auto issue_x = [&](int pos) {
 #pragma unroll
         for (int i = 0; i < XNI; ++i) {
@@ -674,9 +761,16 @@
             gvoff[i] += 4u * grow;
         }
     };
-    issue_x(0);
-    if constexpr (GATH) { gather_load(); gather_store(0); } else issue_g(0);
-    issue_x(1);
+    if constexpr (XM != 0) {
+        xload();
+        issue_g(0);
+        xstore(0);
+        xload(); xstore(1);
+    } else {
+        issue_x(0);
+        if constexpr (GATH) { gather_load(); gather_store(0); } else issue_g(0);
+        issue_x(1);
+    }
 
     f32x4 acc[TAPS];
 #pragma unroll
@@ -689,7 +783,8 @@
     for (int it = 0; it < niter; ++it) {
         asm volatile("s_waitcnt vmcnt(0)" ::: "memory");
         __syncthreads();
-        if (it + 2 <= niter) issue_x((it + 2) % XRING);
+        if constexpr (XM != 0) { if (it + 2 <= niter) xload(); }
+        else if (it + 2 <= niter) issue_x((it + 2) % XRING);
         if constexpr (GATH) { if (it + 1 < niter) gather_load(); }
         else if (it + 1 < niter) issue_g((it + 1) % GRING);
         __builtin_amdgcn_sched_barrier(0);
@@ -720,6 +815,7 @@
                     acc[dy * 3 + dx] = __builtin_amdgcn_mfma_f32_4x4x1f32(a, bcol[dy][(ks + dx) % 3], acc[dy * 3 + dx], 0, 0, 0);
         }
         if constexpr (GATH) { if (it + 1 < niter) gather_store((it + 1) % GRING); }
+        if constexpr (XM != 0) { if (it + 2 <= niter) xstore((it + 2) % XRING); }
     }
 
 #pragma unroll
@@ -758,6 +854,18 @@
     }
 }
 
+template <int CO, int CI, bool GATH>
+__global__ __launch_bounds__(256, 2) void wgrad_strip_kernel(WArgs p)
+{
+    wgrad_strip_body<CO, CI, GATH, 0>(p);
+}
+
+template <int XM>
+__global__ __launch_bounds__(256, 2) void wgrad_strip_rgb_kernel(WArgs p)
+{
+    wgrad_strip_body<8, 8, false, XM>(p);
+}
+
 template <int CO, int CI, bool GATH = false>
 int launch_wgrad_strip_t(const WArgs& a, int N, hipStream_t s)
 {
@@ -770,10 +878,30 @@
     return (int)hipGetLastError();
 }
 
+template <int XM>
+int launch_wgrad_strip_rgb_t(const WArgs& a, int N, hipStream_t s)
+{
+    const size_t smem = ((size_t)2 * (3 * 320 + 2) + (size_t)2 * (2 * RB * SW + 2)) * 16;
+    auto kern = wgrad_strip_rgb_kernel<XM>;
+    if (int rc = set_smem(kern, smem, SMEM_ANY)) return rc;
+    snprintf(g_last_kernel, sizeof(g_last_kernel), "wgrad_strip_rgb_kernel<%d>", XM);
+    hipLaunchKernelGGL(kern, dim3((unsigned)(N * a.strips * a.segs)), dim3(256), smem, s, a);
+    return (int)hipGetLastError();
+}
+
 int strip_seg_rows(int N, int H, int W)
 {
     int seg = 64;
     while (seg > 16 && ((long long)N * (W / SW) * (H / seg) < 768 || (H % seg))) seg >>= 1;
+    return (seg < 16 || (seg % RB) || (H % seg)) ? 0 : seg;
+}
+
+int wgrad_seg_rows(int N, int H, int W)
+{
+    int seg = 256;
+    auto tasks = [&](int sg) { return (long long)N * (W / SW) * (H / sg); };
+    while (seg > 64 && (seg > H || (H % seg) || tasks(seg) < 1024)) seg >>= 1;
+    while (seg > 16 && (seg > H || (H % seg) || tasks(seg) < 512)) seg >>= 1;
     return (seg < 16 || (seg % RB) || (H % seg)) ? 0 : seg;
 }
 
@@ -879,12 +1007,9 @@
     if ((p.Wout % SW) || (p.Hout % 16)) return PG_E_UNSUP;
     if (!((p.Cout == 8 && p.Cin == 8) || (p.Cout == 16 && p.Cin == 8) || (p.Cout == 8 && p.Cin == 16))) return PG_E_UNSUP;
     if ((long long)p.Hin * p.Win * 16 * 4 >= (1ll << 31)) return PG_E_UNSUP;
-    int seg = 256;
-    auto tasks = [&](int sg) { return (long long)p.N * (p.Wout / SW) * (p.Hout / sg); };
-    while (seg > 64 && (seg > p.Hout || (p.Hout % seg) || tasks(seg) < 1024)) seg >>= 1;
-    while (seg > 16 && (seg > p.Hout || (p.Hout % seg) || tasks(seg) < 512)) seg >>= 1;
-    if (seg < 16 || (seg % RB) || (p.Hout % seg)) return PG_E_UNSUP;
-    WArgs a;
+    const int seg = wgrad_seg_rows(p.N, p.Hout, p.Wout);
+    if (!seg) return PG_E_UNSUP;
+    WArgs a{};
     a.x = p.x; a.gz = p.gz; a.dw = p.dw; a.db = p.db; a.scale = p.scale;
     a.H = p.Hout; a.W = p.Wout; a.ups = p.ups; a.strips = p.Wout / SW; a.segs = p.Hout / seg; a.seg_rows = seg;
     a.gbytes = p.gbytes; a.gmul = p.gmul; a.gslope = p.gslope;
@@ -897,3 +1022,40 @@
     if (p.Cout == 16 && p.Cin == 8) return launch_wgrad_strip_t<16, 8>(a, p.N, s);
     return launch_wgrad_strip_t<8, 16>(a, p.N, s);
 }
+
+int pgk::launch_wgrad_strip_fromrgb(const float* img, const float* rgb_w, const float* rgb_b, float rgb_scale, float rgb_slope,
+                                    const unsigned char* x_signs, const float* gz, float* dw, float* db,
+                                    int N, int C, int H, int W, int Cmid, int Cout, float scale, hipStream_t s)
+{
+    if (C < 1 || C > RGB_MAXC || Cmid != 8 || Cout != 8 || (W % SW) || (H % 16)) return PG_E_UNSUP;
+    if ((long long)H * W * 16 * 4 >= (1ll << 31)) return PG_E_UNSUP;
+    const int seg = wgrad_seg_rows(N, H, W);
+    if (!seg) return PG_E_UNSUP;
+    WArgs a{};
+    a.x = img; a.gz = gz; a.dw = dw; a.db = db; a.scale = scale;
+    a.H = H; a.W = W; a.strips = W / SW; a.segs = H / seg; a.seg_rows = seg;
+    a.rgb_w = rgb_w; a.rgb_b = rgb_b; a.rgb_scale = rgb_scale; a.rgb_slope = rgb_slope; a.rgbC = C; a.xsigns = x_signs;
+    if (x_signs) return launch_wgrad_strip_rgb_t<2>(a, N, s);
+    return launch_wgrad_strip_rgb_t<1>(a, N, s);
+}
+
+int pgk::launch_conv_strip_fromrgb_tangent(const float* v, const float* rgb_w, float rgb_scale, const unsigned char* x_signs, float rgb_slope,
+                                           const float* w, const unsigned char* mask_bytes, float mask_slope, float* y,
+                                           int N, int C, int H, int W, int Cmid, int Cout, float scale, hipStream_t s)
+{
+    if (C < 1 || C > RGB_MAXC || Cmid != 8 || Cout != 8 || (W % SW) || (H % 16)) return PG_E_UNSUP;
+    if ((long long)H * W * 16 * 4 >= (1ll << 31)) return PG_E_UNSUP;
+    const int seg = strip_seg_rows(N, H, W);
+    if (!seg) return PG_E_UNSUP;
+    SArgs a{};
+    a.x = v; a.w = w; a.mask = mask_bytes; a.mask_bytes = 1; a.y = y;
+    a.scale = scale; a.slope = 1.f; a.mask_slope = mask_slope; a.pool_a = 1.f;
+    a.H = H; a.W = W; a.strips = W / SW; a.segs = H / seg; a.seg_rows = seg;
+    a.rgb_w = rgb_w; a.rgb_scale = rgb_scale; a.rgb_slope = rgb_slope; a.rgbC = C; a.xsigns = const_cast<unsigned char*>(x_signs);
+    const size_t smem = (size_t)NBLK * Blk<8>::SLOTS * 16 + (size_t)9 * 8 * 8 * 4;
+    auto kern = conv_strip_rgb_kernel<EPI_MASK, 3>;
+    if (int rc = set_smem(kern, smem, SMEM_ANY)) return rc;
+    snprintf(g_last_kernel, sizeof(g_last_kernel), "conv_strip_rgb_kernel<%d, 3>", (int)EPI_MASK);
+    hipLaunchKernelGGL(kern, dim3((unsigned)(N * a.strips * a.segs)), dim3(256), smem, s, a);
+    return (int)hipGetLastError();
+}
diff --git a/pggan-pytorch_amd/csrc/conv_wgrad.hip b/pggan-pytorch_amd/csrc/conv_wgrad.hip
--- a/pggan-pytorch_amd/csrc/conv_wgrad.hip
+++ b/pggan-pytorch_amd/csrc/conv_wgrad.hip
@@ -1,4 +1,5 @@
 #include "convp.h"
+#include "pggan_hip_fromrgb.h"
 
 namespace {
 
@@ -609,6 +610,24 @@
     return launch_wgrad_thin<64>(p, (hipStream_t)stream);
 }
 
+extern "C" int pg_conv2d_wgrad_fromrgb_nhwc(const float* img, const float* rgb_w, const float* rgb_b, float rgb_scale, float rgb_slope,
+                                            const float* gz, float* dw, float* db,
+                                            int N, int C, int H, int W, int Cmid, int Cout, float scale, pg_stream_t stream)
+{
+    if (!img || !rgb_w || !gz || !dw || N <= 0 || C <= 0 || H <= 0 || W <= 0 || Cmid <= 0 || Cout <= 0) return PG_E_ARG;
+    return launch_wgrad_strip_fromrgb(img, rgb_w, rgb_b, rgb_scale, rgb_slope, nullptr, gz, dw, db, N, C, H, W, Cmid, Cout, scale,
+                                      (hipStream_t)stream);
+}
+
+extern "C" int pg_conv2d_wgrad_fromrgb_tangent_nhwc(const float* v, const float* rgb_w, float rgb_scale, const unsigned char* x_signs,
+                                                    float rgb_slope, const float* gz, float* dw,
+                                                    int N, int C, int H, int W, int Cmid, int Cout, float scale, pg_stream_t stream)
+{
+    if (!v || !rgb_w || !x_signs || !gz || !dw || N <= 0 || C <= 0 || H <= 0 || W <= 0 || Cmid <= 0 || Cout <= 0) return PG_E_ARG;
+    return launch_wgrad_strip_fromrgb(v, rgb_w, nullptr, rgb_scale, rgb_slope, x_signs, gz, dw, nullptr, N, C, H, W, Cmid, Cout, scale,
+                                      (hipStream_t)stream);
+}
+
 #ifdef PG_WINO_TRACE
 extern "C" int pg_debug_wgrad_trace(void* buf) { g_wgrad_trace = (unsigned long long*)buf; return 0; }
 #endif
diff --git a/pggan-pytorch_amd/csrc/convp.h b/pggan-pytorch_amd/csrc/convp.h
--- a/pggan-pytorch_amd/csrc/convp.h
+++ b/pggan-pytorch_amd/csrc/convp.h
@@ -158,5 +158,11 @@
 int launch_conv_strip_fromrgb(const float* img, const float* rgb_w, const float* rgb_b, float rgb_scale, float rgb_slope,
                               unsigned char* x_signs, const float* w, const float* bias, float* y, unsigned char* y_signs,
                               int N, int C, int H, int W, int Cmid, int Cout, float scale, float slope, hipStream_t s);
+int launch_conv_strip_fromrgb_tangent(const float* v, const float* rgb_w, float rgb_scale, const unsigned char* x_signs, float rgb_slope,
+                                      const float* w, const unsigned char* mask_bytes, float mask_slope, float* y,
+                                      int N, int C, int H, int W, int Cmid, int Cout, float scale, hipStream_t s);
+int launch_wgrad_strip_fromrgb(const float* img, const float* rgb_w, const float* rgb_b, float rgb_scale, float rgb_slope,
+                               const unsigned char* x_signs, const float* gz, float* dw, float* db,
+                               int N, int C, int H, int W, int Cmid, int Cout, float scale, hipStream_t s);
 
 }
diff --git a/pggan-pytorch_amd/engine.py b/pggan-pytorch_amd/engine.py
--- a/pggan-pytorch_amd/engine.py
+++ b/pggan-pytorch_amd/engine.py
@@ -392,8 +392,11 @@
             and min(layer._gw.shape[2], layer._gw.shape[3]) >= _WINO_WGRAD_MIN_CHANNELS)
 
 
+_TAIL_1024 = int(os.environ.get('PGGAN_TAIL_WGRAD_ON_MAIN', '2'))
+
+
 def _tail_wgrad_on_main(H):
-    return 2 if H >= 1024 else 1 if H >= 512 else 0
+    return _TAIL_1024 if H >= 1024 else 1 if H >= 512 else 0
 
 
 def _on_main(*tensors):
@@ -608,6 +611,9 @@
     return gin
 
 
+FUSE_FROMRGB_DSTEP = os.environ.get('PGGAN_FUSE_FROMRGB_DSTEP', '1') != '0'
+
+
 def d_forward(D, x, groups=1, keep_input=True):
     wait_pending(D)
     D._sync_version()
@@ -624,7 +630,8 @@
     sb = USE_SIGN_BYTES and not pn
     curb = None
     fused = None
-    if not keep_input and sb and r >= SIGN_BYTES_MIN_H and e < nb - 1 and x.is_cuda:
+    lazy_input = not keep_input or (FUSE_FROMRGB_DSTEP and alpha >= 1.0 and D._rt.grad_hook is None)
+    if lazy_input and sb and r >= SIGN_BYTES_MIN_H and e < nb - 1 and x.is_cuda:
         c1 = D.blocks[e].c1
         if c1.ksize == 3 and c1.pad == 1 and _wino(c1, NB, r, c1.conv.weight.shape[2]) is None:
             try:
@@ -710,7 +717,7 @@
     return w[3] == 8 and w[2] in (8, 16) and c2.ksize == 3
 
 
-def _consume(D, hand, rec, n, full):
+def _consume(D, hand, rec, n, full, on_main=False):
     c2, H = rec.blk.c2, rec.H
     a1 = saved.Sign.a1(rec, n if rec.last else None)
 
@@ -721,13 +728,13 @@
                                   mask=a1.bytes if a1.bytes is not None else a1.f32, mask_slope=a1.slope)
         if full:
             _flush_wgrad(c2)
-            with _on_side(a1.f32, hand.coarse, up):
+            with (_on_main if on_main else _on_side)(a1.f32, hand.coarse, up):
                 ops.conv2d_wgrad_unpooled(a1.f32, hand.coarse, up, hand.mul, hand.up.slope, c2._gw, c2._gb, n, H, H, c2.c)
         return None, gz1
     gz2, gz1 = (hand.g, None) if hand.g is not None else _bytes_first(lazy, hand.up, lambda: 'lazy unpool %dx%d' % (H, H))
     if gz1 is None:
         if full:
-            _wgrad(a1.f32, gz2, c2, n, H)
+            _wgrad(a1.f32, gz2, c2, n, H, on_main=on_main)
         gz1 = _dgrad(D, gz2, c2, n, 1 if rec.last else H, a1)
     return gz2, gz1
 
@@ -856,8 +863,14 @@
         if pn:
             gz2, gz1 = _pn_adjoints(D, hand, rec, n, nh, full, adj[idx], injs[idx] if injs is not None else _NO_INJECTION)
         else:
-            gz2, gz1 = _consume(D, hand, rec, n, full)
-        if full:
+            gz2, gz1 = _consume(D, hand, rec, n, full, on_main=rec.first and not rec.last and tail >= 3)
+        if full and rec.first and not rec.last and rec.inp is None:
+            fr = rec.blk.fromRGB
+            _flush_wgrad(c1)
+            with (_on_main if tail >= 2 else _on_side)(ctx.x, gz1):
+                ops.conv2d_wgrad_fromrgb(ctx.x, fr.conv.weight.data, fr.conv.bias.data, fr.c, fr.slope, gz1, c1._gw, c1._gb,
+                                         n, D.num_channels, H, H, c1.c)
+        elif full:
             _wgrad(rec.mb[:n] if rec.last else rec.inp, gz1, c1, n, H, on_main=rec.first and not rec.last and tail >= 2)
         gin = None
         if rec.last:
@@ -899,10 +912,20 @@
     rec0 = recs[0]
     fr = rec0.blk.fromRGB
     H = rec0.H
-    with _on_side(adj[0].gf, u):
+    fused = rec0.inp is None and not rec0.last
+    t1_fused = None
+    with _on_side(adj[0].gf, u, *((adj[0].gz1, rec0.inpb) if fused else ())):
         ops.fromrgb_wgrad(adj[0].gf, u, fr._gw, None, N, C, H, H, fr.c)
-    cur = _bytes_first(lambda m, _: ops.fromrgb_fwd(u, fr.conv.weight.data, None, N, C, H, H, fr.c, 1.0, mask=m, mask_slope=fr.slope),
-                       saved.Sign.inp(rec0), None, count=False)
+        if fused:
+            c1 = rec0.blk.c1
+            ops.conv2d_wgrad_fromrgb_tangent(u, fr.conv.weight.data, fr.c, rec0.inpb, fr.slope, adj[0].gz1, c1._gw, N, C, H, H, c1.c)
+    if fused:
+        t1_fused = ops.conv2d_fromrgb_tangent(u, fr.conv.weight.data, fr.c, rec0.inpb, fr.slope, c1.conv.weight.data, rec0.a1b, c1.slope,
+                                              N, C, H, H, c1.c)
+        cur = None
+    else:
+        cur = _bytes_first(lambda m, _: ops.fromrgb_fwd(u, fr.conv.weight.data, None, N, C, H, H, fr.c, 1.0, mask=m, mask_slope=fr.slope),
+                           saved.Sign.inp(rec0), None, count=False)
     hvp = None
     t2 = None
     pn = bool(getattr(D, 'pixelnorm', False))
@@ -922,8 +945,11 @@
             if pn:
                 t2, injs[idx].inj2 = ops.pixelnorm_tangent(t2, rec.a2, rec.r2, adj[idx].gy2)
         else:
-            _wgrad(cur, adj[idx].gz1, c1, N, H, bias=False, defer=True)
-            t1 = _conv(cur, c1, N, H, mask=saved.Sign.a1(rec), bias=False)
+            if idx == 0 and t1_fused is not None:
+                t1 = t1_fused
+            else:
+                _wgrad(cur, adj[idx].gz1, c1, N, H, bias=False, defer=True)
+                t1 = _conv(cur, c1, N, H, mask=saved.Sign.a1(rec), bias=False)
             if pn:
                 t1, injs[idx].inj1 = ops.pixelnorm_tangent(t1, rec.a1, rec.r1, adj[idx].gy1)
             _wgrad(t1, adj[idx].gz2, c2, N, H, bias=False, defer=True)
diff --git a/pggan-pytorch_amd/ops.py b/pggan-pytorch_amd/ops.py
--- a/pggan-pytorch_amd/ops.py
+++ b/pggan-pytorch_amd/ops.py
@@ -319,6 +319,26 @@
     _lib.call('pg_conv2d_masked_fromrgb_bwd_nhwc', _p(gz), _p(wt), _p(mask_bytes), mask_slope, _p(gf), _p(rgb_w), rgb_scale, _p(gimg),
               _p(img), _p(rgb_dw), _p(rgb_db), N, C, H, W, cin, cout, scale, _stream())
     return gf, gimg
+
+
+def conv2d_wgrad_fromrgb(img, rgb_w, rgb_b, rgb_scale, rgb_slope, gz, dw, db, N, C, H, W, scale):
+    cout, cmid = dw.shape[2], dw.shape[3]
+    _lib.call('pg_conv2d_wgrad_fromrgb_nhwc', _p(img), _p(rgb_w), _p(rgb_b), rgb_scale, rgb_slope, _p(gz), _p(dw), _p(db),
+              N, C, H, W, cmid, cout, scale, _stream())
+
+
+def conv2d_fromrgb_tangent(v, rgb_w, rgb_scale, x_signs, rgb_slope, w, mask_bytes, mask_slope, N, C, H, W, scale):
+    cout, cmid = w.shape[2], w.shape[3]
+    y = _empty((N, H, W, cout), device=v.device, dtype=torch.float32)
+    _lib.call('pg_conv2d_fromrgb_tangent_nhwc', _p(v), _p(rgb_w), rgb_scale, _p(x_signs), rgb_slope, _p(w), _p(mask_bytes), mask_slope,
+              _p(y), N, C, H, W, cmid, cout, scale, _stream())
+    return y
+
+
+def conv2d_wgrad_fromrgb_tangent(v, rgb_w, rgb_scale, x_signs, rgb_slope, gz, dw, N, C, H, W, scale):
+    cout, cmid = dw.shape[2], dw.shape[3]
+    _lib.call('pg_conv2d_wgrad_fromrgb_tangent_nhwc', _p(v), _p(rgb_w), rgb_scale, _p(x_signs), rgb_slope, _p(gz), _p(dw),
+              N, C, H, W, cmid, cout, scale, _stream())
 
 
 
```

Result: no change. 301.6 images/sec (median of 6 runs) (+0.5%).
